# luo-ziyuan/NeRF_Signature

Hardware: AMD Instinct MI355X
Metric: training rays/sec @4096 rays (hotdog, 32-bit msg) (higher is better)
Workload: dtype f32 (hash gather, compositing) + fp16 MFMA with f32 accumulate (MLPs); 1 GPU; BASELINE configs[1]: Blender/hotdog-like S0, --wtmk_tcnn, 4096 content + 32x12x12 block rays, 32-bit msg; content_rays=4096, block_rays_total=4608, block_rays_this_rank=4608, message_dim=32, parallelism=dp1, capacity_overflow=False, recaptured_with_more_headroom_after_warmup=False, execution=hipgraph, graph_segments=1

## Files before the change

include/nerfsig.h:

```cpp
#ifndef NERFSIG_H_
#define NERFSIG_H_

#include <stddef.h>
#include <stdint.h>

#ifdef __cplusplus
extern "C" {
#endif

#define NSIG_OK 0
#define NSIG_ERR_ARG 1
#define NSIG_ERR_LAUNCH 2

#define NSIG_TABLE_ROWS (1u << 19)
#define NSIG_BASE_LEVELS 16
#define NSIG_MAX_MESSAGE_DIM 64

typedef void *nsig_stream_t;

int nsig_abi_version(void);
const char *nsig_last_error(void);


int rm_near_far_from_aabb(const float *rays_o, const float *rays_d, const float *aabb, uint32_t N, float min_near,
                          float *nears, float *fars, nsig_stream_t stream);
int rm_sph_from_ray(const float *rays_o, const float *rays_d, float radius, uint32_t N, float *coords,
                    nsig_stream_t stream);
int rm_morton3D(const int32_t *coords, uint32_t N, int32_t *indices, nsig_stream_t stream);
int rm_morton3D_invert(const int32_t *indices, uint32_t N, int32_t *coords, nsig_stream_t stream);
int rm_packbits(const float *grid, uint32_t n_bytes, float density_thresh, uint8_t *bitfield, nsig_stream_t stream);

size_t rg_refresh_draw_scratch_bytes(uint32_t N, uint32_t H);
int rg_refresh_begin(float *fresh, uint32_t n_cells, nsig_stream_t stream);
int rg_refresh_draw(int32_t *keys, int32_t *ids, uint32_t N, uint32_t H, const float *grid_cas, void *scratch, uint64_t seed, const int32_t *iter_dev,
                    uint32_t cas, nsig_stream_t stream);
int rg_refresh_points(const int32_t *keys, const int32_t *ids, uint32_t n, uint32_t H, float extent, float half_cell, uint64_t seed, const int32_t *iter_dev,
                      uint32_t cas, float *xyz, int32_t *cells, nsig_stream_t stream);
int rg_refresh_scatter(const float *sigmas, const int32_t *cells, uint32_t n, float density_scale, float *fresh, nsig_stream_t stream);
size_t rg_refresh_partials_bytes(uint32_t n_cells);
int rg_refresh_finish(float *grid, const float *fresh, uint32_t n_cells, float decay, void *partials, float density_thresh, uint8_t *bitfield,
                      float *mean_density, int32_t *iter_dev, const int32_t *count_ring, uint32_t window, const uint32_t *step_dev, int32_t *mean_count,
                      nsig_stream_t stream);


size_t rm_march_train_scratch_bytes(uint32_t N, uint32_t max_steps);
int rm_march_train_count(const float *rays_o, const float *rays_d, const uint8_t *grid, float bound, float dt_gamma,
                         uint32_t max_steps, uint32_t N, uint32_t C, uint32_t H, const float *nears,
                         const float *fars, const float *noises, int32_t *counts, float *t_rec,
                         nsig_stream_t stream);
int rm_march_train_scan(const int32_t *counts, uint32_t N, int32_t *rays, int32_t *counter, nsig_stream_t stream);
int rm_march_train_scan_blocks(uint32_t N);
int rm_march_train_scan_wide(const int32_t *counts, uint32_t N, int32_t *rays, int32_t *counter, int32_t *block_sums,
                             nsig_stream_t stream);
int rm_march_train_write(const float *rays_o, const float *rays_d, float bound, float dt_gamma, uint32_t max_steps,
                         uint32_t N, uint32_t C, uint32_t H, uint32_t M, const float *nears, const float *noises,
                         const float *t_rec, const int32_t *rays, const int32_t *counter, float *xyzs, float *dirs,
                         float *deltas, nsig_stream_t stream);

int rm_march_train_count_nf(const float *rays_o, const float *rays_d, const float *aabb, float min_near, const uint8_t *grid,
                            float bound, float dt_gamma, uint32_t max_steps, uint32_t N, uint32_t C, uint32_t H,
                            const float *noises, float *nears, float *fars, int32_t *counts, float *t_rec, nsig_stream_t stream);
int rm_march_train_scan_write_max_rays(void);
int rm_march_train_scan_write(const float *rays_o, const float *rays_d, float bound, float dt_gamma, uint32_t max_steps, uint32_t N,
                              uint32_t C, uint32_t H, uint32_t M, const float *nears, const float *noises, const float *t_rec,
                              const int32_t *counts, int32_t *rays, int32_t *counter, float *xyzs, float *dirs, float *deltas,
                              nsig_stream_t stream);

int rm_composite_train_fwd(const float *sigmas, const float *rgbs, const float *deltas, const int32_t *rays,
                           uint32_t M, uint32_t N, float T_thresh, float *weights_sum, float *depth, float *image,
                           nsig_stream_t stream);
int rm_composite_train_bwd(const float *grad_weights_sum, const float *grad_image, const float *sigmas,
                           const float *rgbs, const float *deltas, const int32_t *rays, const float *weights_sum,
                           const float *image, uint32_t M, uint32_t N, float T_thresh, float *grad_sigmas,
                           float *grad_rgbs, nsig_stream_t stream);


int rm_march(uint32_t n_alive, uint32_t n_step, const int32_t *rays_alive, const float *rays_t, const float *rays_o,
             const float *rays_d, float bound, float dt_gamma, uint32_t max_steps, uint32_t C, uint32_t H,
             const uint8_t *grid, const float *nears, const float *fars, float *xyzs, float *dirs, float *deltas,
             const float *noises, uint32_t M_rows, nsig_stream_t stream);
int rm_composite(uint32_t n_alive, uint32_t n_step, float T_thresh, int32_t *rays_alive, float *rays_t,
                 const float *sigmas, const float *rgbs, const float *deltas, float *weights_sum, float *depth,
                 float *image, nsig_stream_t stream);
int rm_compact_alive(const int32_t *rays_alive, uint32_t n_alive, int32_t *rays_alive_out, int32_t *n_out,
                     nsig_stream_t stream);

int rm_eval_begin(uint32_t N, uint32_t *ctl, int32_t *rays_alive, nsig_stream_t stream);
int rm_eval_march(const uint32_t *ctl, uint32_t N, const int32_t *rays_alive, const float *rays_t, const float *rays_o, const float *rays_d,
                  float bound, float dt_gamma, uint32_t max_steps, uint32_t C, uint32_t H, const uint8_t *density_bitfield, const float *fars,
                  float *xyzs, float *dirs, float *deltas, const float *noises, nsig_stream_t stream);
int rm_eval_composite(const uint32_t *ctl, uint32_t N, float T_thresh, float density_scale, int32_t *rays_alive, float *rays_t,
                      const float *sigmas, const float *rgbs, const float *deltas, float *weights_sum, float *depth, float *image,
                      nsig_stream_t stream);
int rm_eval_compact(uint32_t *ctl, uint32_t N, uint32_t max_steps, const int32_t *rays_alive, int32_t *rays_alive_out, nsig_stream_t stream);


int rg_get_rays(const float *poses, float fx, float fy, float cx, float cy, uint32_t H, uint32_t W, const int64_t *inds,
                uint32_t B, uint32_t N, float *rays_o, float *rays_d, nsig_stream_t stream);

int rg_sample_rays(const float *poses, uint32_t P, const float *images, float fx, float fy, float cx, float cy, uint32_t H, uint32_t W,
                   uint32_t N, const int32_t *step_counter, uint32_t stride, uint32_t offset, uint64_t seed, float *rays_o, float *rays_d,
                   float *gt, int64_t *inds_out, int32_t *pose_out, nsig_stream_t stream);


int hg_codebook_presum(const float *const *tables_host, uint32_t D, float *S, nsig_stream_t stream);

int hg_codebook_presum_sel(const float *const *all_tables_host, const float *message, uint32_t D, float *S,
                           nsig_stream_t stream);

int hg_encode_fwd(const float *x01, uint32_t M, const float *const *base_tables_host, const float *S, float *feat,
                  nsig_stream_t stream);

int hg_codebook_encode_fwd(const float *x01, uint32_t M, const float *const *tables_host, uint32_t D, float *out,
                           nsig_stream_t stream);

int hg_codebook_bwd(const float *x01, uint32_t M, const float *dfeat, float *G, nsig_stream_t stream);

int hg_scatter_sliced(const float *rec, uint32_t M, float *G, nsig_stream_t stream);

size_t hg_scatter_binned_scratch_bytes(uint32_t M);
int hg_scatter_binned(const float *rec, uint32_t M, float *G, void *scratch, nsig_stream_t stream);

size_t hg_scatter_plan_bytes(uint32_t M);
int hg_scatter_plan(const float *xyzs, uint32_t M, float bound, void *plan, nsig_stream_t stream);
int hg_scatter_planned(const void *plan, uint32_t M, float *G, nsig_stream_t stream);

int hg_fanout_grad(const float *G, float *const *grads_host, uint32_t D, int accumulate, nsig_stream_t stream);

int hg_level_lookup(const float *x01, uint32_t M, float resolution, int32_t *rows, float *weights,
                    nsig_stream_t stream);


int opt_codebook_adam(const float *G, float *const *params_host, float *const *exp_avg_host, float *const *exp_avg_sq_host,
                      uint32_t D, float beta1, float beta2, float eps, const float *step_size_host,
                      const float *inv_bc2_sqrt_host, float grad_scale, nsig_stream_t stream);

int opt_codebook_adam_sel(const float *G, float *const *params_host, float *const *exp_avg_host, float *const *exp_avg_sq_host,
                          float *const *steps_host, const float *message, uint32_t D, const float *lr, float beta1,
                          float beta2, float eps, float grad_scale, float *scratch, nsig_stream_t stream);

int opt_codebook_adam_sel_next(const float *G, float *const *params_host, float *const *exp_avg_host, float *const *exp_avg_sq_host,
                               float *const *steps_host, const float *message, uint32_t D, const float *lr, float beta1,
                               float beta2, float eps, float grad_scale, float *scratch, const float *next_message,
                               float *S_next, nsig_stream_t stream);


size_t mlp_packed_bytes(void);
int mlp_pack_weights(const float *sigma_params, const float *color_params, void *packed, nsig_stream_t stream);

int mlp_get_precision(void);
int mlp_set_precision(int mode);
int mlp_get_pipelined(void);
int mlp_set_pipelined(int mask);

#define FIELD_MASK_WORDS 6

#define NSIG_PLANES_F32 0
#define NSIG_PLANES_MIXED 1
int field_fwd(const float *xyzs, const float *dirs, uint32_t M, float bound, const float *const *base_tables_host,
              const float *S, const void *packed, float *sigmas, float *rgbs, float *geo_feat, uint32_t *masks,
              const void *planes, int planes_layout, nsig_stream_t stream);

size_t hg_planes_bytes(uint32_t M);
int hg_encode_planes(const float *xyzs, uint32_t M, float bound, const float *const *base_tables_host, const float *S,
                     void *planes, nsig_stream_t stream);
int hg_encode_planes_rows(const float *xyzs, uint32_t M_capacity, const uint32_t *rows_dev, float bound,
                          const float *const *base_tables_host, const float *S, void *planes, nsig_stream_t stream);
int hg_encode_planes_mixed(const float *xyzs, uint32_t M_capacity, const uint32_t *rows_dev, float bound, const float *const *base_tables_host,
                           const float *S, void *planes, nsig_stream_t stream);
int field_fwd_rows(const float *xyzs, const float *dirs, uint32_t M_capacity, const uint32_t *rows_dev, float bound,
                   const float *const *base_tables_host, const float *S, const void *packed, float *sigmas, float *rgbs, const void *planes,
                   int planes_layout, nsig_stream_t stream);

int hg_warm_tables(const float *const *base_tables_host, const float *S, float *sink, nsig_stream_t stream);

int hg_encode_codebook_plane(const float *xyzs, uint32_t M, float bound, const float *S, void *planes, int planes_layout, void *plan_to_reset,
                             nsig_stream_t stream);

int field_color_fwd(const float *dirs, const float *geo_feat, uint32_t M, const void *packed, float *rgbs,
                    nsig_stream_t stream);

int field_bwd(const float *xyzs, uint32_t M, float bound, const float *grad_sigmas, const float *grad_rgbs,
              const float *sigmas, const float *rgbs, const uint32_t *masks, const void *packed, float *G,
              float *dfeat_out, float *rec_out, nsig_stream_t stream);
int field_bwd_planned(const float *xyzs, uint32_t M, float bound, const float *grad_sigmas, const float *grad_rgbs,
                      const float *sigmas, const float *rgbs, const uint32_t *masks, const void *packed, void *plan,
                      nsig_stream_t stream);

int opt_adam_dense(uint32_t n, float *const *params_host, const float *const *grads_host, float *const *exp_avg_host,
                   float *const *exp_avg_sq_host, float *const *steps_host, const uint32_t *numel_host, const float *lr, float beta1,
                   float beta2, float eps, float grad_scale, float *scratch, nsig_stream_t stream);
int opt_adam_dense_host(uint32_t n, float *const *params_host, const float *const *grads_host, float *const *exp_avg_host,
                        float *const *exp_avg_sq_host, const uint32_t *numel_host, const float *step_sizes_host, const float *inv_bc2_host,
                        float beta1, float beta2, float eps, float grad_scale, nsig_stream_t stream);

int rm_composite_train_finish_fwd(const float *sigmas, const float *rgbs, const float *deltas, const int32_t *rays, uint32_t M, uint32_t N,
                                  float T_thresh, const float *nears, const float *fars, const float *bg, uint32_t bg_stride,
                                  float *weights_sum, float *depth, float *image, float *image_out, float *depth_out, nsig_stream_t stream);
int rm_composite_train_finish_bwd(const float *grad_weights_sum, const float *grad_image_out, const float *sigmas, const float *rgbs,
                                  const float *deltas, const int32_t *rays, const float *weights_sum, const float *image, const float *bg,
                                  uint32_t bg_stride, uint32_t M, uint32_t N, float T_thresh, uint32_t rays_in_order, float *grad_sigmas,
                                  float *grad_rgbs, nsig_stream_t stream);


int rm_finish_fwd(const float *image, const float *depth, const float *weights_sum, const float *nears, const float *fars, const float *bg,
                  uint32_t bg_stride, uint32_t N, float *image_out, float *depth_out, nsig_stream_t stream);
int rm_finish_bwd(const float *grad_image, const float *grad_depth, const float *depth, const float *nears, const float *fars, const float *bg,
                  uint32_t bg_stride, uint32_t N, float *grad_weights_sum, float *grad_depth_in, nsig_stream_t stream);

int loop_step_begin(float *G, uint32_t n_floats, const float *ring_dev, uint32_t slots, uint32_t width, uint32_t *counter, float *msg,
                    nsig_stream_t stream);
void *nsig_host_device_pointer(const void *pinned_host);

int wm_loss_fwd(const float *content, const float *gt, uint32_t n_content, const float *decoded, const float *message, uint32_t D, float temp,
                float lambda_w, float lambda_i, float *losses3, float *d_content, float *d_decoded, nsig_stream_t stream);
int wm_loss_bwd(const float *g_lossi, const float *g_lossw, const float *g_loss, float lambda_w, float lambda_i, const float *d_content,
                uint32_t n_content, const float *d_decoded, uint32_t D, float *grad_content, float *grad_decoded, nsig_stream_t stream);


int dec_bn_gelu_fwd(const float *x, const float *gamma, const float *beta, uint32_t N, uint32_t C, uint32_t P, float eps, float *y,
                    float *save, nsig_stream_t stream);
int dec_bn_gelu_bwd(const float *dy, const float *x, const float *gamma, const float *beta, const float *save, uint32_t N, uint32_t C,
                    uint32_t P, float *dx, float *dgamma, float *dbeta, nsig_stream_t stream);

size_t dec_workspace_bytes(uint32_t B, uint32_t Cin, uint32_t H, uint32_t W);
int dec_forward(const float *img, uint32_t input_mode, const float *mean_host, const float *std_host, const float *const *params_host,
                uint32_t B, uint32_t Cin, uint32_t H, uint32_t W, float eps, void *workspace, float *decoded, float *clamped_out,
                nsig_stream_t stream);
int dec_backward(const float *grad_decoded, const float *img, uint32_t input_mode, const float *mean_host, const float *std_host,
                 const float *const *params_host, uint32_t B, uint32_t Cin, uint32_t H, uint32_t W, void *workspace,
                 float *const *grads_host, float *grad_img, nsig_stream_t stream, nsig_stream_t weights_stream);

int dec_forward_train(const float *img, const float *mean_host, const float *std_host, const float *const *params_host, uint32_t B,
                      uint32_t Cin, uint32_t H, uint32_t W, float eps, void *workspace, float *decoded, float *clamped_out,
                      uint32_t distortion, const float *dist_param, const float *dist_noise, const float *bce_message, float bce_temp,
                      float bce_scale, float *bce_seed, nsig_stream_t stream);
int dec_backward_train(const float *grad_decoded, const float *img, const float *mean_host, const float *std_host,
                       const float *const *params_host, uint32_t B, uint32_t Cin, uint32_t H, uint32_t W, void *workspace,
                       float *const *grads_host, float *grad_img, uint32_t distortion, const float *dist_param,
                       const float *dist_noise, float *grad_scratch, nsig_stream_t stream, nsig_stream_t weights_stream);
int wm_distort_draw(uint32_t distortion, uint64_t seed, const uint32_t *step_counter, uint32_t n_noise, float *param_out,
                    float *noise_out, nsig_stream_t stream);
int wm_distort_fwd(const float *img, uint32_t B, uint32_t H, uint32_t W, uint32_t C, uint32_t distortion, const float *dist_param,
                   const float *dist_noise, float *out, nsig_stream_t stream);
int wm_distort_bwd(const float *grad_out, const float *img, uint32_t B, uint32_t H, uint32_t W, uint32_t C, uint32_t distortion,
                   const float *dist_param, const float *dist_noise, float *grad_img, nsig_stream_t stream);
int wm_distort_geom_fwd(const float *img, uint32_t B, uint32_t H, uint32_t W, uint32_t C, uint32_t distortion, const float *dist_param,
                        uint32_t W_out, float *out, float *clamped_out, nsig_stream_t stream);
int wm_distort_geom_bwd(const float *grad_out, const float *img, uint32_t B, uint32_t H, uint32_t W, uint32_t C, uint32_t distortion,
                        const float *dist_param, uint32_t W_out, float *grad_img, nsig_stream_t stream);


int field_fwd_trace(const float *xyzs, const float *dirs, uint32_t M, float bound, const float *const *base_tables_host,
                    const void *packed, const void *planes, float *sigmas, float *rgbs, uint32_t *masks, float *act_hs,
                    float *act_cin, float *act_h1, float *act_h2, nsig_stream_t stream);
int field_bwd_trace(uint32_t M, const float *grad_sigmas, const float *grad_rgbs, const float *sigmas, const float *rgbs,
                    const uint32_t *masks, const void *packed, float *d_hs, float *d_so, float *d_h1, float *d_h2, float *d_out,
                    void *d_planes, nsig_stream_t stream);
int hg_scatter_level(const float *xyzs, float bound, const void *d_plane, uint32_t M, uint32_t level, float *G,
                     nsig_stream_t stream);
size_t hg_scatter_levels_scratch_bytes(uint32_t M);
int hg_scatter_levels(const float *xyzs, float bound, const void *d_planes, uint32_t M, uint32_t stride, float *const *G_host,
                      void *scratch, nsig_stream_t stream);


int field_fwd_trace_rows(const float *xyzs, const float *dirs, uint32_t M_capacity, const uint32_t *rows_dev, float bound,
                         const float *const *base_tables_host, const void *packed, const void *planes, float *sigmas, float *rgbs,
                         uint32_t *masks, float *act_hs, float *act_cin, float *act_h1, float *act_h2, nsig_stream_t stream);
int field_bwd_trace_rows(uint32_t M_capacity, const uint32_t *rows_dev, const float *grad_sigmas, const float *grad_rgbs, const float *sigmas,
                         const float *rgbs, const uint32_t *masks, const void *packed, float *d_hs, float *d_so, float *d_h1, float *d_h2,
                         float *d_out, void *d_planes, nsig_stream_t stream);
size_t field_wgrad_scratch_bytes(uint32_t M);
int field_wgrad(uint32_t M, const uint32_t *rows_dev, const void *planes, const float *act_hs, const float *act_cin, const float *act_h1,
                const float *act_h2, const float *d_hs, const float *d_so, const float *d_h1, const float *d_h2, const float *d_out,
                void *scratch, float *grad_sigma_params, float *grad_color_params, nsig_stream_t stream);
size_t field_bwd_wgrad_scratch_bytes(uint32_t M);
int field_bwd_wgrad(uint32_t M, const uint32_t *rows_dev, const float *grad_sigmas, const float *grad_rgbs, const float *sigmas, const float *rgbs,
                    const uint32_t *masks, const void *packed, const void *planes, const float *act_hs, const float *act_cin, const float *act_h1,
                    const float *act_h2, void *d_planes, void *scratch, float *grad_sigma_params, float *grad_color_params, nsig_stream_t stream);
int field_fwd_trace_f16(const float *xyzs, const float *dirs, uint32_t M_capacity, const uint32_t *rows_dev, float bound,
                        const float *const *base_tables_host, const void *packed, const void *planes, float *sigmas, float *rgbs,
                        uint32_t *masks, void *act_hs, void *act_cin, void *act_h1, void *act_h2, nsig_stream_t stream);
int field_bwd_wgrad_f16(uint32_t M, const uint32_t *rows_dev, const float *grad_sigmas, const float *grad_rgbs, const float *sigmas, const float *rgbs,
                        const uint32_t *masks, const void *packed, const void *planes, const void *act_hs, const void *act_cin, const void *act_h1,
                        const void *act_h2, void *d_planes, void *scratch, float *grad_sigma_params, float *grad_color_params, nsig_stream_t stream);
int rm_composite_train_mse(const float *sigmas, const float *rgbs, const float *deltas, const int32_t *rays, uint32_t M, uint32_t N, float T_thresh,
                           const float *nears, const float *fars, const float *bg, uint32_t bg_stride, const float *gt, uint32_t n_values,
                           float grad_scale, float *weights_sum, float *depth, float *image, float *image_out, float *depth_out, float *grad_image,
                           float *grad_sigmas, float *grad_rgbs, nsig_stream_t stream);
int opt_ema_update(uint32_t n, const float *const *params_host, float *const *shadow_host, const uint32_t *numel_host, const uint32_t *num_updates,
                   double decay, nsig_stream_t stream);
int clean_loss(const float *image, const float *gt, uint32_t n_values, float grad_scale, float *loss, float *grad_image,
               uint32_t *step_dev, const int32_t *march_counter, int32_t *count_ring, float *loss_ring, uint32_t loss_ring_len,
               float *noise_next, uint32_t n_noise, uint64_t seed, nsig_stream_t stream);
size_t hg_levels_plan_bytes(uint32_t M);
int hg_levels_plan(const float *xyzs, uint32_t M, const uint32_t *rows_dev, float bound, void *plan, nsig_stream_t stream);
int hg_levels_scatter(const float *xyzs, uint32_t M, const uint32_t *rows_dev, float bound, const void *d_planes, uint32_t stride,
                      void *plan, float *const *G_host, nsig_stream_t stream);
int hg_levels_scatter_adam(const float *xyzs, uint32_t M, const uint32_t *rows_dev, float bound, const void *d_planes, uint32_t stride,
                           void *plan, float *const *params_host, float *const *exp_avg_host, float *const *exp_avg_sq_host,
                           float *const *steps_host, const float *lr, float beta1, float beta2, float eps, float grad_scale, float *scratch,
                           nsig_stream_t stream);


size_t mc_scratch_bytes(uint32_t nx, uint32_t ny, uint32_t nz);
int mc_count(const float *u, uint32_t nx, uint32_t ny, uint32_t nz, float threshold, void *scratch, uint32_t *totals, nsig_stream_t stream);
int mc_emit(const float *u, uint32_t nx, uint32_t ny, uint32_t nz, float threshold, void *scratch, uint32_t n_vertices, uint32_t n_triangles,
            float *vertices, int32_t *triangles, nsig_stream_t stream);

#ifdef __cplusplus
}
#endif
#endif
```

nerf_signature_amd/_native.py:

```python
import ctypes
import os

import torch

_PKG = os.path.dirname(os.path.abspath(__file__))
LIB_PATH = os.path.join(_PKG, "lib", "libnerfsig.so")

_c = ctypes
_vp, _u32, _fl, _int, _sz = _c.c_void_p, _c.c_uint32, _c.c_float, _c.c_int, _c.c_size_t

SIGNATURES = {
    "nsig_abi_version": [],
    "nsig_last_error": [],
    "nsig_host_device_pointer": [_vp],
    "rg_sample_rays": [_vp, _u32, _vp, _fl, _fl, _fl, _fl, _u32, _u32, _u32, _vp, _u32, _u32, _c.c_uint64, _vp, _vp, _vp, _vp, _vp, _vp],
    "rg_get_rays": [_vp, _fl, _fl, _fl, _fl, _u32, _u32, _vp, _u32, _u32, _vp, _vp, _vp],
    "rm_near_far_from_aabb": [_vp, _vp, _vp, _u32, _fl, _vp, _vp, _vp],
    "rm_sph_from_ray": [_vp, _vp, _fl, _u32, _vp, _vp],
    "rm_morton3D": [_vp, _u32, _vp, _vp],
    "rm_morton3D_invert": [_vp, _u32, _vp, _vp],
    "rm_packbits": [_vp, _u32, _fl, _vp, _vp],
    "rg_refresh_draw_scratch_bytes": [_u32, _u32],
    "rg_refresh_begin": [_vp, _u32, _vp],
    "rg_refresh_draw": [_vp, _vp, _u32, _u32, _vp, _vp, _c.c_uint64, _vp, _u32, _vp],
    "rg_refresh_points": [_vp, _vp, _u32, _u32, _fl, _fl, _c.c_uint64, _vp, _u32, _vp, _vp, _vp],
    "rg_refresh_scatter": [_vp, _vp, _u32, _fl, _vp, _vp],
    "rg_refresh_partials_bytes": [_u32],
    "rg_refresh_finish": [_vp, _vp, _u32, _fl, _vp, _fl, _vp, _vp, _vp, _vp, _u32, _vp, _vp, _vp],
    "rm_march_train_scratch_bytes": [_u32, _u32],
    "rm_march_train_count": [_vp, _vp, _vp, _fl, _fl, _u32, _u32, _u32, _u32, _vp, _vp, _vp, _vp, _vp, _vp],
    "rm_march_train_scan": [_vp, _u32, _vp, _vp, _vp],
    "rm_march_train_scan_blocks": [_u32],
    "rm_march_train_scan_wide": [_vp, _u32, _vp, _vp, _vp, _vp],
    "rm_march_train_write": [_vp, _vp, _fl, _fl, _u32, _u32, _u32, _u32, _u32, _vp, _vp, _vp, _vp, _vp, _vp, _vp, _vp, _vp],
    "rm_march_train_count_nf": [_vp, _vp, _vp, _fl, _vp, _fl, _fl, _u32, _u32, _u32, _u32, _vp, _vp, _vp, _vp, _vp, _vp],
    "rm_march_train_scan_write_max_rays": [],
    "rm_march_train_scan_write": [_vp, _vp, _fl, _fl, _u32, _u32, _u32, _u32, _u32, _vp, _vp, _vp, _vp, _vp, _vp, _vp, _vp, _vp, _vp],
    "rm_composite_train_fwd": [_vp, _vp, _vp, _vp, _u32, _u32, _fl, _vp, _vp, _vp, _vp],
    "rm_composite_train_bwd": [_vp, _vp, _vp, _vp, _vp, _vp, _vp, _vp, _u32, _u32, _fl, _vp, _vp, _vp],
    "rm_march": [_u32, _u32, _vp, _vp, _vp, _vp, _fl, _fl, _u32, _u32, _u32, _vp, _vp, _vp, _vp, _vp, _vp, _vp, _u32, _vp],
    "rm_composite": [_u32, _u32, _fl, _vp, _vp, _vp, _vp, _vp, _vp, _vp, _vp, _vp],
    "rm_compact_alive": [_vp, _u32, _vp, _vp, _vp],
    "rm_eval_begin": [_u32, _vp, _vp, _vp],
    "rm_eval_march": [_vp, _u32, _vp, _vp, _vp, _vp, _fl, _fl, _u32, _u32, _u32, _vp, _vp, _vp, _vp, _vp, _vp, _vp],
    "rm_eval_composite": [_vp, _u32, _fl, _fl, _vp, _vp, _vp, _vp, _vp, _vp, _vp, _vp, _vp],
    "rm_eval_compact": [_vp, _u32, _u32, _vp, _vp, _vp],
    "hg_encode_planes_rows": [_vp, _u32, _vp, _fl, _vp, _vp, _vp, _vp],
    "hg_encode_planes_mixed": [_vp, _u32, _vp, _fl, _vp, _vp, _vp, _vp],
    "field_fwd_rows": [_vp, _vp, _u32, _vp, _fl, _vp, _vp, _vp, _vp, _vp, _vp, _int, _vp],
    "hg_codebook_presum": [_vp, _u32, _vp, _vp],
    "hg_codebook_presum_sel": [_vp, _vp, _u32, _vp, _vp],
    "hg_encode_fwd": [_vp, _u32, _vp, _vp, _vp, _vp],
    "hg_codebook_encode_fwd": [_vp, _u32, _vp, _u32, _vp, _vp],
    "hg_codebook_bwd": [_vp, _u32, _vp, _vp, _vp],
    "hg_scatter_sliced": [_vp, _u32, _vp, _vp],
    "hg_fanout_grad": [_vp, _vp, _u32, _int, _vp],
    "hg_level_lookup": [_vp, _u32, _fl, _vp, _vp, _vp],
    "opt_codebook_adam": [_vp, _vp, _vp, _vp, _u32, _fl, _fl, _fl, _vp, _vp, _fl, _vp],
    "opt_codebook_adam_sel": [_vp, _vp, _vp, _vp, _vp, _vp, _u32, _vp, _fl, _fl, _fl, _fl, _vp, _vp],
    "opt_codebook_adam_sel_next": [_vp, _vp, _vp, _vp, _vp, _vp, _u32, _vp, _fl, _fl, _fl, _fl, _vp, _vp, _vp, _vp],
    "mlp_packed_bytes": [],
    "mlp_get_precision": [],
    "mlp_set_precision": [_int],
    "mlp_get_pipelined": [],
    "mlp_set_pipelined": [_int],
    "mlp_pack_weights": [_vp, _vp, _vp, _vp],
    "hg_planes_bytes": [_u32],
    "hg_encode_planes": [_vp, _u32, _fl, _vp, _vp, _vp, _vp],
    "hg_warm_tables": [_vp, _vp, _vp, _vp],
    "hg_encode_codebook_plane": [_vp, _u32, _fl, _vp, _vp, _int, _vp, _vp],
    "field_fwd": [_vp, _vp, _u32, _fl, _vp, _vp, _vp, _vp, _vp, _vp, _vp, _vp, _int, _vp],
    "field_color_fwd": [_vp, _vp, _u32, _vp, _vp, _vp],
    "opt_adam_dense_host": [_u32, _vp, _vp, _vp, _vp, _vp, _vp, _vp, _fl, _fl, _fl, _fl, _vp],
    "opt_adam_dense": [_u32, _vp, _vp, _vp, _vp, _vp, _vp, _vp, _fl, _fl, _fl, _fl, _vp, _vp],
    "rm_composite_train_finish_fwd": [_vp, _vp, _vp, _vp, _u32, _u32, _fl, _vp, _vp, _vp, _u32, _vp, _vp, _vp, _vp, _vp, _vp],
    "rm_composite_train_finish_bwd": [_vp, _vp, _vp, _vp, _vp, _vp, _vp, _vp, _vp, _u32, _u32, _u32, _fl, _u32, _vp, _vp, _vp],
    "rm_finish_fwd": [_vp, _vp, _vp, _vp, _vp, _vp, _u32, _u32, _vp, _vp, _vp],
    "rm_finish_bwd": [_vp, _vp, _vp, _vp, _vp, _vp, _u32, _u32, _vp, _vp, _vp],
    "loop_step_begin": [_vp, _u32, _vp, _u32, _u32, _vp, _vp, _vp],
    "wm_loss_fwd": [_vp, _vp, _u32, _vp, _vp, _u32, _fl, _fl, _fl, _vp, _vp, _vp, _vp],
    "wm_loss_bwd": [_vp, _vp, _vp, _fl, _fl, _vp, _u32, _vp, _u32, _vp, _vp, _vp],
    "dec_bn_gelu_fwd": [_vp, _vp, _vp, _u32, _u32, _u32, _fl, _vp, _vp, _vp],
    "dec_bn_gelu_bwd": [_vp, _vp, _vp, _vp, _vp, _u32, _u32, _u32, _vp, _vp, _vp, _vp],
    "dec_workspace_bytes": [_u32, _u32, _u32, _u32],
    "dec_forward": [_vp, _u32, _vp, _vp, _vp, _u32, _u32, _u32, _u32, _fl, _vp, _vp, _vp, _vp],
    "dec_backward": [_vp, _vp, _u32, _vp, _vp, _vp, _u32, _u32, _u32, _u32, _vp, _vp, _vp, _vp, _vp],
    "dec_forward_train": [_vp, _vp, _vp, _vp, _u32, _u32, _u32, _u32, _fl, _vp, _vp, _vp, _u32, _vp, _vp, _vp, _fl, _fl, _vp, _vp],
    "dec_backward_train": [_vp, _vp, _vp, _vp, _vp, _u32, _u32, _u32, _u32, _vp, _vp, _vp, _u32, _vp, _vp, _vp, _vp, _vp],
    "wm_distort_draw": [_u32, _c.c_uint64, _vp, _u32, _vp, _vp, _vp],
    "wm_distort_fwd": [_vp, _u32, _u32, _u32, _u32, _u32, _vp, _vp, _vp, _vp],
    "wm_distort_bwd": [_vp, _vp, _u32, _u32, _u32, _u32, _u32, _vp, _vp, _vp, _vp],
    "wm_distort_geom_fwd": [_vp, _u32, _u32, _u32, _u32, _u32, _vp, _u32, _vp, _vp, _vp],
    "wm_distort_geom_bwd": [_vp, _vp, _u32, _u32, _u32, _u32, _u32, _vp, _u32, _vp, _vp],
    "field_fwd_trace": [_vp, _vp, _u32, _fl, _vp, _vp, _vp, _vp, _vp, _vp, _vp, _vp, _vp, _vp, _vp],
    "field_bwd_trace": [_u32, _vp, _vp, _vp, _vp, _vp, _vp, _vp, _vp, _vp, _vp, _vp, _vp, _vp],
    "hg_scatter_level": [_vp, _fl, _vp, _u32, _u32, _vp, _vp],
    "hg_scatter_binned_scratch_bytes": [_u32],
    "hg_scatter_binned": [_vp, _u32, _vp, _vp, _vp],
    "hg_scatter_levels_scratch_bytes": [_u32],
    "hg_scatter_levels": [_vp, _fl, _vp, _u32, _u32, _vp, _vp, _vp],
    "field_bwd": [_vp, _u32, _fl, _vp, _vp, _vp, _vp, _vp, _vp, _vp, _vp, _vp, _vp],
    "field_bwd_planned": [_vp, _u32, _fl, _vp, _vp, _vp, _vp, _vp, _vp, _vp, _vp],
    "hg_scatter_plan_bytes": [_u32],
    "hg_scatter_plan": [_vp, _u32, _fl, _vp, _vp],
    "hg_scatter_planned": [_vp, _u32, _vp, _vp],
    "field_fwd_trace_rows": [_vp, _vp, _u32, _vp, _fl, _vp, _vp, _vp, _vp, _vp, _vp, _vp, _vp, _vp, _vp, _vp],
    "field_fwd_trace_f16": [_vp, _vp, _u32, _vp, _fl, _vp, _vp, _vp, _vp, _vp, _vp, _vp, _vp, _vp, _vp, _vp],
    "field_bwd_trace_rows": [_u32, _vp, _vp, _vp, _vp, _vp, _vp, _vp, _vp, _vp, _vp, _vp, _vp, _vp, _vp],
    "field_wgrad_scratch_bytes": [_u32],
    "field_wgrad": [_u32, _vp, _vp, _vp, _vp, _vp, _vp, _vp, _vp, _vp, _vp, _vp, _vp, _vp, _vp, _vp],
    "field_bwd_wgrad_scratch_bytes": [_u32],
    "field_bwd_wgrad": [_u32, _vp, _vp, _vp, _vp, _vp, _vp, _vp, _vp, _vp, _vp, _vp, _vp, _vp, _vp, _vp, _vp, _vp],
    "field_bwd_wgrad_f16": [_u32, _vp, _vp, _vp, _vp, _vp, _vp, _vp, _vp, _vp, _vp, _vp, _vp, _vp, _vp, _vp, _vp, _vp],
    "rm_composite_train_mse": [_vp, _vp, _vp, _vp, _u32, _u32, _fl, _vp, _vp, _vp, _u32, _vp, _u32, _fl, _vp, _vp, _vp, _vp, _vp, _vp, _vp, _vp, _vp],
    "opt_ema_update": [_u32, _vp, _vp, _vp, _vp, _c.c_double, _vp],
    "clean_loss": [_vp, _vp, _u32, _fl, _vp, _vp, _vp, _vp, _vp, _vp, _u32, _vp, _u32, _c.c_uint64, _vp],
    "hg_levels_plan_bytes": [_u32],
    "hg_levels_plan": [_vp, _u32, _vp, _fl, _vp, _vp],
    "hg_levels_scatter": [_vp, _u32, _vp, _fl, _vp, _u32, _vp, _vp, _vp],
    "hg_levels_scatter_adam": [_vp, _u32, _vp, _fl, _vp, _u32, _vp, _vp, _vp, _vp, _vp, _vp, _fl, _fl, _fl, _fl, _vp, _vp],
    "mc_scratch_bytes": [_u32, _u32, _u32],
    "mc_count": [_vp, _u32, _u32, _u32, _fl, _vp, _vp, _vp],
    "mc_emit": [_vp, _u32, _u32, _u32, _fl, _vp, _u32, _u32, _vp, _vp, _vp],
}
_RESTYPES = {"nsig_last_error": _c.c_char_p, "nsig_host_device_pointer": _c.c_void_p, "rm_march_train_scratch_bytes": _sz, "mlp_packed_bytes": _sz, "hg_planes_bytes": _sz, "dec_workspace_bytes": _sz, "hg_scatter_levels_scratch_bytes": _sz, "hg_scatter_binned_scratch_bytes": _sz, "hg_scatter_plan_bytes": _sz, "field_wgrad_scratch_bytes": _sz, "field_bwd_wgrad_scratch_bytes": _sz, "hg_levels_plan_bytes": _sz, "rg_refresh_partials_bytes": _sz, "rg_refresh_draw_scratch_bytes": _sz, "mc_scratch_bytes": _sz}

_lib = None


class NativeError(RuntimeError):
    pass


def load():
    global _lib
    if _lib is not None:
        return _lib
    path = os.environ.get("NERFSIG_LIB", LIB_PATH)
    if not os.path.exists(path):
        raise NativeError(f"{path} not found: the HIP extension is required (no fallback). "
                          f"Build it with `python -m nerf_signature_amd.build`.")
    _lib = ctypes.CDLL(path)
    _lib.nsig_last_error.restype = _c.c_char_p
    return _lib


_bound = {}


def fn(name):
    f = _bound.get(name)
    if f is None:
        lib = load()
        try:
            f = getattr(lib, name)
        except AttributeError as e:
            raise NativeError(f"libnerfsig.so does not export {name}; rebuild with `python -m nerf_signature_amd.build --force`") from e
        f.argtypes = SIGNATURES[name]
        f.restype = _RESTYPES.get(name, _int)
        _bound[name] = f
    return f


def verify_exports():
    for name in SIGNATURES:
        fn(name)
    return sorted(SIGNATURES)


def call(name, *args):
    rc = fn(name)(*args)
    if rc != 0:
        msg = load().nsig_last_error().decode("utf-8", "replace")
        raise (ValueError if rc == 1 else NativeError)(f"{name} failed (code {rc}): {msg}")


def mlp_precision_name():
    return ("fp16 MFMA with f32 accumulate (MLPs)" if fn("mlp_get_precision")() == 1 else "split-bf16 MFMA (3 per product) with f32 accumulate (MLPs)")


def mlp_mfma_per_wave():
    return (24, "f16") if fn("mlp_get_precision")() == 1 else (72, "bf16")


def set_mlp_precision(name):
    call("mlp_set_precision", {"bf16x3": 0, "f16": 1}[name])


def ptr(t):
    if t is None:
        return None
    if not t.is_cuda:
        raise ValueError("libnerfsig entry points take device tensors; got a CPU tensor")
    if not t.is_contiguous():
        raise ValueError("libnerfsig entry points take contiguous tensors")
    return t.data_ptr()


_raw_stream = getattr(torch._C, "_cuda_getCurrentRawStream", None)


def stream():
    if _raw_stream is not None:
        return _raw_stream(torch.cuda.current_device())
    return torch.cuda.current_stream().cuda_stream


def ptr_array(tensors):
    arr = (ctypes.c_void_p * len(tensors))(*[ptr(t) for t in tensors])
    return arr


def check(t, dtype, name, shape_last=None):
    if t.dtype != dtype:
        raise ValueError(f"{name}: expected dtype {dtype}, got {t.dtype}")
    if shape_last is not None and t.shape[-1] != shape_last:
        raise ValueError(f"{name}: expected last dimension {shape_last}, got {tuple(t.shape)}")
    return t
```

nerf_signature_amd/csrc/field.hip:

```cpp
#include <cstdlib>
#include <cstring>
#include <mutex>
#include <unordered_set>
#include "fieldmlp.h"

#include <stdlib.h>

namespace nsig {


__device__ inline float fwd_weight(int frag, int lane, int j, const float *__restrict__ sp, const float *__restrict__ cp) {
    const int r = lane & 31, h = lane >> 5;
    if (frag < F1) {
        const int rb = (frag - F0) >> 1, ks = (frag - F0) & 1;
        return sp[kSigmaW1 + (32 * rb + r) * 32 + 16 * ks + 8 * h + j];
    }
    if (frag < F2) return r < 16 ? sp[kSigmaW2 + r * 64 + k_from_acc(frag - F1, h, j)] : 0.0f;
    if (frag < F3) {
        const int rb = (frag - F2) >> 1, ks = (frag - F2) & 1;
        int cin;
        if (ks == 0) cin = 8 * h + j;
        else { const int rho = row_of_reg(h, j); cin = rho == 0 ? 31 : 15 + rho; }
        return cp[kColorW1 + (32 * rb + r) * 32 + cin];
    }
// ... 477 lines not shown
        color_branch<P>(lds, lane, h, dirs[3 * (size_t)sl], dirs[3 * (size_t)sl + 1], dirs[3 * (size_t)sl + 2], geo8, mask_c, rgb);
        if (s < M && h == 0) { rgbs[3 * (size_t)s] = rgb[0]; rgbs[3 * (size_t)s + 1] = rgb[1]; rgbs[3 * (size_t)s + 2] = rgb[2]; }
    }
}


template <typename P, bool kFull = false>
__global__ void __launch_bounds__(256) k_field_bwd(const float *__restrict__ xyzs, uint32_t M, float bound, float cb_cell,
                                                   const float *__restrict__ g_sigma, const float *__restrict__ g_rgb,
                                                   const float *__restrict__ sigmas, const float *__restrict__ rgbs,
                                                   const uint32_t *__restrict__ masks, const char *__restrict__ packed,
                                                   float *__restrict__ G, float *__restrict__ dfeat_out, float *__restrict__ rec_out,
                                                   GradTrace gt = GradTrace{}, uint32_t stride = 0, ScatterPlan plan = ScatterPlan{},
                                                   const uint32_t *__restrict__ rows_dev = nullptr) {
    extern __shared__ __attribute__((aligned(16))) char lds[];
    if (rows_dev != nullptr) {
        const uint32_t r = *rows_dev;
        if (r == 0) return;
        M = min(M, r);
    }
    stage_weights(lds, packed + P::kBwdOffset, (int)P::kBwdLds);
    constexpr size_t kHalf = kBwdBytes;
    constexpr bool kNormalise = P::kMfmaPerProduct == 1 && !kFull;
    const int lane = threadIdx.x & 63, wid = threadIdx.x >> 6;
    const int p = lane & 31, h = lane >> 5;
    const uint32_t n_tiles = ceil_div(M, 32u);
    const float e_lo = expf(-15.0f), e_hi = expf(15.0f);
    const bool planned = !kFull && plan.hd != nullptr;
    uint32_t gbits = 0;
    const uint32_t xcd = blockIdx.x & 7u, per_xcd = gridDim.x >> 3, n_chunks = ceil_div(n_tiles, 32u);
    for (uint32_t lq = blockIdx.x >> 3;; lq += per_xcd) {
        const uint32_t chunk = (lq >> 3) * 8u + xcd;
        if (chunk >= n_chunks) break;
        const uint32_t tile = (chunk * 8u + (lq & 7u)) * 4u + wid;
        if (tile >= n_tiles) continue;
        const uint32_t s = tile * 32 + p;
        const bool live = s < M;
        const uint32_t sl = min(s, M - 1);
        const uint32_t *mrow = masks + (size_t)tile * 192 + lane;
        const uint32_t mask_s = mrow[0], mask_c0 = mrow[64], mask_c1 = mrow[128];
        uint4 dst = make_uint4(0u, 0u, 0u, 0u);
        if (planned) dst = plan.dest[sl];

        typename P::Op dout[1];
        float dv[8];
#pragma unroll
        for (int j = 0; j < 8; ++j) {
            float v = 0.0f;
            if (j < 3 && h == 0 && live) {
                const float c = rgbs[3 * (size_t)sl + j];
                v = g_rgb[3 * (size_t)sl + j] * (c * (1.0f - c));
            }
            dv[j] = v;
            if (kFull) gt.d_out[(size_t)(8 * h + j) * stride + s] = v;
        }
        float head0 = 0.0f;
        if (h == 0 && live) head0 = g_sigma[sl] * fminf(fmaxf(sigmas[sl], e_lo), e_hi);
        float unscale = 1.0f;
        if (kNormalise) {
            float amp = fmaxf(fmaxf(fabsf(dv[0]), fabsf(dv[1])), fmaxf(fabsf(dv[2]), fabsf(head0)));
            amp = fmaxf(amp, __shfl_xor(amp, 32, 64));
            const uint32_t e = (__float_as_uint(amp) >> 23) & 0xffu;
            if (e >= 1u && e <= 253u) {
                const float sc = __uint_as_float((254u - e) << 23);
                unscale = __uint_as_float(e << 23);
                dv[0] *= sc; dv[1] *= sc; dv[2] *= sc; head0 *= sc;
            }
        }
#pragma unroll
        for (int j = 0; j < 8; j += 2) P::put2(dout[0], j >> 1, dv[j], dv[j + 1]);
        f32x16 hid[2];
        typename P::Op b4[4];
        mfma_layer<P, 2, 1>(lds, kHalf, B0, lane, dout, hid);
        mask_to_operand<P>(hid, mask_c1, b4);
        if (kFull) store_rows64(gt.d_h2, stride, s, h, hid, [=](float v, int i) { return ((mask_c1 >> mask_bit<P>(i)) & 1u) ? v : 0.0f; });
        mfma_layer<P, 2, 4>(lds, kHalf, B1, lane, b4, hid);
        mask_to_operand<P>(hid, mask_c0, b4);
        if (kFull) store_rows64(gt.d_h1, stride, s, h, hid, [=](float v, int i) { return ((mask_c0 >> mask_bit<P>(i)) & 1u) ? v : 0.0f; });
        f32x16 dso[1];
        mfma_layer<P, 1, 4>(lds, kHalf, B2, lane, b4, dso);

        typename P::Op dhead[1];
        float head8[8];
#pragma unroll
        for (int r = 0; r < 8; ++r) head8[r] = dso[0][r];
        if (h == 0) head8[0] = head0;
#pragma unroll
        for (int r = 0; r < 8; ++r)
            if (kFull) gt.d_so[(size_t)row_of_reg(h, r) * stride + s] = head8[r];
#pragma unroll
        for (int r = 0; r < 8; r += 2) P::put2(dhead[0], r >> 1, head8[r], head8[r + 1]);
        mfma_layer<P, 2, 1>(lds, kHalf, B3, lane, dhead, hid);
        mask_to_operand<P>(hid, mask_s, b4);
        if (kFull) {
            store_rows64(gt.d_hs, stride, s, h, hid, [=](float v, int i) { return ((mask_s >> mask_bit<P>(i)) & 1u) ? v : 0.0f; });
            f32x16 dall[1];
            mfma_layer<P, 1, 4>(lds, kHalf, B4F, lane, b4, dall);
#pragma unroll
            for (int r = 0; r < 16; r += 2) {
                float2 v;
                v.x = dall[0][r]; v.y = dall[0][r + 1];
                gt.d_planes[(size_t)(row_of_reg16(h, r) >> 1) * stride + s] = v;
            }
            continue;
        }
        f32x16 dfe[1];
        mfma_layer<P, 1, 4>(lds, kHalf, B4, lane, b4, dfe);

        const float g0 = __shfl(dfe[0][0], p, 64) * unscale, g1 = __shfl(dfe[0][1], p, 64) * unscale;
        if (!live) continue;
        if (dfeat_out != nullptr && h == 0) { dfeat_out[2 * (size_t)s] = g0; dfeat_out[2 * (size_t)s + 1] = g1; }
        const float two_b = 2.0f * bound;
        const float x01 = (xyzs[3 * (size_t)s] + bound) / two_b, y01 = (xyzs[3 * (size_t)s + 1] + bound) / two_b, z01 = (xyzs[3 * (size_t)s + 2] + bound) / two_b;
        if (planned) {
            uint32_t ix, iy, iz;
            float wx, wy, wz;
            codebook_axis(x01, ix, wx);
            codebook_axis(y01, iy, wy);
            codebook_axis(z01, iz, wz);
            const uint32_t q0 = 2u * (uint32_t)h;
            plan.queue[h ? dst.z : dst.x] = pair_entry(ix, pair_hash(iy, iz, q0), wx, wy, wz, g0, g1, q0);
            plan.queue[h ? dst.w : dst.y] = pair_entry(ix, pair_hash(iy, iz, q0 + 1u), wx, wy, wz, g0, g1, q0 + 1u);
            gbits = max(gbits, max(__float_as_uint(g0) & 0x7fffffffu, __float_as_uint(g1) & 0x7fffffffu));
            continue;
        }
        if (rec_out != nullptr && h == 0) {
            uint32_t ix, iy, iz;
            float wx, wy, wz;
            codebook_axis(x01, ix, wx);
            codebook_axis(y01, iy, wy);
            codebook_axis(z01, iz, wz);
            uint4 *r4 = reinterpret_cast<uint4 *>(rec_out) + 2 * (size_t)s;
            r4[0] = make_uint4(ix | (iy << 16), iz, __float_as_uint(wx), __float_as_uint(wy));
            r4[1] = make_uint4(__float_as_uint(wz), __float_as_uint(g0), __float_as_uint(g1), 0u);
        }
        if (G == nullptr || (g0 == 0.0f && g1 == 0.0f)) continue;
        Corner8 c;
        corner_rows(x01, y01, z01, cb_cell, c);
#pragma unroll
        for (int k = 0; k < 8; ++k) {
            if ((k >> 2) != h) continue;
            float *row = G + 2 * (size_t)c.row[k];
            atomicAdd(row, corner_weight(c, k, g0));
            atomicAdd(row + 1, corner_weight(c, k, g1));
        }
    }
    if (planned) {
#pragma unroll
        for (int d = 32; d >= 1; d >>= 1) gbits = max(gbits, (uint32_t)__shfl_xor((int)gbits, d, 64));
        if (lane == 0 && gbits > __hip_atomic_load(&plan.hd->gmax_bits, __ATOMIC_RELAXED, __HIP_MEMORY_SCOPE_AGENT)) atomicMax(&plan.hd->gmax_bits, gbits);
    }
}

template <typename P>
__device__ inline void field_bwd_pipelined(const char *lds, int lane, const float *__restrict__ xyzs, uint32_t M, float bound,
                                           const float *__restrict__ g_sigma, const float *__restrict__ g_rgb, const float *__restrict__ sigmas,
                                           const float *__restrict__ rgbs, const uint32_t *__restrict__ masks, ScatterPlan plan) {
    constexpr size_t kHalf = kBwdBytes;
    constexpr bool kNormalise = P::kMfmaPerProduct == 1;
    const int p = lane & 31, h = lane >> 5;
    const uint32_t wid = (uint32_t)__builtin_amdgcn_readfirstlane((int)(threadIdx.x >> 6));
    const uint32_t n_tiles = ceil_div(M, 32u);
    const float e_lo = expf(-15.0f), e_hi = expf(15.0f), two_b = 2.0f * bound;
    uint32_t gbits = 0;
    const uint32_t xcd = blockIdx.x & 7u, per_xcd = gridDim.x >> 3, n_chunks = ceil_div(n_tiles, 32u);
    uint32_t lq = blockIdx.x >> 3;
    auto next_tile = [&]() -> uint32_t {
        for (;; lq += per_xcd) {
            const uint32_t chunk = (lq >> 3) * 8u + xcd;
            if (chunk >= n_chunks) return ~0u;
            const uint32_t tile = (chunk * 8u + (lq & 7u)) * 4u + wid;
            if (tile < n_tiles) {
                lq += per_xcd;
                return tile;
            }
        }
    };
    typedef float f32x3u __attribute__((ext_vector_type(3), aligned(4)));
    uint32_t n_mask[3] = {0u, 0u, 0u};
    typedef uint32_t u32x4 __attribute__((ext_vector_type(4)));
    u32x4 n_dst = {0u, 0u, 0u, 0u};
    f32x3u n_rgb = {0.0f, 0.0f, 0.0f}, n_grgb = {0.0f, 0.0f, 0.0f}, n_xyz = {0.0f, 0.0f, 0.0f};
    float n_gs = 0.0f, n_sig = 0.0f;
    auto request = [&](uint32_t tile) {
        const uint32_t s = tile * 32 + p, sl = min(s, M - 1);
        const uint32_t *mrow = masks + (size_t)tile * 192 + lane;
        n_mask[0] = mrow[0]; n_mask[1] = mrow[64]; n_mask[2] = mrow[128];
        n_dst = *reinterpret_cast<const u32x4 *>(plan.dest + sl);
        n_rgb = *reinterpret_cast<const f32x3u *>(rgbs + 3 * (size_t)sl);
        n_grgb = *reinterpret_cast<const f32x3u *>(g_rgb + 3 * (size_t)sl);
        n_xyz = *reinterpret_cast<const f32x3u *>(xyzs + 3 * (size_t)sl);
        n_gs = g_sigma[sl];
        n_sig = sigmas[sl];
    };
    bool have = false;
    float p_x = 0.0f, p_y = 0.0f, p_z = 0.0f, p_g0 = 0.0f, p_g1 = 0.0f;
    uint32_t p_d0 = 0u, p_d1 = 0u;
    bool p_live = false;
    auto store_prev = [&]() {
        if (!p_live) return;
        uint32_t ix, iy, iz;
        float wx, wy, wz;
        codebook_axis((p_x + bound) / two_b, ix, wx);
        codebook_axis((p_y + bound) / two_b, iy, wy);
        codebook_axis((p_z + bound) / two_b, iz, wz);
        const uint32_t q0 = 2u * (uint32_t)h;
        plan.queue[p_d0] = pair_entry(ix, pair_hash(iy, iz, q0), wx, wy, wz, p_g0, p_g1, q0);
        plan.queue[p_d1] = pair_entry(ix, pair_hash(iy, iz, q0 + 1u), wx, wy, wz, p_g0, p_g1, q0 + 1u);
        gbits = max(gbits, max(__float_as_uint(p_g0) & 0x7fffffffu, __float_as_uint(p_g1) & 0x7fffffffu));
    };
    uint32_t tile = next_tile();
    if (tile != ~0u) request(tile);
    while (tile != ~0u) {
        const uint32_t s = tile * 32 + p;
        const bool live = s < M;
        float dv[3] = {0.0f, 0.0f, 0.0f}, head0 = 0.0f;
        if (h == 0 && live) {
            dv[0] = n_grgb.x * (n_rgb.x * (1.0f - n_rgb.x));
            dv[1] = n_grgb.y * (n_rgb.y * (1.0f - n_rgb.y));
            dv[2] = n_grgb.z * (n_rgb.z * (1.0f - n_rgb.z));
            head0 = n_gs * fminf(fmaxf(n_sig, e_lo), e_hi);
        }
        uint32_t mask_s = n_mask[0], mask_c0 = n_mask[1], mask_c1 = n_mask[2];
        uint32_t d0 = h ? n_dst.z : n_dst.x, d1 = h ? n_dst.w : n_dst.y;
        float cx = n_xyz.x, cy = n_xyz.y, cz = n_xyz.z;
        asm volatile("" : "+v"(dv[0]), "+v"(dv[1]), "+v"(dv[2]), "+v"(head0), "+v"(mask_s), "+v"(mask_c0), "+v"(mask_c1), "+v"(d0), "+v"(d1),
                     "+v"(cx), "+v"(cy), "+v"(cz) :: "memory");
        if (have) store_prev();
        const uint32_t upcoming = next_tile();
        if (upcoming != ~0u) request(upcoming);
        asm volatile("" ::: "memory");

        float unscale = 1.0f;
        if (kNormalise) {
            float amp = fmaxf(fmaxf(fabsf(dv[0]), fabsf(dv[1])), fmaxf(fabsf(dv[2]), fabsf(head0)));
            amp = fmaxf(amp, __shfl_xor(amp, 32, 64));
            const uint32_t e = (__float_as_uint(amp) >> 23) & 0xffu;
            if (e >= 1u && e <= 253u) {
                const float sc = __uint_as_float((254u - e) << 23);
                unscale = __uint_as_float(e << 23);
                dv[0] *= sc; dv[1] *= sc; dv[2] *= sc; head0 *= sc;
            }
        }
        typename P::Op dout[1];
        P::put2(dout[0], 0, dv[0], dv[1]);
        P::put2(dout[0], 1, dv[2], 0.0f);
        P::put2(dout[0], 2, 0.0f, 0.0f);
        P::put2(dout[0], 3, 0.0f, 0.0f);
        f32x16 hid[2];
        typename P::Op b4[4];
        mfma_layer<P, 2, 1>(lds, kHalf, B0, lane, dout, hid);
        mask_to_operand<P>(hid, mask_c1, b4);
        mfma_layer<P, 2, 4>(lds, kHalf, B1, lane, b4, hid);
        mask_to_operand<P>(hid, mask_c0, b4);
        f32x16 dso[1];
        mfma_layer<P, 1, 4>(lds, kHalf, B2, lane, b4, dso);
        typename P::Op dhead[1];
        float head8[8];
#pragma unroll
        for (int r = 0; r < 8; ++r) head8[r] = dso[0][r];
        if (h == 0) head8[0] = head0;
#pragma unroll
        for (int r = 0; r < 8; r += 2) P::put2(dhead[0], r >> 1, head8[r], head8[r + 1]);
        mfma_layer<P, 2, 1>(lds, kHalf, B3, lane, dhead, hid);
        mask_to_operand<P>(hid, mask_s, b4);
        f32x16 dfe[1];
        mfma_layer<P, 1, 4>(lds, kHalf, B4, lane, b4, dfe);
        p_g0 = __shfl(dfe[0][0], p, 64) * unscale;
        p_g1 = __shfl(dfe[0][1], p, 64) * unscale;
        p_x = cx; p_y = cy; p_z = cz; p_d0 = d0; p_d1 = d1; p_live = live;
        have = true;
        tile = upcoming;
    }
    if (have) store_prev();
#pragma unroll
    for (int d = 32; d >= 1; d >>= 1) gbits = max(gbits, (uint32_t)__shfl_xor((int)gbits, d, 64));
    if (lane == 0 && gbits > __hip_atomic_load(&plan.hd->gmax_bits, __ATOMIC_RELAXED, __HIP_MEMORY_SCOPE_AGENT)) atomicMax(&plan.hd->gmax_bits, gbits);
}

template <typename P>
__global__ void __launch_bounds__(256) k_field_bwd_train(const float *__restrict__ xyzs, uint32_t M, float bound, const float *__restrict__ g_sigma,
                                                         const float *__restrict__ g_rgb, const float *__restrict__ sigmas, const float *__restrict__ rgbs,
                                                         const uint32_t *__restrict__ masks, const char *__restrict__ packed, ScatterPlan plan) {
    extern __shared__ __attribute__((aligned(16))) char lds[];
    stage_weights(lds, packed + P::kBwdOffset, (int)P::kBwdLds);
    field_bwd_pipelined<P>(lds, threadIdx.x & 63, xyzs, M, bound, g_sigma, g_rgb, sigmas, rgbs, masks, plan);
}

}

using namespace nsig;

NSIG_EXPORT size_t mlp_packed_bytes(void) { return kPackedBytes; }

static int g_mlp_precision = -1;
static int mlp_precision() {
    if (g_mlp_precision < 0) {
        const char *e = getenv("NERFSIG_MLP");
        g_mlp_precision = (e != nullptr && (e[0] == 'b' || e[0] == 'B')) ? 0 : 1;
    }
    return g_mlp_precision;
}
NSIG_EXPORT int mlp_get_precision(void) { return mlp_precision(); }
NSIG_EXPORT int mlp_set_precision(int mode) {
    NSIG_REQUIRE(mode == 0 || mode == 1, "mlp_set_precision: 0 (bf16x3) or 1 (f16)");
    g_mlp_precision = mode;
    return NSIG_OK;
}

NSIG_EXPORT int mlp_pack_weights(const float *sigma_params, const float *color_params, void *packed, nsig_stream_t stream) {
    NSIG_REQUIRE(sigma_params && color_params && packed, "mlp_pack_weights: null pointer");
    NSIG_REQUIRE((reinterpret_cast<uintptr_t>(packed) & 15) == 0, "mlp_pack_weights: packed must be 16-byte aligned");
    const int total = (kFwdFrags + kBwdFrags) * 512;
    k_pack_weights<<<ceil_div(total, 256), 256, 0, as_stream(stream)>>>(sigma_params, color_params, reinterpret_cast<__bf16 *>(packed));
    return check_launch("mlp_pack_weights");
}

static int g_mlp_pipelined = 3;
static int mlp_pipelined() {
    return g_mlp_pipelined;
}
static bool fwd_pipelined() { return (mlp_pipelined() & 1) != 0; }
static bool bwd_pipelined() { return (mlp_pipelined() & 2) != 0; }
NSIG_EXPORT int mlp_get_pipelined(void) { return mlp_pipelined(); }
NSIG_EXPORT int mlp_set_pipelined(int mask) {
    NSIG_REQUIRE(mask >= 0 && mask <= 3, "mlp_set_pipelined: bit 0 = forward, bit 1 = backward");
    g_mlp_pipelined = mask;
    return NSIG_OK;
}
static uint32_t field_grid(uint32_t M, bool forward = false, uint32_t per_cu = 0) {
    const uint32_t blocks = ceil_div(ceil_div(ceil_div(M, 32u), 4u), 8u) * 8u;
    const uint32_t cap = (uint32_t)kCUs * (per_cu ? per_cu : (forward ? 4u : 3u));
    return blocks < cap ? blocks : cap;
}

static int fill_base_tables(const float *const *host, TablePtrs &base, const char *who) {
    NSIG_REQUIRE(host, "%s: null base table list", who);
    for (int l = 0; l < NSIG_BASE_LEVELS; ++l) {
        NSIG_REQUIRE(host[l] != nullptr, "%s: base table %d is null", who, l);
        base.p[l] = host[l];
    }
    return NSIG_OK;
}

static SlotTable default_slots(bool with_codebook) {
    static const uint8_t kWith[8][4] = {{16, 255, 255, 255}, {15, 255, 255, 255}, {14, 0, 255, 255}, {13, 1, 255, 255}, {12, 2, 3, 255}, {11, 4, 5, 255}, {10, 9, 255, 255}, {8, 7, 6, 255}};
    static const uint8_t kWithout[8][4] = {{15, 255, 255, 255}, {14, 255, 255, 255}, {13, 255, 255, 255}, {12, 255, 255, 255}, {11, 0, 1, 255}, {10, 2, 3, 255}, {9, 8, 4, 255}, {7, 6, 5, 255}};
    SlotTable t{};
    for (int slot = 0; slot < 8; ++slot)
        for (int k = 0; k < 4; ++k) {
            const uint8_t l = (with_codebook ? kWith : kWithout)[slot][k];
            if (l != 255) t.level[slot][t.n[slot]++] = l;
        }
    return t;
}

NSIG_EXPORT int hg_warm_tables(const float *const *base_tables_host, const float *S, float *sink, nsig_stream_t stream) {
    NSIG_REQUIRE(sink != nullptr, "hg_warm_tables: sink is one writable float (never written)");
    TablePtrs base{};
    if (int e = fill_base_tables(base_tables_host, base, "hg_warm_tables")) return e;
    k_warm_tables<<<8 * 128, 256, 0, as_stream(stream)>>>(base, S, default_slots(S != nullptr), sink);
    return check_launch("hg_warm_tables");
}

NSIG_EXPORT size_t hg_planes_bytes(uint32_t M) { return (size_t)(NSIG_BASE_LEVELS + 1) * ceil_div(M, 32u) * 32u * sizeof(float2); }

static int check_layout(int layout, const char *who) {
    NSIG_REQUIRE(layout == NSIG_PLANES_F32 || layout == NSIG_PLANES_MIXED, "%s: planes_layout must be NSIG_PLANES_F32 (0) or NSIG_PLANES_MIXED (1)", who);
    return NSIG_OK;
}

static int encode_planes_impl(const float *xyzs, uint32_t M, float bound, const float *const *base_tables_host, const float *S, void *planes,
                              const uint32_t *rows_dev, nsig_stream_t stream, bool mixed = false) {
    if (M == 0) return NSIG_OK;
    NSIG_REQUIRE(xyzs && planes, "hg_encode_planes: null pointer");
    NSIG_REQUIRE(bound > 0.0f, "hg_encode_planes: bound must be positive");
    NSIG_REQUIRE((reinterpret_cast<uintptr_t>(planes) & 7) == 0, "hg_encode_planes: planes must be 8-byte aligned");
    TablePtrs base{};
    if (int e = fill_base_tables(base_tables_host, base, "hg_encode_planes")) return e;
    const uint32_t stride = ceil_div(M, 32u) * 32u;
    const SlotTable tab = default_slots(S != nullptr);
    int covered[NSIG_BASE_LEVELS + 1] = {};
    for (int s = 0; s < 8; ++s)
        for (int i = 0; i < tab.n[s]; ++i) covered[tab.level[s][i]] += 1;
    for (int l = 0; l < NSIG_BASE_LEVELS + (S != nullptr ? 1 : 0); ++l)
        NSIG_REQUIRE(covered[l] == 1, "hg_encode_planes: level %d is assigned to %d slots", l, covered[l]);
    NSIG_REQUIRE(S != nullptr || covered[NSIG_BASE_LEVELS] == 0, "hg_encode_planes: slot table names the codebook level but S is NULL");
    const uint32_t tiles = ceil_div(stride, 256u);
    const uint32_t per_slot = tiles < 8192u ? tiles : 8192u;
    if (mixed) k_encode_planes<true><<<per_slot * 8, 256, 0, as_stream(stream)>>>(xyzs, M, bound, base, make_level_geom(), S, reinterpret_cast<float2 *>(planes), stride, tab, rows_dev);
    else k_encode_planes<false><<<per_slot * 8, 256, 0, as_stream(stream)>>>(xyzs, M, bound, base, make_level_geom(), S, reinterpret_cast<float2 *>(planes), stride, tab, rows_dev);
    return check_launch("hg_encode_planes");
}

NSIG_EXPORT int hg_encode_planes_mixed(const float *xyzs, uint32_t M_capacity, const uint32_t *rows_dev, float bound, const float *const *base_tables_host,
                                       const float *S, void *planes, nsig_stream_t stream) {
    NSIG_REQUIRE(mlp_precision() == 1, "hg_encode_planes_mixed: the mixed layout carries the fp16 MLP's operands (mlp_set_precision(1))");
    return encode_planes_impl(xyzs, M_capacity, bound, base_tables_host, S, planes, rows_dev, stream, true);
}

NSIG_EXPORT int hg_encode_planes(const float *xyzs, uint32_t M, float bound, const float *const *base_tables_host, const float *S, void *planes,
                                 nsig_stream_t stream) {
    return encode_planes_impl(xyzs, M, bound, base_tables_host, S, planes, nullptr, stream);
}

NSIG_EXPORT int hg_encode_planes_rows(const float *xyzs, uint32_t M_capacity, const uint32_t *rows_dev, float bound, const float *const *base_tables_host,
                                      const float *S, void *planes, nsig_stream_t stream) {
    NSIG_REQUIRE(rows_dev != nullptr, "hg_encode_planes_rows: null row count");
    return encode_planes_impl(xyzs, M_capacity, bound, base_tables_host, S, planes, rows_dev, stream);
}

NSIG_EXPORT int hg_encode_codebook_plane(const float *xyzs, uint32_t M, float bound, const float *S, void *planes, int planes_layout, void *plan_to_reset,
                                         nsig_stream_t stream) {
    if (M == 0) return NSIG_OK;
    if (int e = check_layout(planes_layout, "hg_encode_codebook_plane")) return e;
    NSIG_REQUIRE(xyzs && S && planes, "hg_encode_codebook_plane: null pointer");
    NSIG_REQUIRE(bound > 0.0f, "hg_encode_codebook_plane: bound must be positive");
    NSIG_REQUIRE((reinterpret_cast<uintptr_t>(planes) & 7) == 0, "hg_encode_codebook_plane: planes must be 8-byte aligned");
    NSIG_REQUIRE(plan_to_reset == nullptr || (reinterpret_cast<uintptr_t>(plan_to_reset) & 15) == 0, "hg_encode_codebook_plane: plan must be 16-byte aligned");
    const uint32_t stride = ceil_div(M, 32u) * 32u;
    float2 *plane = planes_layout == NSIG_PLANES_MIXED ? mixed_f32_plane(planes, stride, NSIG_BASE_LEVELS) : reinterpret_cast<float2 *>(planes) + (size_t)NSIG_BASE_LEVELS * stride;
    k_encode_codebook_plane<<<ceil_div(stride, 256u), 256, 0, as_stream(stream)>>>(xyzs, M, bound, make_level_geom().cell[NSIG_BASE_LEVELS], S, plane, stride,
                                                                                  reinterpret_cast<BinHeader *>(plan_to_reset));
    return check_launch("hg_encode_codebook_plane");
}

static int field_fwd_impl(const float *xyzs, const float *dirs, uint32_t M, float bound, const float *const *base_tables_host,
                          const float *S, const void *packed, float *sigmas, float *rgbs, float *geo_feat, uint32_t *masks,
                          const void *planes, int planes_layout, const uint32_t *rows_dev, nsig_stream_t stream) {
    if (M == 0) return NSIG_OK;
    NSIG_REQUIRE(xyzs && packed && sigmas, "field_fwd: null pointer");
    NSIG_REQUIRE(rgbs == nullptr || dirs != nullptr, "field_fwd: dirs is required when rgbs is requested");
    NSIG_REQUIRE(bound > 0.0f, "field_fwd: bound must be positive");
    NSIG_REQUIRE((reinterpret_cast<uintptr_t>(packed) & 15) == 0, "field_fwd: packed must be 16-byte aligned");
    TablePtrs base{};
    if (int e = fill_base_tables(base_tables_host, base, "field_fwd")) return e;
    const char *pk = reinterpret_cast<const char *>(packed);
    hipStream_t st = as_stream(stream);
    const bool f16 = mlp_precision() == 1;
    if (planes == nullptr) {
        if (f16) k_field_fwd<F16, 0><<<field_grid(M, true), 256, F16::kFwdLds, st>>>(xyzs, dirs, M, bound, base, make_level_geom(), S, nullptr, 0, pk, sigmas, rgbs, geo_feat, masks, ActTrace{}, rows_dev);
        else k_field_fwd<Bf16x3, 0><<<field_grid(M, true), 256, Bf16x3::kFwdLds, st>>>(xyzs, dirs, M, bound, base, make_level_geom(), S, nullptr, 0, pk, sigmas, rgbs, geo_feat, masks, ActTrace{}, rows_dev);
        return check_launch("field_fwd");
    }
    NSIG_REQUIRE((reinterpret_cast<uintptr_t>(planes) & 7) == 0, "field_fwd: planes must be 8-byte aligned");
    const uint32_t stride = ceil_div(M, 32u) * 32u;
    const float2 *pl = reinterpret_cast<const float2 *>(planes);
    if (int e = check_layout(planes_layout, "field_fwd")) return e;
    const bool mixed = planes_layout == NSIG_PLANES_MIXED;
    NSIG_REQUIRE(!mixed || f16, "field_fwd: this plane set was written in the mixed (fp16) layout; the split-bf16 MLP needs hg_encode_planes");
    if (f16 && fwd_pipelined() && dirs != nullptr && rgbs != nullptr && geo_feat == nullptr) {
        if (mixed) k_field_fwd_train<F16, true><<<field_grid(M, true, 2), 256, F16::kFwdLds, st>>>(dirs, M, S != nullptr, pl, stride, pk, sigmas, rgbs, masks, rows_dev);
        else k_field_fwd_train<F16, false><<<field_grid(M, true, 2), 256, F16::kFwdLds, st>>>(dirs, M, S != nullptr, pl, stride, pk, sigmas, rgbs, masks, rows_dev);
        return check_launch("field_fwd");
    }
    if (f16) k_field_fwd<F16, 1><<<field_grid(M, true), 256, F16::kFwdLds, st>>>(xyzs, dirs, M, bound, base, make_level_geom(), S, pl, stride, pk, sigmas, rgbs, geo_feat, masks, ActTrace{}, rows_dev, mixed);
    else k_field_fwd<Bf16x3, 1><<<field_grid(M, true), 256, Bf16x3::kFwdLds, st>>>(xyzs, dirs, M, bound, base, make_level_geom(), S, pl, stride, pk, sigmas, rgbs, geo_feat, masks, ActTrace{}, rows_dev);
    return check_launch("field_fwd");
}

NSIG_EXPORT int field_fwd(const float *xyzs, const float *dirs, uint32_t M, float bound, const float *const *base_tables_host,
                          const float *S, const void *packed, float *sigmas, float *rgbs, float *geo_feat, uint32_t *masks,
                          const void *planes, int planes_layout, nsig_stream_t stream) {
    return field_fwd_impl(xyzs, dirs, M, bound, base_tables_host, S, packed, sigmas, rgbs, geo_feat, masks, planes, planes_layout, nullptr, stream);
}

NSIG_EXPORT int field_fwd_rows(const float *xyzs, const float *dirs, uint32_t M_capacity, const uint32_t *rows_dev, float bound,
                               const float *const *base_tables_host, const float *S, const void *packed, float *sigmas, float *rgbs, const void *planes,
                               int planes_layout, nsig_stream_t stream) {
    NSIG_REQUIRE(rows_dev != nullptr, "field_fwd_rows: null row count");
    return field_fwd_impl(xyzs, dirs, M_capacity, bound, base_tables_host, S, packed, sigmas, rgbs, nullptr, nullptr, planes, planes_layout, rows_dev, stream);
}

NSIG_EXPORT int field_color_fwd(const float *dirs, const float *geo_feat, uint32_t M, const void *packed, float *rgbs, nsig_stream_t stream) {
    if (M == 0) return NSIG_OK;
    NSIG_REQUIRE(dirs && geo_feat && packed && rgbs, "field_color_fwd: null pointer");
    if (mlp_precision() == 1) k_field_color<F16><<<field_grid(M), 256, F16::kFwdLds, as_stream(stream)>>>(dirs, geo_feat, M, reinterpret_cast<const char *>(packed), rgbs);
    else k_field_color<Bf16x3><<<field_grid(M), 256, Bf16x3::kFwdLds, as_stream(stream)>>>(dirs, geo_feat, M, reinterpret_cast<const char *>(packed), rgbs);
    return check_launch("field_color_fwd");
}

NSIG_EXPORT int field_bwd(const float *xyzs, uint32_t M, float bound, const float *grad_sigmas, const float *grad_rgbs, const float *sigmas,
                          const float *rgbs, const uint32_t *masks, const void *packed, float *G, float *dfeat_out, float *rec_out,
                          nsig_stream_t stream) {
    if (M == 0) return NSIG_OK;
    NSIG_REQUIRE(xyzs && grad_sigmas && grad_rgbs && sigmas && rgbs && masks && packed, "field_bwd: null pointer");
    NSIG_REQUIRE(G || dfeat_out || rec_out, "field_bwd: at least one of G / dfeat_out / rec_out must be given");
    NSIG_REQUIRE(bound > 0.0f, "field_bwd: bound must be positive");
    if (mlp_precision() == 1)
        k_field_bwd<F16, false><<<field_grid(M), 256, F16::kBwdLds, as_stream(stream)>>>(xyzs, M, bound, 1.0f / kCodebookResolution, grad_sigmas, grad_rgbs, sigmas, rgbs, masks,
                                                                                 reinterpret_cast<const char *>(packed), G, dfeat_out, rec_out);
    else
        k_field_bwd<Bf16x3, false><<<field_grid(M), 256, Bf16x3::kBwdLds, as_stream(stream)>>>(xyzs, M, bound, 1.0f / kCodebookResolution, grad_sigmas, grad_rgbs, sigmas, rgbs,
                                                                                       masks, reinterpret_cast<const char *>(packed), G, dfeat_out, rec_out);
    return check_launch("field_bwd");
}

NSIG_EXPORT int field_bwd_planned(const float *xyzs, uint32_t M, float bound, const float *grad_sigmas, const float *grad_rgbs, const float *sigmas,
                                  const float *rgbs, const uint32_t *masks, const void *packed, void *plan, nsig_stream_t stream) {
    if (M == 0) return NSIG_OK;
    NSIG_REQUIRE(xyzs && grad_sigmas && grad_rgbs && sigmas && rgbs && masks && packed && plan, "field_bwd_planned: null pointer");
    NSIG_REQUIRE(bound > 0.0f && (reinterpret_cast<uintptr_t>(plan) & 15) == 0 && M < (1u << 28), "field_bwd_planned: bound must be positive, plan 16-byte aligned, M < 2^28");
    if (mlp_precision() == 1 && bwd_pipelined())
        k_field_bwd_train<F16><<<field_grid(M), 256, F16::kBwdLds, as_stream(stream)>>>(xyzs, M, bound, grad_sigmas, grad_rgbs, sigmas, rgbs, masks,
                                                                                reinterpret_cast<const char *>(packed), scatter_plan_view(plan, M));
    else if (mlp_precision() == 1)
        k_field_bwd<F16, false><<<field_grid(M), 256, F16::kBwdLds, as_stream(stream)>>>(xyzs, M, bound, 1.0f / kCodebookResolution, grad_sigmas, grad_rgbs, sigmas, rgbs, masks,
                                                                                 reinterpret_cast<const char *>(packed), nullptr, nullptr, nullptr, GradTrace{}, 0,
                                                                                 scatter_plan_view(plan, M));
    else
        k_field_bwd<Bf16x3, false><<<field_grid(M), 256, Bf16x3::kBwdLds, as_stream(stream)>>>(xyzs, M, bound, 1.0f / kCodebookResolution, grad_sigmas, grad_rgbs, sigmas, rgbs,
                                                                                       masks, reinterpret_cast<const char *>(packed), nullptr, nullptr, nullptr, GradTrace{}, 0,
                                                                                       scatter_plan_view(plan, M));
    return check_launch("field_bwd_planned");
}


static int fwd_trace_impl(const float *xyzs, const float *dirs, uint32_t M, const uint32_t *rows_dev, float bound, const float *const *base_tables_host,
                          const void *packed, const void *planes, float *sigmas, float *rgbs, uint32_t *masks, float *act_hs,
                          float *act_cin, float *act_h1, float *act_h2, nsig_stream_t stream, bool trace_f16 = false) {
    if (M == 0) return NSIG_OK;
    NSIG_REQUIRE(xyzs && dirs && packed && planes && sigmas && rgbs && masks && act_hs && act_cin && act_h1 && act_h2, "field_fwd_trace: null pointer");
    NSIG_REQUIRE(bound > 0.0f, "field_fwd_trace: bound must be positive");
    NSIG_REQUIRE(M <= (1u << 26), "field_fwd_trace: M=%u out of range (<= 2^26: the lane part of a trace address is a 32-bit byte offset of up to 32 x stride)", M);
    TablePtrs base{};
    if (int e = fill_base_tables(base_tables_host, base, "field_fwd_trace")) return e;
    const uint32_t stride = ceil_div(M, 32u) * 32u;
    ActTrace tr{act_hs, act_cin, act_h1, act_h2};
    if (trace_f16)
        k_field_fwd_trace<_Float16><<<field_grid(M), 256, Bf16x3::kFwdLds, as_stream(stream)>>>(dirs, M, reinterpret_cast<const float2 *>(planes), stride,
                                                                                        reinterpret_cast<const char *>(packed), sigmas, rgbs, masks, tr, rows_dev);
    else if (!fwd_pipelined())
        k_field_fwd<Bf16x3, 1, true><<<field_grid(M), 256, Bf16x3::kFwdLds, as_stream(stream)>>>(xyzs, dirs, M, bound, base, make_level_geom(), nullptr,
                                                                                         reinterpret_cast<const float2 *>(planes), stride,
                                                                                         reinterpret_cast<const char *>(packed), sigmas, rgbs, nullptr, masks, tr,
                                                                                         rows_dev);
    else
        k_field_fwd_trace<float><<<field_grid(M), 256, Bf16x3::kFwdLds, as_stream(stream)>>>(dirs, M, reinterpret_cast<const float2 *>(planes), stride,
                                                                                     reinterpret_cast<const char *>(packed), sigmas, rgbs, masks, tr, rows_dev);
    return check_launch("field_fwd_trace");
}

NSIG_EXPORT int field_fwd_trace(const float *xyzs, const float *dirs, uint32_t M, float bound, const float *const *base_tables_host,
                                const void *packed, const void *planes, float *sigmas, float *rgbs, uint32_t *masks, float *act_hs,
                                float *act_cin, float *act_h1, float *act_h2, nsig_stream_t stream) {
    return fwd_trace_impl(xyzs, dirs, M, nullptr, bound, base_tables_host, packed, planes, sigmas, rgbs, masks, act_hs, act_cin, act_h1, act_h2, stream);
}

NSIG_EXPORT int field_fwd_trace_f16(const float *xyzs, const float *dirs, uint32_t M_capacity, const uint32_t *rows_dev, float bound,
                                    const float *const *base_tables_host, const void *packed, const void *planes, float *sigmas, float *rgbs, uint32_t *masks,
                                    void *act_hs, void *act_cin, void *act_h1, void *act_h2, nsig_stream_t stream) {
    return fwd_trace_impl(xyzs, dirs, M_capacity, rows_dev, bound, base_tables_host, packed, planes, sigmas, rgbs, masks, reinterpret_cast<float *>(act_hs),
                          reinterpret_cast<float *>(act_cin), reinterpret_cast<float *>(act_h1), reinterpret_cast<float *>(act_h2), stream, true);
}

NSIG_EXPORT int field_fwd_trace_rows(const float *xyzs, const float *dirs, uint32_t M_capacity, const uint32_t *rows_dev, float bound,
                                     const float *const *base_tables_host, const void *packed, const void *planes, float *sigmas, float *rgbs,
                                     uint32_t *masks, float *act_hs, float *act_cin, float *act_h1, float *act_h2, nsig_stream_t stream) {
    NSIG_REQUIRE(rows_dev != nullptr, "field_fwd_trace_rows: null row count");
    return fwd_trace_impl(xyzs, dirs, M_capacity, rows_dev, bound, base_tables_host, packed, planes, sigmas, rgbs, masks, act_hs, act_cin, act_h1, act_h2, stream);
}

static int bwd_trace_impl(uint32_t M, const uint32_t *rows_dev, const float *grad_sigmas, const float *grad_rgbs, const float *sigmas, const float *rgbs,
                          const uint32_t *masks, const void *packed, float *d_hs, float *d_so, float *d_h1, float *d_h2, float *d_out,
                          void *d_planes, nsig_stream_t stream) {
    if (M == 0) return NSIG_OK;
    NSIG_REQUIRE(grad_sigmas && grad_rgbs && sigmas && rgbs && masks && packed && d_hs && d_so && d_h1 && d_h2 && d_out && d_planes,
                 "field_bwd_trace: null pointer");
    NSIG_REQUIRE(M <= (1u << 26), "field_bwd_trace: M=%u out of range (<= 2^26: the lane part of a trace address is a 32-bit byte offset of up to 32 x stride)", M);
    const uint32_t stride = ceil_div(M, 32u) * 32u;
    GradTrace gt{d_hs, d_h1, d_h2, d_so, d_out, reinterpret_cast<float2 *>(d_planes)};
    k_field_bwd<Bf16x3, true><<<field_grid(M), 256, Bf16x3::kBwdLds, as_stream(stream)>>>(nullptr, M, 1.0f, 1.0f / kCodebookResolution, grad_sigmas, grad_rgbs, sigmas,
                                                                               rgbs, masks, reinterpret_cast<const char *>(packed), nullptr, nullptr,
                                                                               nullptr, gt, stride, ScatterPlan{}, rows_dev);
    return check_launch("field_bwd_trace");
}

NSIG_EXPORT int field_bwd_trace(uint32_t M, const float *grad_sigmas, const float *grad_rgbs, const float *sigmas, const float *rgbs,
                                const uint32_t *masks, const void *packed, float *d_hs, float *d_so, float *d_h1, float *d_h2, float *d_out,
                                void *d_planes, nsig_stream_t stream) {
    return bwd_trace_impl(M, nullptr, grad_sigmas, grad_rgbs, sigmas, rgbs, masks, packed, d_hs, d_so, d_h1, d_h2, d_out, d_planes, stream);
}

NSIG_EXPORT int field_bwd_trace_rows(uint32_t M_capacity, const uint32_t *rows_dev, const float *grad_sigmas, const float *grad_rgbs, const float *sigmas,
                                     const float *rgbs, const uint32_t *masks, const void *packed, float *d_hs, float *d_so, float *d_h1, float *d_h2,
                                     float *d_out, void *d_planes, nsig_stream_t stream) {
    NSIG_REQUIRE(rows_dev != nullptr, "field_bwd_trace_rows: null row count");
    return bwd_trace_impl(M_capacity, rows_dev, grad_sigmas, grad_rgbs, sigmas, rgbs, masks, packed, d_hs, d_so, d_h1, d_h2, d_out, d_planes, stream);
}
```

nerf_signature_amd/csrc/hashgrid.hip:

```cpp
#include <cstdlib>
#include "hashgrid.h"

namespace nsig {

__global__ void __launch_bounds__(256) k_codebook_presum(CodebookPtrs tabs, uint32_t D, float4 *__restrict__ S) {
    const uint32_t e = blockIdx.x * blockDim.x + threadIdx.x;
    if (e >= NSIG_TABLE_ROWS / 2) return;
    float4 acc = {0.f, 0.f, 0.f, 0.f};
    uint32_t i = 0;
    for (; i + 4 <= D; i += 4) {
        const float4 a = reinterpret_cast<const float4 *>(tabs.p[i])[e];
        const float4 b = reinterpret_cast<const float4 *>(tabs.p[i + 1])[e];
        const float4 c = reinterpret_cast<const float4 *>(tabs.p[i + 2])[e];
        const float4 d = reinterpret_cast<const float4 *>(tabs.p[i + 3])[e];
        acc.x = (((acc.x + a.x) + b.x) + c.x) + d.x;
        acc.y = (((acc.y + a.y) + b.y) + c.y) + d.y;
        acc.z = (((acc.z + a.z) + b.z) + c.z) + d.z;
        acc.w = (((acc.w + a.w) + b.w) + c.w) + d.w;
    }
    for (; i < D; ++i) {
        const float4 a = reinterpret_cast<const float4 *>(tabs.p[i])[e];
        acc.x += a.x; acc.y += a.y; acc.z += a.z; acc.w += a.w;
    }
    S[e] = acc;
// ... 500 lines not shown
        if (threadIdx.x == 0) pl.chunk_max[(size_t)level * pl.n_chunks + chunk] = 0u;
        return;
    }
    if (threadIdx.x < kBinSlices) {
        h[threadIdx.x] = 0;
        roff[threadIdx.x] = my_roff;
    }
    if (threadIdx.x == 0) wg_max = 0;
    __syncthreads();
    ENT_STAMP(0);
    const bool live = m < n, merged = level < kMergeLevels;
    LevelPoint p{};
    if (live) {
        const float two_b = 2.0f * bound, cell = geom.cell[level];
        axis_cell((px + bound) / two_b, cell, p.ix, p.wx);
        axis_cell((py + bound) / two_b, cell, p.iy, p.wy);
        axis_cell((pz + bound) / two_b, cell, p.iz, p.wz);
    } else {
        g = make_float2(0.0f, 0.0f);
    }
    const bool leader = run_leader(merged, live, p);
    uint32_t sl[4], hyz[4], rank[4];
    if (leader) {
#pragma unroll
        for (uint32_t q = 0; q < 4; ++q) {
            hyz[q] = pair_hash(p.iy, p.iz, q);
            sl[q] = pair_slice(hyz[q]);
            rank[q] = atomicAdd(&h[sl[q]], merged ? 2u : 1u);
        }
    }
    ENT_STAMP(1);
    float c[4][2][2];
    uint32_t gb = max(__float_as_uint(g.x) & 0x7fffffffu, __float_as_uint(g.y) & 0x7fffffffu);
    if (merged) {
        const uint32_t l16 = lane & 15u;
        const uint32_t row_leaders = (uint32_t)(__ballot(leader || !live) >> (lane & 48u)) & 0xffffu;
        const uint32_t higher = row_leaders & ~((2u << l16) - 1u);
        const uint32_t run_end = higher ? (uint32_t)__ffs((int)higher) - 2u : 15u;
        gb = 0;
#pragma unroll
        for (uint32_t q = 0; q < 4; ++q) {
            const float fz = (q & 1u) ? p.wz : 1.0f - p.wz, fy = (q >> 1) ? p.wy : 1.0f - p.wy;
            const float a0 = (g.x * fz) * fy, a1 = (g.y * fz) * fy;
            c[q][0][0] = run_sum(a0 * (1.0f - p.wx), l16, run_end);
            c[q][0][1] = run_sum(a1 * (1.0f - p.wx), l16, run_end);
            c[q][1][0] = run_sum(a0 * p.wx, l16, run_end);
            c[q][1][1] = run_sum(a1 * p.wx, l16, run_end);
            if (leader)
#pragma unroll
                for (int t = 0; t < 4; ++t) gb = max(gb, __float_as_uint(c[q][t >> 1][t & 1]) & 0x7fffffffu);
        }
    }
    ENT_STAMP(2);
    __syncthreads();
    ENT_STAMP(3);
    if (threadIdx.x < kBinSlices) {
        const uint32_t t = h[threadIdx.x];
        uint32_t incl = t;
#pragma unroll
        for (int d = 1; d < 64; d <<= 1) {
            const uint32_t v = (uint32_t)__shfl_up((int)incl, d, 64);
            if ((int)threadIdx.x >= d) incl += v;
        }
        base[threadIdx.x] = incl - t;
        if (threadIdx.x == kBinSlices - 1) base[kBinSlices] = incl;
    }
    __syncthreads();
    ENT_STAMP(4);
    const uint32_t total = base[kBinSlices];
    const bool direct = total > kLevelStage;
    uint4 *__restrict__ queue = pl.queue + (size_t)level * kLevelQueueStride * M;
    if (leader) {
#pragma unroll
        for (uint32_t q = 0; q < 4; ++q) {
            uint4 e0, e1 = make_uint4(0u, 0u, 0u, 0u);
            if (merged) {
                const uint32_t key = p.ix | ((hyz[q] & (kBinRows - 1)) << 16);
                e0 = make_uint4(key, __float_as_uint(0.0f), __float_as_uint(c[q][0][0]), __float_as_uint(c[q][0][1]));
                e1 = make_uint4(key, __float_as_uint(1.0f), __float_as_uint(c[q][1][0]), __float_as_uint(c[q][1][1]));
            } else {
                e0 = pair_entry(p.ix, hyz[q], p.wx, p.wy, p.wz, g.x, g.y, q);
            }
            if (direct) {
                uint4 *__restrict__ dst = queue + roff[sl[q]] + rank[q];
                dst[0] = e0;
                if (merged) dst[1] = e1;
            } else {
                const uint32_t at = base[sl[q]] + rank[q];
                staged[at] = e0;
                slice_of[at] = (uint8_t)sl[q];
                if (merged) {
                    staged[at + 1] = e1;
                    slice_of[at + 1] = (uint8_t)sl[q];
                }
            }
        }
    }
    ENT_STAMP(5);
    __syncthreads();
    ENT_STAMP(6);
    if (!direct && total != 0u) {
        typedef uint32_t u32x4_t __attribute__((ext_vector_type(4)));
        constexpr uint32_t kPer = kLevelStage / kBinThreads;
        uint32_t sj[kPer], ro[kPer], ba[kPer];
        u32x4_t e[kPer];
#pragma unroll
        for (uint32_t u = 0; u < kPer; ++u) {
            const uint32_t j = min(threadIdx.x + u * kBinThreads, total - 1u);
            sj[u] = slice_of[j];
            const uint4 t = staged[j];
            e[u] = u32x4_t{t.x, t.y, t.z, t.w};
        }
#pragma unroll
        for (uint32_t u = 0; u < kPer; ++u) asm volatile("" : "+v"(sj[u]));
#pragma unroll
        for (uint32_t u = 0; u < kPer; ++u) {
            ro[u] = roff[sj[u]];
            ba[u] = base[sj[u]];
        }
#pragma unroll
        for (uint32_t u = 0; u < kPer; ++u) asm volatile("" : "+v"(ro[u]), "+v"(ba[u]), "+v"(e[u]));
#pragma unroll
        for (uint32_t u = 0; u < kPer; ++u) {
            const uint32_t j = threadIdx.x + u * kBinThreads;
            if (j < total) __builtin_nontemporal_store(e[u], reinterpret_cast<u32x4_t *>(queue + ro[u] + (j - ba[u])));
        }
    }
    gb = wave_max_u32(gb);
    if (lane == 0 && gb) atomicMax(&wg_max, gb);
    __syncthreads();
    if (threadIdx.x == 0) pl.chunk_max[(size_t)level * pl.n_chunks + chunk] = wg_max;
    ENT_STAMP(7);
}

#ifdef NSIG_ENT_TIMING
NSIG_EXPORT int level_entries_phase_ticks(unsigned long long *out144, int reset) {
    if (hipMemcpyFromSymbol(out144, HIP_SYMBOL(g_ent_phase), sizeof(unsigned long long) * 144) != hipSuccess) return 1;
    if (reset) {
        unsigned long long zero[144] = {};
        if (hipMemcpyToSymbol(HIP_SYMBOL(g_ent_phase), zero, sizeof(zero)) != hipSuccess) return 1;
    }
    return 0;
}
#endif

__device__ inline long long to_fixed(float c, int k) { return __double2ll_rn(ldexp((double)c, k)); }

__device__ inline int fixed_scale(uint32_t gmax_bits, uint32_t n) {
    int E;
    frexpf(__uint_as_float(gmax_bits), &E);
    return n > 2048u ? 62 - E - (32 - __builtin_clz(n)) : 51 - E;
}

__device__ inline void adam_update(float g, float &p, float &m, float &v, float beta1, float beta2, float eps, float step_size, float inv_bc2_sqrt) {
    m = m + (1.0f - beta1) * (g - m);
    v = v * beta2 + ((1.0f - beta2) * g) * g;
    const float denom = sqrtf(v) * inv_bc2_sqrt + eps;
    p = p - step_size * (m / denom);
}

constexpr int kOwnerAdamMax = 32;
struct OwnerAdam {
    float *p[NSIG_BASE_LEVELS], *m[NSIG_BASE_LEVELS], *v[NSIG_BASE_LEVELS];
    const float *scratch;
    float beta1, beta2, eps, grad_scale;
    uint32_t on;
};

__global__ void __launch_bounds__(1024) k_scatter_binned(const BinHeader *__restrict__ hd_all, const uint4 *__restrict__ queue_all, uint32_t M,
                                                         ScatterTargets tg, uint32_t replicas,
                                                         const uint32_t *__restrict__ set_max = nullptr, uint32_t n_set_max = 0, OwnerAdam adam = OwnerAdam{},
                                                         unsigned long long *__restrict__ slabs = nullptr) {
    extern __shared__ unsigned long long acc64[];
    const BinHeader *__restrict__ hd = hd_all + blockIdx.y;
    const uint4 *__restrict__ queue = queue_all + (size_t)blockIdx.y * 4 * M;
    float *__restrict__ G = tg.g[blockIdx.y];
    const uint32_t slice = blockIdx.x / replicas, replica = blockIdx.x - slice * replicas;
    static_assert(kBinSlices == 64, "one slice count per lane");
    const uint32_t lane = threadIdx.x & 63u, cnt = hd->counts[lane];
    uint32_t before = lane < slice ? cnt : 0u;
#pragma unroll
    for (int d = 32; d >= 1; d >>= 1) before += (uint32_t)__shfl_xor((int)before, d, 64);
    const uint32_t start = (uint32_t)__builtin_amdgcn_readfirstlane((int)before);
    const uint32_t n = (uint32_t)__builtin_amdgcn_readfirstlane(__shfl((int)cnt, (int)slice, 64)), chunk = ceil_div(n, replicas);
    const uint32_t beg = min(n, replica * chunk), end = min(n, beg + chunk);
    constexpr int kAhead = 4;
    typedef uint32_t u32x4_t __attribute__((ext_vector_type(4)));
    const u32x4_t *__restrict__ q = reinterpret_cast<const u32x4_t *>(queue + start);
    const uint32_t round = blockDim.x * kAhead;
    u32x4_t cur[kAhead] = {}, nxt[kAhead];
    if (beg < end) {
#pragma unroll
        for (int u = 0; u < kAhead; ++u) cur[u] = __builtin_nontemporal_load(q + min(beg + u * blockDim.x + threadIdx.x, end - 1));
    }
    uint32_t gb = hd->gmax_bits, mx = 0;
    __shared__ uint32_t smax;
    if (set_max != nullptr) {
        for (uint32_t i = threadIdx.x; i < n_set_max; i += blockDim.x) mx = max(mx, set_max[(size_t)blockIdx.y * n_set_max + i]);
        if (threadIdx.x == 0) smax = 0;
    }
    if (beg < end || adam.on)
        for (uint32_t i = threadIdx.x; i < 2u * kBinRows; i += blockDim.x) acc64[i] = 0ull;
    __syncthreads();
    if (set_max != nullptr) {
#pragma unroll
        for (int d = 32; d >= 1; d >>= 1) mx = max(mx, (uint32_t)__shfl_xor((int)mx, d, 64));
        if (lane == 0 && mx) atomicMax(&smax, mx);
        __syncthreads();
        gb = smax;
    }
    const bool poisoned = gb >= 0x7f800000u;
    const int k = poisoned ? 0 : fixed_scale(gb, n);
    float *out = G + 2 * (size_t)slice * kBinRows;
    if (beg >= end && !adam.on) {
        if (poisoned || replicas == 1) {
            const float f = poisoned ? __uint_as_float(0x7fc00000u) : 0.0f;
            for (uint32_t i4 = threadIdx.x; i4 < kBinRows / 2u; i4 += blockDim.x) *reinterpret_cast<float4 *>(out + 4u * i4) = make_float4(f, f, f, f);
        }
        return;
    }
    if (beg < end) {
        for (uint32_t base = beg; base < end; base += round) {
#pragma unroll
            for (int u = 0; u < kAhead; ++u) nxt[u] = __builtin_nontemporal_load(q + min(base + round + u * blockDim.x + threadIdx.x, end - 1));
            __builtin_amdgcn_sched_barrier(0);
#pragma unroll
            for (int u = 0; u < kAhead; ++u) {
                if (base + u * blockDim.x + threadIdx.x < end) {
                    const uint32_t ix = cur[u][0] & 0xffffu, hyz = cur[u][0] >> 16;
                    const float wx = __uint_as_float(cur[u][1]), a0 = __uint_as_float(cur[u][2]), a1 = __uint_as_float(cur[u][3]);
                    unsigned long long *d0 = acc64 + 2u * ((ix ^ hyz) & (kBinRows - 1)), *d1 = acc64 + 2u * (((ix + 1u) ^ hyz) & (kBinRows - 1));
                    if (wx != 1.0f) {
                        atomicAdd(d0, (unsigned long long)to_fixed(a0 * (1.0f - wx), k));
                        atomicAdd(d0 + 1, (unsigned long long)to_fixed(a1 * (1.0f - wx), k));
                    }
                    if (wx != 0.0f) {
                        atomicAdd(d1, (unsigned long long)to_fixed(a0 * wx, k));
                        atomicAdd(d1 + 1, (unsigned long long)to_fixed(a1 * wx, k));
                    }
                }
            }
#pragma unroll
            for (int u = 0; u < kAhead; ++u) cur[u] = nxt[u];
        }
    }
    __syncthreads();
    if (adam.on) {
        constexpr uint32_t kTrips = kBinRows / 2u / 1024u;
        typedef float f32x4_t __attribute__((ext_vector_type(4)));
        const size_t first = (size_t)slice * (kBinRows / 2u);
        f32x4_t *pp = reinterpret_cast<f32x4_t *>(adam.p[blockIdx.y]) + first, *pm = reinterpret_cast<f32x4_t *>(adam.m[blockIdx.y]) + first,
                *pv = reinterpret_cast<f32x4_t *>(adam.v[blockIdx.y]) + first;
        const float ss = adam.scratch[blockIdx.y], ib = adam.scratch[kOwnerAdamMax + blockIdx.y];
        f32x4_t p[kTrips], m[kTrips], v[kTrips];
#pragma unroll
        for (uint32_t u = 0; u < kTrips; ++u) {
            const uint32_t i4 = threadIdx.x + u * 1024u;
            p[u] = pp[i4];
            m[u] = __builtin_nontemporal_load(pm + i4);
            v[u] = __builtin_nontemporal_load(pv + i4);
        }
#pragma unroll
        for (uint32_t u = 0; u < kTrips; ++u) {
            const uint32_t i4 = threadIdx.x + u * 1024u;
#pragma unroll
            for (int c = 0; c < 4; ++c) {
                const long long a = (long long)acc64[4u * i4 + c];
                const float g = (poisoned ? __uint_as_float(0x7fc00000u) : (a != 0 ? (float)ldexp((double)a, -k) : 0.0f)) * adam.grad_scale;
                float pe = p[u][c], me = m[u][c], ve = v[u][c];
                adam_update(g, pe, me, ve, adam.beta1, adam.beta2, adam.eps, ss, ib);
                p[u][c] = pe; m[u][c] = me; v[u][c] = ve;
            }
            pp[i4] = p[u];
            __builtin_nontemporal_store(m[u], pm + i4);
            __builtin_nontemporal_store(v[u], pv + i4);
        }
        return;
    }
    if (poisoned || replicas == 1) {
        for (uint32_t i4 = threadIdx.x; i4 < kBinRows / 2u; i4 += blockDim.x) {
            float r[4];
#pragma unroll
            for (int c = 0; c < 4; ++c) {
                const long long v = (long long)acc64[4u * i4 + c];
                r[c] = poisoned ? __uint_as_float(0x7fc00000u) : (v != 0 ? (float)ldexp((double)v, -k) : 0.0f);
            }
            *reinterpret_cast<float4 *>(out + 4u * i4) = make_float4(r[0], r[1], r[2], r[3]);
        }
    } else {
        typedef unsigned long long u64x2_t __attribute__((ext_vector_type(2)));
        constexpr uint32_t kSlab = 2u * kBinRows;
        u64x2_t *mine = reinterpret_cast<u64x2_t *>(slabs + ((size_t)blockIdx.y * kBinSlices * replicas + (size_t)slice * replicas + replica) * kSlab);
        for (uint32_t i2 = threadIdx.x; i2 < kBinRows; i2 += blockDim.x) mine[i2] = *reinterpret_cast<const u64x2_t *>(acc64 + 2u * i2);
    }
}

constexpr uint32_t kMergeParts = 4, kMergeThreads = 1024;
__global__ void __launch_bounds__(kMergeThreads) k_scatter_merge(const BinHeader *__restrict__ hd_all, ScatterTargets tg, uint32_t replicas,
                                                                 const unsigned long long *__restrict__ slabs) {
    constexpr uint32_t kSlab = 2u * kBinRows, kPartWords = kSlab / kMergeParts, kTrips = kPartWords / kMergeThreads;
    static_assert(kPartWords % kMergeThreads == 0, "whole trips");
    const BinHeader *__restrict__ hd = hd_all + blockIdx.y;
    const uint32_t slice = blockIdx.x / kMergeParts, part = blockIdx.x - slice * kMergeParts;
    const uint32_t n = hd->counts[slice], gb = hd->gmax_bits;
    if (n == 0 || gb >= 0x7f800000u) return;
    const int k = fixed_scale(gb, n);
    const uint32_t chunk = ceil_div(n, replicas);
    const unsigned long long *slice_slabs = slabs + ((size_t)blockIdx.y * kBinSlices + slice) * replicas * kSlab + (size_t)part * kPartWords;
    unsigned long long sum[kTrips];
#pragma unroll
    for (uint32_t u = 0; u < kTrips; ++u) sum[u] = 0ull;
    for (uint32_t r = 0; r < replicas; ++r) {
        if (min(n, r * chunk) >= n) break;
        unsigned long long got[kTrips];
#pragma unroll
        for (uint32_t u = 0; u < kTrips; ++u) got[u] = __builtin_nontemporal_load(slice_slabs + (size_t)r * kSlab + threadIdx.x + u * kMergeThreads);
#pragma unroll
        for (uint32_t u = 0; u < kTrips; ++u) sum[u] += got[u];
    }
    float *out = tg.g[blockIdx.y] + 2 * (size_t)slice * kBinRows + (size_t)part * kPartWords;
#pragma unroll
    for (uint32_t u = 0; u < kTrips; ++u) {
        const long long v = (long long)sum[u];
        if (v != 0) atomicAdd(out + threadIdx.x + u * kMergeThreads, (float)ldexp((double)v, -k));
    }
}

__global__ void __launch_bounds__(256) k_level_records(const float *__restrict__ xyzs, float bound, const float2 *__restrict__ dplanes, uint32_t M,
                                                       uint32_t stride, LevelGeom geom, uint4 *__restrict__ rec) {
    const uint32_t m = blockIdx.x * 256 + threadIdx.x, level = blockIdx.y;
    if (m >= M) return;
    const float2 g = dplanes[(size_t)level * stride + m];
    const float two_b = 2.0f * bound, cell = geom.cell[level];
    uint32_t idx[3];
    float w[3];
#pragma unroll
    for (int a = 0; a < 3; ++a) axis_cell((xyzs[3 * (size_t)m + a] + bound) / two_b, cell, idx[a], w[a]);
    uint4 *r4 = rec + 2 * ((size_t)level * M + m);
    r4[0] = make_uint4(idx[0] | (idx[1] << 16), idx[2], __float_as_uint(w[0]), __float_as_uint(w[1]));
    r4[1] = make_uint4(__float_as_uint(w[2]), __float_as_uint(g.x), __float_as_uint(g.y), 0u);
}

__global__ void __launch_bounds__(256) k_fanout(const float4 *__restrict__ G, GradPtrs grads, uint32_t D, int accumulate) {
    const uint32_t e = blockIdx.x * blockDim.x + threadIdx.x;
    if (e >= NSIG_TABLE_ROWS / 2) return;
    const float4 g = G[e];
    for (uint32_t i = 0; i < D; ++i) {
        float4 *dst = reinterpret_cast<float4 *>(grads.p[i]) + e;
        if (accumulate) {
            float4 v = *dst;
            v.x += g.x; v.y += g.y; v.z += g.z; v.w += g.w;
            *dst = v;
        } else *dst = g;
    }
}

__global__ void __launch_bounds__(256) k_level_lookup(const float *__restrict__ x01, uint32_t M, float cell, int32_t *__restrict__ rows,
                                                      float *__restrict__ weights) {
    const uint32_t m = blockIdx.x * blockDim.x + threadIdx.x;
    if (m >= M) return;
    Corner8 c;
    corner_rows(x01[3 * (size_t)m], x01[3 * (size_t)m + 1], x01[3 * (size_t)m + 2], cell, c);
#pragma unroll
    for (int k = 0; k < 8; ++k) rows[8 * (size_t)m + k] = (int32_t)c.row[k];
    weights[3 * (size_t)m] = c.wx; weights[3 * (size_t)m + 1] = c.wy; weights[3 * (size_t)m + 2] = c.wz;
}

struct AdamPtrs {
    float *p[NSIG_MAX_MESSAGE_DIM];
    float *m[NSIG_MAX_MESSAGE_DIM];
    float *v[NSIG_MAX_MESSAGE_DIM];
    float step_size[NSIG_MAX_MESSAGE_DIM];
    float inv_bc2_sqrt[NSIG_MAX_MESSAGE_DIM];
};

__global__ void __launch_bounds__(256) k_codebook_adam(const float4 *__restrict__ G, AdamPtrs a, uint32_t D, float beta1, float beta2, float eps,
                                                       float grad_scale) {
    const uint32_t e = blockIdx.x * blockDim.x + threadIdx.x;
    if (e >= NSIG_TABLE_ROWS / 2) return;
    float4 g = G[e];
    g.x *= grad_scale; g.y *= grad_scale; g.z *= grad_scale; g.w *= grad_scale;
    for (uint32_t i = 0; i < D; ++i) {
        float4 *pp = reinterpret_cast<float4 *>(a.p[i]) + e, *pm = reinterpret_cast<float4 *>(a.m[i]) + e, *pv = reinterpret_cast<float4 *>(a.v[i]) + e;
        float4 p = *pp, m = *pm, v = *pv;
        const float ss = a.step_size[i], ib = a.inv_bc2_sqrt[i];
        adam_update(g.x, p.x, m.x, v.x, beta1, beta2, eps, ss, ib);
        adam_update(g.y, p.y, m.y, v.y, beta1, beta2, eps, ss, ib);
        adam_update(g.z, p.z, m.z, v.z, beta1, beta2, eps, ss, ib);
        adam_update(g.w, p.w, m.w, v.w, beta1, beta2, eps, ss, ib);
        *pp = p; *pm = m; *pv = v;
    }
}


struct PairPtrs {
    const float *p[2 * NSIG_MAX_MESSAGE_DIM];
};

__global__ void __launch_bounds__(256) k_codebook_presum_sel(PairPtrs tabs, const float *__restrict__ message, uint32_t D, float4 *__restrict__ S) {
    __shared__ const float4 *sel[NSIG_MAX_MESSAGE_DIM];
    if (threadIdx.x < D) sel[threadIdx.x] = reinterpret_cast<const float4 *>(tabs.p[2 * threadIdx.x + (message[threadIdx.x] != 0.0f)]);
    __syncthreads();
    const uint32_t e = blockIdx.x * blockDim.x + threadIdx.x;
    if (e >= NSIG_TABLE_ROWS / 2) return;
    float4 acc = {0.f, 0.f, 0.f, 0.f};
    uint32_t i = 0;
    for (; i + 8 <= D; i += 8) {
        float4 t[8];
#pragma unroll
        for (int u = 0; u < 8; ++u) t[u] = sel[i + u][e];
#pragma unroll
        for (int u = 0; u < 8; ++u) {
            acc.x += t[u].x; acc.y += t[u].y; acc.z += t[u].z; acc.w += t[u].w;
        }
    }
    for (; i < D; ++i) {
        const float4 a = sel[i][e];
        acc.x += a.x; acc.y += a.y; acc.z += a.z; acc.w += a.w;
    }
    S[e] = acc;
}

struct AdamPairPtrs {
    float *p[2 * NSIG_MAX_MESSAGE_DIM];
    float *m[2 * NSIG_MAX_MESSAGE_DIM];
    float *v[2 * NSIG_MAX_MESSAGE_DIM];
};
struct StepPtrs {
    float *s[2 * NSIG_MAX_MESSAGE_DIM];
};

__global__ void k_adam_prepare(StepPtrs steps, const float *__restrict__ message, uint32_t D, const float *__restrict__ lr, float beta1, float beta2,
                               float *__restrict__ scratch) {
    const uint32_t i = threadIdx.x;
    if (i >= D) return;
    float *sp = steps.s[2 * i + (message[i] != 0.0f)];
    const float step = *sp + 1.0f;
    *sp = step;
    scratch[i] = (float)((double)*lr / (1.0 - exp((double)step * log((double)beta1))));
    scratch[D + i] = (float)(1.0 / sqrt(1.0 - exp((double)step * log((double)beta2))));
}

typedef float nsig_f32x4 __attribute__((ext_vector_type(4)));
template <bool NT>
__device__ __forceinline__ float4 ld4(const float4 *p) {
    if (!NT) return *p;
    const nsig_f32x4 v = __builtin_nontemporal_load(reinterpret_cast<const nsig_f32x4 *>(p));
    return make_float4(v.x, v.y, v.z, v.w);
}
template <bool NT>
__device__ __forceinline__ void st4(float4 *p, const float4 &a) {
    if (!NT) {
        *p = a;
        return;
    }
    const nsig_f32x4 v = {a.x, a.y, a.z, a.w};
    __builtin_nontemporal_store(v, reinterpret_cast<nsig_f32x4 *>(p));
// ... 250 lines not shown
    const float step = *a.step[i] + 1.0f;
    *a.step[i] = step;
    scratch[i] = (float)((double)*lr / (1.0 - exp((double)step * log((double)beta1))));
    scratch[kDenseMax + i] = (float)(1.0 / sqrt(1.0 - exp((double)step * log((double)beta2))));
}

__global__ void __launch_bounds__(256) k_adam_dense(DenseAdam a, uint32_t n, const float *__restrict__ scratch, float beta1, float beta2, float eps,
                                                    float grad_scale) {
    uint32_t i = 0;
    while (i + 1 < n && blockIdx.x >= a.chunk0[i + 1]) ++i;
    const uint32_t base = (blockIdx.x - a.chunk0[i]) * kDenseChunk;
    const float ss = scratch[a.slot[i]], ib = scratch[kDenseMax + a.slot[i]];
    float *__restrict__ pp = a.p[i], *__restrict__ pm = a.m[i], *__restrict__ pv = a.v[i];
    const float *__restrict__ pg = a.g[i];
#pragma unroll
    for (int u = 0; u < 4; ++u) {
        const uint32_t e = base + u * 256 + threadIdx.x;
        if (e < a.numel[i]) {
            float p = pp[e], m = pm[e], v = pv[e];
            adam_update(pg[e] * grad_scale, p, m, v, beta1, beta2, eps, ss, ib);
            pp[e] = p; pm[e] = m; pv[e] = v;
        }
    }
}

struct DenseScalars {
    float ss[kDenseMax], ib[kDenseMax];
};
__global__ void __launch_bounds__(256) k_adam_dense_host(DenseAdam a, uint32_t n, DenseScalars sc, float beta1, float beta2, float eps, float grad_scale) {
    uint32_t i = 0;
    while (i + 1 < n && blockIdx.x >= a.chunk0[i + 1]) ++i;
    const uint32_t base = (blockIdx.x - a.chunk0[i]) * kDenseChunk;
    const float ss = sc.ss[i], ib = sc.ib[i];
    float *__restrict__ pp = a.p[i], *__restrict__ pm = a.m[i], *__restrict__ pv = a.v[i];
    const float *__restrict__ pg = a.g[i];
#pragma unroll
    for (int u = 0; u < 4; ++u) {
        const uint32_t e = base + u * 256 + threadIdx.x;
        if (e < a.numel[i]) {
            float p = pp[e], m = pm[e], v = pv[e];
            adam_update(pg[e] * grad_scale, p, m, v, beta1, beta2, eps, ss, ib);
            pp[e] = p; pm[e] = m; pv[e] = v;
        }
    }
}

NSIG_EXPORT int opt_adam_dense_host(uint32_t n, float *const *params_host, const float *const *grads_host, float *const *exp_avg_host,
                                    float *const *exp_avg_sq_host, const uint32_t *numel_host, const float *step_sizes_host, const float *inv_bc2_host,
                                    float beta1, float beta2, float eps, float grad_scale, nsig_stream_t stream) {
    NSIG_REQUIRE(params_host && grads_host && exp_avg_host && exp_avg_sq_host && numel_host && step_sizes_host && inv_bc2_host, "opt_adam_dense_host: null pointer");
    hipStream_t st = as_stream(stream);
    for (uint32_t first = 0; first < n; first += kDenseMax) {
        const uint32_t cnt = n - first < (uint32_t)kDenseMax ? n - first : (uint32_t)kDenseMax;
        DenseAdam a{};
        DenseScalars sc{};
        uint32_t chunks = 0;
        for (uint32_t i = 0; i < cnt; ++i) {
            const uint32_t j = first + i;
            NSIG_REQUIRE(params_host[j] && grads_host[j] && exp_avg_host[j] && exp_avg_sq_host[j] && numel_host[j] > 0,
                         "opt_adam_dense_host: tensor %u has a null pointer or no elements", j);
            a.p[i] = params_host[j]; a.g[i] = grads_host[j]; a.m[i] = exp_avg_host[j]; a.v[i] = exp_avg_sq_host[j];
            a.numel[i] = numel_host[j];
            a.chunk0[i] = chunks;
            chunks += ceil_div(numel_host[j], kDenseChunk);
            sc.ss[i] = step_sizes_host[j];
            sc.ib[i] = inv_bc2_host[j];
        }
        a.chunk0[cnt] = chunks;
        k_adam_dense_host<<<chunks, 256, 0, st>>>(a, cnt, sc, beta1, beta2, eps, grad_scale);
        if (int e = check_launch("opt_adam_dense_host")) return e;
    }
    return NSIG_OK;
}

constexpr uint32_t kDenseChunk4 = 4096, kDenseBigNumel = 1u << 16, kDenseRideAlong = 1024;
__global__ void __launch_bounds__(256) k_adam_dense_v4(DenseAdam a, uint32_t n, const float *__restrict__ scratch, float beta1, float beta2, float eps,
                                                       float grad_scale) {
    uint32_t i = 0;
    while (i + 1 < n && blockIdx.x >= a.chunk0[i + 1]) ++i;
    const uint32_t base = (blockIdx.x - a.chunk0[i]) * (kDenseChunk4 / 4), n4 = a.numel[i] / 4;
    const float ss = scratch[a.slot[i]], ib = scratch[kDenseMax + a.slot[i]];
    float4 *__restrict__ pp = reinterpret_cast<float4 *>(a.p[i]), *__restrict__ pm = reinterpret_cast<float4 *>(a.m[i]), *__restrict__ pv = reinterpret_cast<float4 *>(a.v[i]);
    const float4 *__restrict__ pg = reinterpret_cast<const float4 *>(a.g[i]);
    float4 p[4], m[4], v[4], g[4];
#pragma unroll
    for (int u = 0; u < 4; ++u) {
        const uint32_t e = min(base + u * 256u + threadIdx.x, n4 - 1u);
        p[u] = ld4<true>(pp + e); m[u] = ld4<true>(pm + e); v[u] = ld4<true>(pv + e); g[u] = ld4<true>(pg + e);
    }
#pragma unroll
    for (int u = 0; u < 4; ++u) {
        const uint32_t e = base + u * 256u + threadIdx.x;
        if (e >= n4) break;
        adam_update(g[u].x * grad_scale, p[u].x, m[u].x, v[u].x, beta1, beta2, eps, ss, ib);
        adam_update(g[u].y * grad_scale, p[u].y, m[u].y, v[u].y, beta1, beta2, eps, ss, ib);
        adam_update(g[u].z * grad_scale, p[u].z, m[u].z, v[u].z, beta1, beta2, eps, ss, ib);
        adam_update(g[u].w * grad_scale, p[u].w, m[u].w, v[u].w, beta1, beta2, eps, ss, ib);
        st4<false>(pp + e, p[u]); st4<true>(pm + e, m[u]); st4<true>(pv + e, v[u]);
    }
}

NSIG_EXPORT int opt_adam_dense(uint32_t n, float *const *params_host, const float *const *grads_host, float *const *exp_avg_host,
                               float *const *exp_avg_sq_host, float *const *steps_host, const uint32_t *numel_host, const float *lr, float beta1,
                               float beta2, float eps, float grad_scale, float *scratch, nsig_stream_t stream) {
    NSIG_REQUIRE(params_host && grads_host && exp_avg_host && exp_avg_sq_host && steps_host && numel_host && lr && scratch, "opt_adam_dense: null pointer");
    hipStream_t st = as_stream(stream);
    for (uint32_t first = 0; first < n; first += kDenseMax) {
        const uint32_t cnt = n - first < (uint32_t)kDenseMax ? n - first : (uint32_t)kDenseMax;
        DenseAdam all{}, small{}, big{};
        uint32_t n_small = 0, n_big = 0, chunks_small = 0, chunks_big = 0;
        auto vectorisable = [&](uint32_t j) {
            return numel_host[j] % 4 == 0 && aligned16(params_host[j]) && aligned16(grads_host[j]) && aligned16(exp_avg_host[j]) && aligned16(exp_avg_sq_host[j]);
        };
        bool any_big = false;
        for (uint32_t i = 0; i < cnt; ++i) any_big = any_big || (numel_host[first + i] >= kDenseBigNumel && vectorisable(first + i));
        for (uint32_t i = 0; i < cnt; ++i) {
            const uint32_t j = first + i;
            NSIG_REQUIRE(params_host[j] && grads_host[j] && exp_avg_host[j] && exp_avg_sq_host[j] && steps_host[j] && numel_host[j] > 0,
                         "opt_adam_dense: tensor %u has a null pointer or no elements", j);
            all.step[i] = steps_host[j];
            const bool wide = numel_host[j] >= (any_big ? kDenseRideAlong : kDenseBigNumel) && vectorisable(j);
            DenseAdam &d = wide ? big : small;
            uint32_t &k = wide ? n_big : n_small, &chunks = wide ? chunks_big : chunks_small;
            d.p[k] = params_host[j]; d.g[k] = grads_host[j]; d.m[k] = exp_avg_host[j]; d.v[k] = exp_avg_sq_host[j];
            d.numel[k] = numel_host[j];
            d.slot[k] = (uint8_t)i;
            d.chunk0[k] = chunks;
            chunks += ceil_div(numel_host[j], wide ? kDenseChunk4 : kDenseChunk);
            ++k;
        }
        small.chunk0[n_small] = chunks_small;
        big.chunk0[n_big] = chunks_big;
        float *sc = scratch + (size_t)first * 2;
        k_adam_dense_prepare<<<1, kDenseMax, 0, st>>>(all, cnt, lr, beta1, beta2, sc);
        if (int e = check_launch("opt_adam_dense (prepare)")) return e;
        if (n_big) {
            k_adam_dense_v4<<<chunks_big, 256, 0, st>>>(big, n_big, sc, beta1, beta2, eps, grad_scale);
            if (int e = check_launch("opt_adam_dense (wide)")) return e;
        }
        if (n_small) {
            k_adam_dense<<<chunks_small, 256, 0, st>>>(small, n_small, sc, beta1, beta2, eps, grad_scale);
            if (int e = check_launch("opt_adam_dense")) return e;
        }
    }
    return NSIG_OK;
}

static size_t binned_scratch_bytes(uint32_t M, uint32_t sets) { return (size_t)sets * (sizeof(BinHeader) + (size_t)4 * M * sizeof(uint4)); }

static int reserve_owner_lds(const char *who) {
    static bool attr_set = false;
    const size_t lds = (size_t)kBinRows * 2 * sizeof(unsigned long long);
    if (!attr_set) {
        if (hipFuncSetAttribute(reinterpret_cast<const void *>(k_scatter_binned), hipFuncAttributeMaxDynamicSharedMemorySize, (int)lds) != hipSuccess) {
            set_error("%s: cannot reserve %zu bytes of LDS", who, lds);
            return NSIG_ERR_LAUNCH;
        }
        attr_set = true;
    }
    return NSIG_OK;
}

static int owner_targets_aligned(const ScatterTargets &tg, uint32_t sets, const char *who) {
    for (uint32_t i = 0; i < sets; ++i) NSIG_REQUIRE(aligned16(tg.g[i]), "%s: gradient table %u must be 16-byte aligned", who, i);
    return NSIG_OK;
}

static int launch_binned(const float *rec, uint32_t M, uint32_t sets, const ScatterTargets &tg, uint32_t replicas, void *scratch, hipStream_t st,
                         const char *who) {
    static_assert(sizeof(BinHeader) % 16 == 0 && kBinGrid == 16 * 16, "the queues follow the headers 16-byte aligned; k_bin_scan walks 16 x 16 workgroups");
    BinHeader *hd = reinterpret_cast<BinHeader *>(scratch);
    uint4 *queue = reinterpret_cast<uint4 *>(hd + sets);
    for (uint32_t i = 0; i < sets; ++i)
        if (hipMemsetAsync(&hd[i].gmax_bits, 0, sizeof(uint32_t), st) != hipSuccess) {
            set_error("%s: hipMemsetAsync failed", who);
            return NSIG_ERR_LAUNCH;
        }
    const size_t lds = (size_t)kBinRows * 2 * sizeof(unsigned long long);
    if (int e = reserve_owner_lds(who)) return e;
    if (int e = owner_targets_aligned(tg, sets, who)) return e;
    const uint32_t blocks = ceil_div(M, kBinThreads) < kBinGrid ? ceil_div(M, kBinThreads) : kBinGrid;
    k_bin_count<<<dim3(blocks, sets), kBinThreads, 0, st>>>(rec, M, hd);
    k_bin_scan<<<sets, 1024, 0, st>>>(hd, blocks);
    k_bin_write<<<dim3(blocks, sets), kBinThreads, 0, st>>>(rec, M, hd, queue);
    unsigned long long *slabs = replicas > 1 ? reinterpret_cast<unsigned long long *>(queue + (size_t)sets * 4 * M) : nullptr;
    k_scatter_binned<<<dim3(kBinSlices * replicas, sets), 1024, lds, st>>>(hd, queue, M, tg, replicas, nullptr, 0u, OwnerAdam{}, slabs);
    if (replicas > 1) k_scatter_merge<<<dim3(kBinSlices * kMergeParts, sets), kMergeThreads, 0, st>>>(hd, tg, replicas, slabs);
    return check_launch(who);
}

NSIG_EXPORT size_t hg_scatter_binned_scratch_bytes(uint32_t M) { return binned_scratch_bytes(M, 1) + scatter_merge_bytes(kBinReplicas); }

NSIG_EXPORT int hg_scatter_binned(const float *rec, uint32_t M, float *G, void *scratch, nsig_stream_t stream) {
    if (M == 0) return NSIG_OK;
    NSIG_REQUIRE(rec && G && scratch, "hg_scatter_binned: null pointer");
    NSIG_REQUIRE((reinterpret_cast<uintptr_t>(rec) & 15) == 0 && (reinterpret_cast<uintptr_t>(scratch) & 15) == 0 && M < (1u << 28),
                 "hg_scatter_binned: rec and scratch must be 16-byte aligned and M < 2^28");
    ScatterTargets tg{};
    tg.g[0] = G;
    return launch_binned(rec, M, 1, tg, kBinReplicas, scratch, as_stream(stream), "hg_scatter_binned");
}

NSIG_EXPORT size_t hg_scatter_plan_bytes(uint32_t M) { return scatter_plan_bytes(M); }

NSIG_EXPORT int hg_scatter_plan(const float *xyzs, uint32_t M, float bound, void *plan, nsig_stream_t stream) {
    if (M == 0) return NSIG_OK;
    NSIG_REQUIRE(xyzs && plan, "hg_scatter_plan: null pointer");
    NSIG_REQUIRE((reinterpret_cast<uintptr_t>(plan) & 15) == 0 && M < (1u << 28) && bound > 0.0f, "hg_scatter_plan: plan must be 16-byte aligned, M < 2^28, bound > 0");
    const ScatterPlan pl = scatter_plan_view(plan, M);
    hipStream_t st = as_stream(stream);
    const uint32_t blocks = ceil_div(M, kBinThreads) < kBinGrid ? ceil_div(M, kBinThreads) : kBinGrid;
    k_plan_count<<<blocks, kBinThreads, 0, st>>>(xyzs, M, bound, pl.hd);
    k_plan_dest<<<blocks, kBinThreads, 0, st>>>(xyzs, M, bound, pl.hd, pl.dest);
    return check_launch("hg_scatter_plan");
}

NSIG_EXPORT int hg_scatter_planned(const void *plan, uint32_t M, float *G, nsig_stream_t stream) {
    if (M == 0) return NSIG_OK;
    NSIG_REQUIRE(plan && G, "hg_scatter_planned: null pointer");
    NSIG_REQUIRE((reinterpret_cast<uintptr_t>(plan) & 15) == 0 && M < (1u << 28), "hg_scatter_planned: plan must be 16-byte aligned and M < 2^28");
    if (int e = reserve_owner_lds("hg_scatter_planned")) return e;
    const ScatterPlan pl = scatter_plan_view(const_cast<void *>(plan), M);
    ScatterTargets tg{};
    tg.g[0] = G;
    if (int e = owner_targets_aligned(tg, 1, "hg_scatter_planned")) return e;
    k_scatter_binned<<<dim3(kBinSlices * kBinReplicas, 1), 1024, (size_t)kBinRows * 2 * sizeof(unsigned long long), as_stream(stream)>>>(pl.hd, pl.queue, M, tg,
                                                                                                                                           kBinReplicas, nullptr, 0u,
                                                                                                                                           OwnerAdam{}, pl.slabs);
    k_scatter_merge<<<dim3(kBinSlices * kMergeParts, 1), kMergeThreads, 0, as_stream(stream)>>>(pl.hd, tg, kBinReplicas, pl.slabs);
    return check_launch("hg_scatter_planned");
}

NSIG_EXPORT size_t hg_scatter_levels_scratch_bytes(uint32_t M) {
    return (size_t)NSIG_BASE_LEVELS * M * 32 + binned_scratch_bytes(M, NSIG_BASE_LEVELS);
}

NSIG_EXPORT int hg_scatter_levels(const float *xyzs, float bound, const void *d_planes, uint32_t M, uint32_t stride, float *const *G_host,
                                  void *scratch, nsig_stream_t stream) {
    NSIG_REQUIRE(xyzs && d_planes && G_host && scratch, "hg_scatter_levels: null pointer");
    NSIG_REQUIRE(bound > 0.0f && stride >= M && M < (1u << 28), "hg_scatter_levels: bad bound, stride < M or M >= 2^28");
    NSIG_REQUIRE((reinterpret_cast<uintptr_t>(scratch) & 15) == 0, "hg_scatter_levels: scratch must be 16-byte aligned");
    ScatterTargets tg{};
    for (int l = 0; l < NSIG_BASE_LEVELS; ++l) {
        NSIG_REQUIRE(G_host[l], "hg_scatter_levels: table %d has a null pointer", l);
        tg.g[l] = G_host[l];
    }
    hipStream_t st = as_stream(stream);
    if (M == 0) {
        for (int l = 0; l < NSIG_BASE_LEVELS; ++l)
            if (hipMemsetAsync(tg.g[l], 0, (size_t)NSIG_TABLE_ROWS * 2 * sizeof(float), st) != hipSuccess) {
                set_error("hg_scatter_levels: hipMemsetAsync failed");
                return NSIG_ERR_LAUNCH;
            }
        return NSIG_OK;
    }
    uint4 *rec = reinterpret_cast<uint4 *>(scratch);
    k_level_records<<<dim3(ceil_div(M, 256u), NSIG_BASE_LEVELS), 256, 0, st>>>(xyzs, bound, reinterpret_cast<const float2 *>(d_planes), M, stride,
                                                                              make_level_geom(), rec);
    if (int e = check_launch("hg_scatter_levels (records)")) return e;
    return launch_binned(reinterpret_cast<const float *>(rec), M, NSIG_BASE_LEVELS, tg, 1u,
                         reinterpret_cast<char *>(scratch) + (size_t)NSIG_BASE_LEVELS * M * 32, st, "hg_scatter_levels");
}

NSIG_EXPORT size_t hg_levels_plan_bytes(uint32_t M) { return levels_plan_bytes(M); }

NSIG_EXPORT int hg_levels_plan(const float *xyzs, uint32_t M, const uint32_t *rows_dev, float bound, void *plan, nsig_stream_t stream) {
    if (M == 0) return NSIG_OK;
    NSIG_REQUIRE(xyzs && plan, "hg_levels_plan: null pointer");
    NSIG_REQUIRE((reinterpret_cast<uintptr_t>(plan) & 15) == 0 && M < (1u << 27) && bound > 0.0f, "hg_levels_plan: plan must be 16-byte aligned, M < 2^27, bound > 0");
    const LevelsPlan pl = levels_plan_view(plan, M);
    hipStream_t st = as_stream(stream);
    k_levels_count<<<dim3(pl.n_chunks, NSIG_BASE_LEVELS), kBinThreads, 0, st>>>(xyzs, M, rows_dev, bound, make_level_geom(), pl);
    k_levels_scan<<<NSIG_BASE_LEVELS, kBinThreads, 0, st>>>(M, rows_dev, pl);
    return check_launch("hg_levels_plan");
}

template <typename Prepare>
static int levels_scatter_launch(const char *who, const float *xyzs, uint32_t M, const uint32_t *rows_dev, float bound, const void *d_planes, uint32_t stride, void *plan,
                                 const ScatterTargets &tg, const OwnerAdam &adam, hipStream_t st, Prepare prepare) {
    NSIG_REQUIRE(xyzs && d_planes && plan, "%s: null pointer", who);
    NSIG_REQUIRE((reinterpret_cast<uintptr_t>(plan) & 15) == 0 && (reinterpret_cast<uintptr_t>(d_planes) & 7) == 0 && M < (1u << 27) && bound > 0.0f && stride >= M,
                 "%s: plan must be 16-byte and d_planes 8-byte aligned, M < 2^27, bound > 0, stride >= M", who);
    if (!adam.on)
        if (int e = owner_targets_aligned(tg, NSIG_BASE_LEVELS, who)) return e;
    if (int e = reserve_owner_lds(who)) return e;
    const size_t staging = (size_t)kLevelStage * sizeof(uint4);
    static bool attr_set = false;
    if (!attr_set) {
        if (hipFuncSetAttribute(reinterpret_cast<const void *>(k_level_entries), hipFuncAttributeMaxDynamicSharedMemorySize, (int)staging) != hipSuccess) {
            set_error("%s: cannot reserve %zu bytes of LDS", who, staging);
            return NSIG_ERR_LAUNCH;
        }
        attr_set = true;
    }
    const LevelsPlan pl = levels_plan_view(plan, M);
    k_level_entries<<<dim3(pl.n_chunks, NSIG_BASE_LEVELS), kBinThreads, staging, st>>>(xyzs, M, rows_dev, bound, reinterpret_cast<const float2 *>(d_planes), stride,
                                                                                     make_level_geom(), pl);
    if (int e = check_launch(who)) return e;
    if (int e = prepare()) return e;
    const uint32_t M_stride = M * (kLevelQueueStride / 4);
#ifdef NSIG_LEVELS_SPLIT
    for (int l = 0; l < NSIG_BASE_LEVELS; ++l) {
        ScatterTargets one{};
        one.g[0] = tg.g[l];
        k_scatter_binned<<<dim3(kBinSlices, 1), 1024, (size_t)kBinRows * 2 * sizeof(unsigned long long), st>>>(pl.hd + l, pl.queue + (size_t)l * kLevelQueueStride * M,
                                                                                                               M_stride, one, 1u, pl.chunk_max + (size_t)l * pl.n_chunks, pl.n_chunks);
    }
#else
    k_scatter_binned<<<dim3(kBinSlices, NSIG_BASE_LEVELS), 1024, (size_t)kBinRows * 2 * sizeof(unsigned long long), st>>>(pl.hd, pl.queue, M_stride, tg, 1u,
                                                                                                                          pl.chunk_max, pl.n_chunks, adam);
#endif
    return check_launch(who);
}

NSIG_EXPORT int hg_levels_scatter(const float *xyzs, uint32_t M, const uint32_t *rows_dev, float bound, const void *d_planes, uint32_t stride, void *plan,
                                  float *const *G_host, nsig_stream_t stream) {
    NSIG_REQUIRE(G_host, "hg_levels_scatter: null pointer");
    ScatterTargets tg{};
    for (int l = 0; l < NSIG_BASE_LEVELS; ++l) {
        NSIG_REQUIRE(G_host[l], "hg_levels_scatter: table %d has a null pointer", l);
        tg.g[l] = G_host[l];
    }
    hipStream_t st = as_stream(stream);
    if (M == 0) {
        for (int l = 0; l < NSIG_BASE_LEVELS; ++l)
            if (hipMemsetAsync(tg.g[l], 0, (size_t)NSIG_TABLE_ROWS * 2 * sizeof(float), st) != hipSuccess) {
                set_error("hg_levels_scatter: hipMemsetAsync failed");
                return NSIG_ERR_LAUNCH;
            }
        return NSIG_OK;
    }
    return levels_scatter_launch("hg_levels_scatter", xyzs, M, rows_dev, bound, d_planes, stride, plan, tg, OwnerAdam{}, st, []() { return (int)NSIG_OK; });
}

NSIG_EXPORT int hg_levels_scatter_adam(const float *xyzs, uint32_t M, const uint32_t *rows_dev, float bound, const void *d_planes, uint32_t stride, void *plan,
                                       float *const *params_host, float *const *exp_avg_host, float *const *exp_avg_sq_host, float *const *steps_host, const float *lr,
                                       float beta1, float beta2, float eps, float grad_scale, float *scratch, nsig_stream_t stream) {
    NSIG_REQUIRE(params_host && exp_avg_host && exp_avg_sq_host && steps_host && lr && scratch, "hg_levels_scatter_adam: null pointer");
    NSIG_REQUIRE(M >= 1, "hg_levels_scatter_adam: M must be positive (a step without points still runs the owners: the device row count may be zero)");
    NSIG_REQUIRE(xyzs && d_planes && plan, "hg_levels_scatter_adam: null pointer");
    NSIG_REQUIRE((reinterpret_cast<uintptr_t>(plan) & 15) == 0 && (reinterpret_cast<uintptr_t>(d_planes) & 7) == 0 && M < (1u << 27) && bound > 0.0f && stride >= M,
                 "hg_levels_scatter_adam: plan must be 16-byte and d_planes 8-byte aligned, M < 2^27, bound > 0, stride >= M");
    static_assert(kOwnerAdamMax == kDenseMax, "k_adam_dense_prepare's scratch layout");
    OwnerAdam adam{};
    DenseAdam all{};
    for (int l = 0; l < NSIG_BASE_LEVELS; ++l) {
        NSIG_REQUIRE(params_host[l] && exp_avg_host[l] && exp_avg_sq_host[l] && steps_host[l], "hg_levels_scatter_adam: table %d has a null pointer", l);
        NSIG_REQUIRE(aligned16(params_host[l]) && aligned16(exp_avg_host[l]) && aligned16(exp_avg_sq_host[l]), "hg_levels_scatter_adam: table %d must be 16-byte aligned", l);
        adam.p[l] = params_host[l]; adam.m[l] = exp_avg_host[l]; adam.v[l] = exp_avg_sq_host[l];
        all.step[l] = steps_host[l];
    }
    adam.scratch = scratch;
    adam.beta1 = beta1; adam.beta2 = beta2; adam.eps = eps; adam.grad_scale = grad_scale;
    adam.on = 1u;
    hipStream_t st = as_stream(stream);
    return levels_scatter_launch("hg_levels_scatter_adam", xyzs, M, rows_dev, bound, d_planes, stride, plan, ScatterTargets{}, adam, st, [&]() {
        k_adam_dense_prepare<<<1, kDenseMax, 0, st>>>(all, NSIG_BASE_LEVELS, lr, beta1, beta2, scratch);
        return check_launch("hg_levels_scatter_adam (prepare)");
    });
}

NSIG_EXPORT int hg_scatter_level(const float *xyzs, float bound, const void *d_plane, uint32_t M, uint32_t level, float *G, nsig_stream_t stream) {
    if (M == 0) return NSIG_OK;
    NSIG_REQUIRE(xyzs && d_plane && G, "hg_scatter_level: null pointer");
    NSIG_REQUIRE(level < NSIG_BASE_LEVELS && bound > 0.0f, "hg_scatter_level: level %u out of range or bad bound", level);
    static bool attr_set = false;
    const size_t lds = (size_t)kSliceRows * 2 * sizeof(float);
    if (!attr_set) {
        if (hipFuncSetAttribute(reinterpret_cast<const void *>(k_scatter_level), hipFuncAttributeMaxDynamicSharedMemorySize, (int)lds) != hipSuccess) {
            set_error("hg_scatter_level: cannot reserve %zu bytes of LDS", lds);
            return NSIG_ERR_LAUNCH;
        }
        attr_set = true;
    }
    k_scatter_level<<<kSlices * kReplicas, 1024, lds, as_stream(stream)>>>(xyzs, bound, reinterpret_cast<const float2 *>(d_plane), M,
                                                                         1.0f / kBaseResolution[level], G);
    return check_launch("hg_scatter_level");
}
```

nerf_signature_amd/fieldops.py:

```python
import os

import torch
from torch.autograd import Function
from torch.amp import custom_bwd, custom_fwd

from . import _native as nv

T_ROWS = 1 << 19
MASK_WORDS = 6

_fwd32 = custom_fwd(device_type="cuda", cast_inputs=torch.float32)
_bwd = custom_bwd(device_type="cuda")


def message_bits(message):
    if message is None:
        return None
    if isinstance(message, torch.Tensor):
        return tuple(int(v) for v in message.detach().to("cpu", torch.float32).tolist())
    return tuple(int(v) for v in message)


def select_tables(tables, bits):
    if len(tables) != 2 * len(bits):
# ... 129 lines not shown


def field_backward(xyzs, bound, g_sigma, g_rgb, sigmas, rgbs, masks, packed, G=None, want_dfeat=False, want_rec=False):
    xyzs = xyzs.contiguous().float()
    M = xyzs.shape[0]
    dfeat = torch.empty(M, 2, dtype=torch.float32, device=xyzs.device) if want_dfeat else None
    rec = torch.empty(M, 8, dtype=torch.float32, device=xyzs.device) if want_rec else None
    nv.call("field_bwd", nv.ptr(xyzs), M, float(bound), nv.ptr(g_sigma.contiguous().float()), nv.ptr(g_rgb.contiguous().float()),
            nv.ptr(sigmas), nv.ptr(rgbs), nv.ptr(masks), nv.ptr(packed), nv.ptr(G), nv.ptr(dfeat), nv.ptr(rec), nv.stream())
    if want_dfeat and want_rec:
        return dfeat, rec
    return rec if want_rec else dfeat


BINNED_MIN_POINTS = 65536


def binned_min_points():
    from .switches import deterministic
    return 1 if deterministic() else BINNED_MIN_POINTS


def codebook_scatter_sliced(rec, G, binned=None):
    M = rec.shape[0]
    if (M >= binned_min_points()) if binned is None else binned:
        scratch = torch.empty(int(nv.fn("hg_scatter_binned_scratch_bytes")(M)), dtype=torch.uint8, device=rec.device)
        nv.call("hg_scatter_binned", nv.ptr(rec), M, nv.ptr(G), nv.ptr(scratch), nv.stream())
    else:
        nv.call("hg_scatter_sliced", nv.ptr(rec), M, nv.ptr(G), nv.stream())
    return G


_PLAN_STREAM = None
_PENDING_PLANS = []
_LIVE_PLANS = []


def set_plan_stream(stream):
    global _PLAN_STREAM
    prev, _PLAN_STREAM = _PLAN_STREAM, stream
    return prev


def flush_plans():
    while _PENDING_PLANS:
        _PENDING_PLANS.pop(0).launch()


def forget_plan_events():
    alive = []
    for ref in _LIVE_PLANS:
        plan = ref()
        if plan is not None:
            if plan.launched:
                plan.ready = None
            alive.append(ref)
    _LIVE_PLANS[:] = alive


class ScatterPlan:

    def __init__(self, xyzs, bound):
        self.M, self.xyzs, self.bound = xyzs.shape[0], xyzs, float(bound)
        self.buf = torch.empty(int(nv.fn("hg_scatter_plan_bytes")(self.M)), dtype=torch.uint8, device=xyzs.device)
        self.stream, self.ready, self.launched = _PLAN_STREAM, None, False
        self.src_ready = None
        if self.stream is not None and self.stream == torch.cuda.current_stream():
            self.stream = None
        if self.stream is None:
            self.launch()
        else:
            if self.stream != torch.cuda.current_stream():
                self.src_ready = torch.cuda.Event()
                self.src_ready.record()
            _PENDING_PLANS.append(self)

    def launch(self):
        if self.launched:
            return
        self.launched = True
        if self.stream is None:
            nv.call("hg_scatter_plan", nv.ptr(self.xyzs), self.M, self.bound, nv.ptr(self.buf), nv.stream())
        else:
            if self.src_ready is not None:
                self.stream.wait_event(self.src_ready)
            nv.call("hg_scatter_plan", nv.ptr(self.xyzs), self.M, self.bound, nv.ptr(self.buf), self.stream.cuda_stream)
            self.xyzs.record_stream(self.stream)
            self.buf.record_stream(self.stream)
            self.ready = torch.cuda.Event()
            self.ready.record(self.stream)
            import weakref
            _LIVE_PLANS.append(weakref.ref(self))
        self.xyzs = None

    def join(self):
        if not self.launched:
            if self in _PENDING_PLANS:
                _PENDING_PLANS.remove(self)
            self.stream = None
            self.launch()
        elif self.ready is not None:
            if self.stream is None or torch.cuda.current_stream() != self.stream:
                torch.cuda.current_stream().wait_event(self.ready)
            self.ready = None


class _KeptPlan:

    def __init__(self, M, buf):
        self.M, self.buf, self.launched, self.ready = M, buf, True, None

    def join(self):
        pass


class FixedPoints:

    def __init__(self, xyzs, bound, base_tables):
        self.M, self.bound = int(xyzs.shape[0]), float(bound)
        self.xyzs_ptr = xyzs.data_ptr()
        self.planes = torch.empty(int(nv.fn("hg_planes_bytes")(self.M)), dtype=torch.uint8, device=xyzs.device)
        self.plan = _KeptPlan(self.M, torch.empty(int(nv.fn("hg_scatter_plan_bytes")(self.M)), dtype=torch.uint8, device=xyzs.device))
        self.refreshes = 0
        self.refresh(xyzs, base_tables)

    @staticmethod
    def _tables_key(base_tables):
        return tuple((t.data_ptr(), t._version) for t in base_tables) + (mixed_planes(),)

    def refresh(self, xyzs, base_tables):
        if xyzs.data_ptr() != self.xyzs_ptr or xyzs.shape[0] != self.M:
            raise ValueError("FixedPoints.refresh: these are not the points the cache was built for")
        base_ptrs = nv.ptr_array([_check_table(t.detach(), "base table") for t in base_tables])
        self.layout = encode_planes(xyzs, self.M, self.bound, base_ptrs, None, self.planes)
        nv.call("hg_scatter_plan", nv.ptr(xyzs), self.M, self.bound, nv.ptr(self.plan.buf), nv.stream())
        self.key = self._tables_key(base_tables)
        self.refreshes += 1

    def check(self, xyzs, bound, base_tables):
        if xyzs.data_ptr() != self.xyzs_ptr or xyzs.shape[0] != self.M or float(bound) != self.bound:
            raise ValueError("FixedPoints: the field pass was handed other points than the cache was built for")
        if self._tables_key(base_tables) != self.key and not torch.cuda.is_current_stream_capturing():
            self.refresh(xyzs, base_tables)


def field_backward_planned(xyzs, bound, g_sigma, g_rgb, sigmas, rgbs, masks, packed, plan, G):
    plan.join()
    nv.call("field_bwd_planned", nv.ptr(xyzs), plan.M, float(bound), nv.ptr(g_sigma.contiguous().float()), nv.ptr(g_rgb.contiguous().float()),
            nv.ptr(sigmas), nv.ptr(rgbs), nv.ptr(masks), nv.ptr(packed), nv.ptr(plan.buf), nv.stream())
    nv.call("hg_scatter_planned", nv.ptr(plan.buf), plan.M, nv.ptr(G), nv.stream())
    return G


def field_backward_into(xyzs, bound, g_sigma, g_rgb, sigmas, rgbs, masks, packed, G, plan=None):
    if plan is not None:
        return field_backward_planned(xyzs, bound, g_sigma, g_rgb, sigmas, rgbs, masks, packed, plan, G)
    rec = field_backward(xyzs, bound, g_sigma, g_rgb, sigmas, rgbs, masks, packed, want_rec=True)
    return codebook_scatter_sliced(rec, G)


class GradSink:

    def __init__(self, device, tail=0):
        self.arena = torch.zeros(T_ROWS * 2 + tail, dtype=torch.float32, device=device)
        self.G = self.arena[:T_ROWS * 2].view(T_ROWS, 2)
        self.tail = self.arena[T_ROWS * 2:]
        self.selected = None

    def zero_(self):
        self.G.zero_()
        self.selected = None

    def fanout(self, accumulate=False):
        if self.selected is None:
            return
        slab = torch.empty(len(self.selected), T_ROWS, 2, dtype=torch.float32, device=self.G.device)
        grads = [slab[i] for i in range(len(self.selected))]
        fanout_grad(self.G, grads)
        for p, g in zip(self.selected, grads):
            p.grad = g if (p.grad is None or not accumulate) else p.grad + g


class SharedGradient(GradSink):

    def __init__(self, device):
        super().__init__(device)
        self.carrier = None
        self.live = None
        from .switches import dropin_off
        self.dense_takeover = not dropin_off("dense_adam")

    def pending(self):
        return self.carrier is not None and self.carrier.grad is self.G

    def begin_accumulation(self, selected):
        if self.pending():
            if len(selected) == len(self.live) and all(a is b for a, b in zip(selected, self.live)):
                return
            self.dissolve()
        self.G.zero_()
        self.live = list(selected)
        self.carrier = selected[0]
        if self.carrier.grad is not None:
            self.G.add_(self.carrier.grad)
        self.carrier.grad = self.G

    def dissolve(self):
        if not self.pending():
            self.carrier = self.live = None
            return
        slab = torch.empty(len(self.live), T_ROWS, 2, dtype=torch.float32, device=self.G.device)
        grads = [slab[i] for i in range(len(self.live))]
        fanout_grad(self.G, grads)
        for p, g in zip(self.live, grads):
            p.grad = g if (p.grad is None or p.grad is self.G) else p.grad + g
        self.carrier = self.live = None

    def consumed(self):
        if self.carrier is not None and self.carrier.grad is self.G:
            self.carrier.grad = None
        self.carrier = self.live = None


class _Tables:
    __slots__ = ("base", "sel")

    def __init__(self, base, sel):
        self.base, self.sel = list(base), list(sel)


class _FieldFunction(Function):

    @staticmethod
    @_fwd32
    def forward(ctx, xyzs, dirs, bound, packed, S, sink, tabs, fixed, *diff):
        base, sel = tabs.base, tabs.sel
        n_sel = len(sel)
        need_grad = n_sel > 0 and len(diff) > 0
        xyzs = xyzs.contiguous().float()
        if fixed is not None:
            ctx.plan = fixed.plan if need_grad else None
        else:
            ctx.plan = ScatterPlan(xyzs, bound) if need_grad and xyzs.shape[0] >= binned_min_points() else None
        sigmas, rgbs, _, masks = field_forward(xyzs, dirs, bound, base, S, packed, want_masks=need_grad, fixed=fixed)
        ctx.bound, ctx.n_diff, ctx.need_grad, ctx.sink = bound, len(diff), need_grad, sink
        if need_grad:
            ctx.mlp_precision = nv.fn("mlp_get_precision")()
            ctx.save_for_backward(xyzs, sigmas, rgbs, masks, packed)
            if sink is not None:
                sink.selected = list(sel)
                ctx.sink_selected = sink.selected
        return sigmas, rgbs

    @staticmethod
    @_bwd
    def backward(ctx, g_sigma, g_rgb):
        head = (None,) * 8
        if not ctx.need_grad:
            return head + (None,) * ctx.n_diff
        xyzs, sigmas, rgbs, masks, packed = ctx.saved_tensors
        plan, ctx.plan = ctx.plan, None
        if nv.fn("mlp_get_precision")() != ctx.mlp_precision:
            raise RuntimeError("mlp_set_precision was called between a field forward pass and its backward: the saved ReLU masks belong to the forward's "
                               "arithmetic (run the backward before switching, or switch before the forward)")
        if ctx.sink is not None:
            if isinstance(ctx.sink, SharedGradient):
                ctx.sink.begin_accumulation(ctx.sink_selected)
            field_backward_into(xyzs, ctx.bound, g_sigma, g_rgb, sigmas, rgbs, masks, packed, ctx.sink.G, plan)
            return head + (None,) * ctx.n_diff
        G = torch.zeros(T_ROWS, 2, dtype=torch.float32, device=xyzs.device)
        field_backward_into(xyzs, ctx.bound, g_sigma, g_rgb, sigmas, rgbs, masks, packed, G, plan)
        slab = torch.empty(ctx.n_diff, T_ROWS, 2, dtype=torch.float32, device=xyzs.device)
        grads = [slab[i] for i in range(ctx.n_diff)]
        fanout_grad(G, grads, accumulate=False)
        return head + tuple(grads)



_SH4 = None


def sh4_basis(d):
    global _SH4
    if _SH4 is None or _SH4.device != d.device:
        c1, c2a, c2b, c2c = 0.4886025119029199, 1.0925484305920792, 0.31539156525252005, 0.5462742152960396
        c3a, c3b, c3c, c3d, c3e = 0.5900435899266435, 2.890611442640554, 0.4570457994644658, 0.3731763325901154, 1.445305721320277
        names = ["1", "x", "y", "z", "xy", "yz", "xz", "xx", "yy", "zz", "xxx", "xyy", "xzz", "yxx", "yyy", "yzz", "zxx", "zyy", "zzz", "xyz"]
        rows = {n: i for i, n in enumerate(names)}
        terms = [{"1": 0.28209479177387814}, {"y": -c1}, {"z": c1}, {"x": -c1},
                 {"xy": c2a}, {"yz": -c2a}, {"zz": 2 * c2b, "xx": -c2b, "yy": -c2b}, {"xz": -c2a}, {"xx": c2c, "yy": -c2c},
                 {"yxx": -3 * c3a, "yyy": c3a}, {"xyz": c3b}, {"yzz": -4 * c3c, "yxx": c3c, "yyy": c3c}, {"zzz": 2 * c3d, "zxx": -3 * c3d, "zyy": -3 * c3d},
                 {"xzz": -4 * c3c, "xxx": c3c, "xyy": c3c}, {"zxx": c3e, "zyy": -c3e}, {"xxx": -c3a, "xyy": 3 * c3a}]
        C = torch.zeros(20, 16, dtype=torch.float64)
        for k, t in enumerate(terms):
            for n, v in t.items():
                C[rows[n], k] = v
        _SH4 = C.float().to(d.device)
    x, y, z = d.unbind(-1)
    xx, yy, zz = x * x, y * y, z * z
    mono = torch.stack([torch.ones_like(x), x, y, z, x * y, y * z, x * z, xx, yy, zz, x * xx, x * yy, x * zz, y * xx, y * yy, y * zz, z * xx, z * yy, z * zz, x * y * z], dim=-1)
    return mono @ _SH4


class _DensityFunction(Function):

    @staticmethod
    @_fwd32
    def forward(ctx, xyzs, bound, packed, S, sink, tabs, sigma_params, *diff):
        xyzs = xyzs.contiguous().float()
        sigmas, _, geo, _ = field_forward(xyzs, None, bound, tabs.base, S, packed, want_rgb=False, want_geo=True)
        ctx.bound, ctx.n_diff, ctx.sink, ctx.tabs, ctx.S = float(bound), len(diff), sink, tabs, S
        ctx.save_for_backward(xyzs, sigmas, sigma_params.detach())
        if sink is not None:
            sink.selected = list(tabs.sel)
            ctx.sink_selected = sink.selected
        return sigmas, geo

    @staticmethod
    @_bwd
    def backward(ctx, g_sigma, g_geo):
        head = (None,) * 7
        xyzs, sigmas, params = ctx.saved_tensors
        M, dev = xyzs.shape[0], xyzs.device
        W1, W2 = params[:2048].view(64, 32), params[2048:3072].view(16, 64)
        x01 = (xyzs + ctx.bound) / (2 * ctx.bound)
        feat = encode(x01, ctx.tabs.base, ctx.S)
        pre = feat @ W1.t()
        d_so = torch.zeros(M, 16, dtype=torch.float32, device=dev)
        if g_sigma is not None:
            d_so[:, 0] = g_sigma.float() * sigmas.clamp(min=3.059023205018258e-07, max=3269017.3724721107)
        if g_geo is not None:
            d_so[:, 1:] = g_geo.float()
        dfeat = (((d_so @ W2) * (pre > 0)) @ W1)[:, 30:32].contiguous()
        if ctx.sink is not None:
            if isinstance(ctx.sink, SharedGradient):
                ctx.sink.begin_accumulation(ctx.sink_selected)
            codebook_scatter(x01, dfeat, ctx.sink.G)
            return head + (None,) * ctx.n_diff
        G = torch.zeros(T_ROWS, 2, dtype=torch.float32, device=dev)
        codebook_scatter(x01, dfeat, G)
        slab = torch.empty(ctx.n_diff, T_ROWS, 2, dtype=torch.float32, device=dev)
        grads = [slab[i] for i in range(ctx.n_diff)]
        fanout_grad(G, grads, accumulate=False)
        return head + tuple(grads)


def density_apply(xyzs, bound, packed, base_tables, selected, S, sink, sigma_params):
    if sink is None:
        diff = tuple(selected) if any(t.requires_grad for t in selected) else ()
    else:
        diff = next(((t,) for t in selected if t.requires_grad), ())
    return _DensityFunction.apply(xyzs, bound, packed, S, sink, _Tables(base_tables, selected), sigma_params, *diff)


class _ColorFunction(Function):

    @staticmethod
    @_fwd32
    def forward(ctx, dirs, geo_feat, packed, color_params):
        rgbs = field_color(dirs, geo_feat, packed)
        ctx.save_for_backward(dirs.contiguous().float(), geo_feat.contiguous().float(), rgbs, color_params.detach())
        return rgbs

    @staticmethod
    @_bwd
    def backward(ctx, g_rgb):
        dirs, geo, rgbs, params = ctx.saved_tensors
        Wc1, Wc2, Wc3 = params[:2048].view(64, 32), params[2048:6144].view(64, 64), params[6144:7168].view(16, 64)
        cin = torch.cat([sh4_basis(((dirs + 1) / 2) * 2 - 1), geo, torch.ones_like(geo[:, :1])], dim=-1)
        p1 = cin @ Wc1.t()
        p2 = torch.relu(p1) @ Wc2.t()
        d_out = torch.zeros(dirs.shape[0], 16, dtype=torch.float32, device=dirs.device)
        d_out[:, :3] = g_rgb.float() * rgbs * (1 - rgbs)
        d_cin = (((d_out @ Wc3) * (p2 > 0)) @ Wc2 * (p1 > 0)) @ Wc1
        return None, d_cin[:, 16:31].contiguous(), None, None


def color_apply(dirs, geo_feat, packed, color_params):
    return _ColorFunction.apply(dirs, geo_feat, packed, color_params)


def field_apply(xyzs, dirs, bound, packed, base_tables, selected, S=None, sink=None, fixed=None):
    if len(selected) and S is None:
        S = codebook_presum(selected)
    if not torch.is_grad_enabled():
        diff = ()
    elif sink is None:
        diff = tuple(selected) if any(t.requires_grad for t in selected) else ()
    else:
        diff = next(((t,) for t in selected if t.requires_grad), ())
    return _FieldFunction.apply(xyzs, dirs, bound, packed, S, sink, _Tables(base_tables, selected), fixed, *diff)
```

nerf_signature_amd/trainer.py:

```python
import ctypes
import os

import numpy as np
import torch
import torch.nn.functional as F

from . import _native as nv
from . import fieldops as fo
from . import dp
from .capture import SegmentedCapture, warm_up
from .dp import GradExchange, exchange_active, world_size
from .distortion import DistortionLayer, host_uniform, scaled_width
from .hidden_models import normalize_img, set_grad_arena, set_weights_stream


def loss_w_bce(decoded, keys, temp=10.0):
    return F.binary_cross_entropy_with_logits(decoded * temp, keys, reduction="mean")


def loss_w_mse(decoded, keys, temp=10.0):
    return torch.mean((decoded * temp - (2 * keys - 1)) ** 2)


class _WatermarkLoss(torch.autograd.Function):
# ... 197 lines not shown
            layer = self.__dict__["_nsig_distortion_layer"] = DistortionLayer(kind)
        o = data["watermark"]["rays_o_block"]
        layer.draw(tuple(o.shape), o.device)
    name = getattr(self.opt, "loss_w", "bce")
    if name not in ("bce", "mse"):
        raise NotImplementedError
    graph = self.__dict__.get("_nsig_block_graph")
    if graph is None:
        from .blockgraph import StepGraph
        graph = self.__dict__["_nsig_block_graph"] = StepGraph()
    return train_step(self.model, data, message, vars(self.opt), lambda_w=self.lambda_w, lambda_i=self.lambda_i, loss_w=loss_w_bce if name == "bce" else loss_w_mse,
                      color_space=getattr(self.opt, "color_space", "srgb"), distortion=layer, block_graph=graph)


def eval_step(model, data, message, render_kwargs, render_whole=True, lambda_w=1.0, lambda_i=1.0, loss_w=loss_w_bce, color_space="srgb", distortion=None):
    dev = message.device
    decoded, gt_rgb = None, None
    lossi, lossw, loss = (torch.zeros(1, device=dev) for _ in range(3))
    kw = dict(render_kwargs)
    if not render_whole:
        out = model.render(data["rays_o_block"], data["rays_d_block"], message, staged=False, bg_color=1, perturb=False, force_all_rays=True, **kw)
        pred_rgb, pred_depth = torch.clamp(out["image"], min=0, max=1), out["depth"]
        if isinstance(distortion, str):
            distortion = DistortionLayer(distortion) if distortion != "none" else None
        pred_rgb_dist = pred_rgb
        if distortion is not None:
            distortion.draw(tuple(pred_rgb.shape), pred_rgb.device)
            pred_rgb_dist = distortion(pred_rgb)
        decoded = model.msg_decoder(model.normalization(pred_rgb_dist.permute(0, 3, 1, 2)))
        gt_rgb = data.get("images_block")
        if gt_rgb is not None:
            lossi = ((pred_rgb - gt_rgb) ** 2).mean()
        lossw = loss_w(decoded, message.to(decoded.device).unsqueeze(-1))
        loss = lambda_w * lossw + lambda_i * lossi
    else:
        B, H, W, C = data["images"].shape
        images = data["images"]
        if color_space == "linear":
            images[..., :3] = srgb_to_linear(images[..., :3])
        gt_rgb = images[..., :3] * images[..., 3:] + 1 * (1 - images[..., 3:]) if C == 4 else images
        out = model.render(data["rays_o"], data["rays_d"], message, staged=True, bg_color=1, perturb=False, force_all_rays=True, **kw)
        pred_rgb = torch.clamp(out["image"].reshape(-1, H, W, 3), min=0, max=1)
        pred_depth = out["depth"].reshape(-1, H, W)
    return pred_rgb, pred_depth, gt_rgb, decoded, lossi, lossw, loss


def test_step(model, data, message, render_kwargs, bg_color=None, perturb=False):
    H, W = data["H"], data["W"]
    out = model.render(data["rays_o"], data["rays_d"], message, staged=True, bg_color=bg_color, perturb=perturb, **dict(render_kwargs))
    return torch.clamp(out["image"].reshape(-1, H, W, 3), min=0, max=1), out["depth"].reshape(-1, H, W)


test_step.__test__ = False


class WatermarkLoop:

    def __init__(self, model, optimizer, render_kwargs, lambda_w=1.0, lambda_i=1.0, lr_scheduler=None, use_sink=True, side_stream=None, distortion="none",
                 distortion_seed=0):
        self.distortion = None if distortion in (None, "none") else (distortion if isinstance(distortion, DistortionLayer) else DistortionLayer(distortion, distortion_seed))
        self.side_stream = side_stream
        self.plan_stream = side_stream
        self.model, self.optimizer, self.lr_scheduler = model, optimizer, lr_scheduler
        self.render_kwargs = dict(render_kwargs)
        self.lambda_w, self.lambda_i = lambda_w, lambda_i
        dev = next(model.parameters()).device
        self.sink = fo.GradSink(dev) if use_sink else None
        model.grad_sink = self.sink
        self.exchange = GradExchange(list(model.msg_decoder.parameters()))
        self.last = None

    def _sharded(self, data):
        return local_blocks(data["watermark"])[2] is not None

    def step(self, data, message):
        if getattr(self.model, "device_select", False):
            raise RuntimeError("the model is in device-select mode (a GraphedWatermarkLoop prepared it): its sink records all 2D tables as "
                               "selected, which the eager optimiser step would update wrongly; call GraphedWatermarkLoop.close() first")
        self.optimizer.zero_grad(set_to_none=True)
        if self.sink is not None:
            self.sink.zero_()
        if self.distortion is not None:
            o = data["watermark"]["rays_o_block"]
            self.distortion.draw(tuple(o.shape), o.device)
        prev = fo.set_plan_stream(self.plan_stream)
        try:
            out = train_step(self.model, data, message, self.render_kwargs, self.lambda_w, self.lambda_i, side_stream=self.side_stream, distortion=self.distortion)
        finally:
            fo.set_plan_stream(prev)
        sharded = self._sharded(data)
        backward_from_loss_kernel(out, dp.content_grad_scale(sharded))
        if self.side_stream is not None:
            torch.cuda.current_stream().wait_stream(self.side_stream)
        if self.sink is None and exchange_active():
            raise RuntimeError("data-parallel steps need the GradSink route (use_sink=True): per-table gradients are not exchanged")
        self.exchange.shared_scale = 1.0 if sharded else None
        self.exchange(self.sink.G if self.sink is not None else None)
        if self.sink is not None and hasattr(self.optimizer, "step_shared"):
            self.optimizer.step_shared(self.sink.selected, self.sink.G)
        elif self.sink is not None:
            self.sink.fanout()
        self.optimizer.step()
        if self.lr_scheduler is not None:
            self.lr_scheduler.step()
        self.last = out
        return out


class BIT_ACC:

    def __init__(self, device=None):
        self.V, self.N, self.instant_V = 0, 0, 0

    def clear(self):
        self.V, self.N = 0, 0

    def update(self, preds, truths):
        diff = ~torch.logical_xor(preds > 0, truths > 0)
        acc = (torch.sum(diff, dim=-1) / diff.shape[-1]).item()
        self.instant_V = acc
        self.V += acc
        self.N += 1

    def measure(self):
        return self.V / self.N

    def report(self):
        return f"bit_acc = {self.measure():.6f}"


class PSNRMeter:

    def __init__(self):
        self.V, self.N = 0, 0

    def clear(self):
        self.V, self.N = 0, 0

    def update(self, preds, truths):
        p = preds.detach().cpu().numpy() if torch.is_tensor(preds) else preds
        t = truths.detach().cpu().numpy() if torch.is_tensor(truths) else truths
        self.V += -10 * np.log10(np.mean((p - t) ** 2))
        self.N += 1

    def measure(self):
        return self.V / self.N

    def report(self):
        return f"PSNR = {self.measure():.6f}"


class GraphedWatermarkLoop:

    def __init__(self, model, optimizer, render_kwargs, data, lambda_w=1.0, lambda_i=1.0, lr_lambda=None, headroom=0.0, overlap_content=True,
                 content_headroom=None, content_sampler=None, fixed_blocks=False, distortion="none", distortion_seed=0):
        self.distortion = None if distortion in (None, "none") else (distortion if isinstance(distortion, DistortionLayer) else DistortionLayer(distortion, distortion_seed))
        self.fixed_blocks = bool(fixed_blocks)
        self._refix_pending = False
        self._kept_key = None
        self.content_sampler = content_sampler
        self._s_for = None
        self.marched = None
        self._pending_content = None
        self.side_stream = torch.cuda.Stream() if overlap_content else None
        self.plan_stream = self.side_stream
        self.weights_stream = self.side_stream
        self.content_backward_first = False
        if not hasattr(optimizer, "step_shared_sel"):
            raise TypeError("GraphedWatermarkLoop needs nerf_signature_amd.optim.CodebookAdam(capturable=True)")
        if not any(t.requires_grad for t in model.msg_encoder.tables()):
            raise NotImplementedError("GraphedWatermarkLoop captures the step that trains the codebook; with a frozen codebook "
                                      "(finetune_decoder=True) drive the model with WatermarkLoop")
        self.model, self.optimizer = model, optimizer
        self.render_kwargs = dict(render_kwargs)
        self.lambda_w, self.lambda_i = lambda_w, lambda_i
        self.lr_lambda, self.headroom = lr_lambda, headroom
        self.content_headroom = headroom if content_headroom is None else content_headroom
        dev = next(model.parameters()).device
        self.device = dev
        self._warm_sink = torch.zeros(1, dtype=torch.float32, device=dev)
        D = model.message_dim
        self.sink = fo.GradSink(dev, tail=sum(p.numel() for p in model.msg_decoder.parameters()))
        model.grad_sink = self.sink
        self.exchange = GradExchange(list(model.msg_decoder.parameters()), average=False)
        self.data = {"watermark": {k: v.clone() for k, v in data["watermark"].items()},
                     "content": {k: v.clone() for k, v in data["content"].items()}}
        self.msg_all = torch.zeros(2 * D + 1, dtype=torch.float32, device=dev)
        self.msg_dev, self.msg_next_dev = self.msg_all[:D], self.msg_all[D:2 * D]
        self.stage_width = 2 * D + (1 if lr_lambda is not None else 0)
        self.msg_ring = torch.zeros(16, self.stage_width, dtype=torch.float32).pin_memory()
        self.msg_events = [None] * len(self.msg_ring)
        self.stage_counter = torch.zeros(1, dtype=torch.int32, device=dev)
        self.ring_dev = nv.fn("nsig_host_device_pointer")(ctypes.c_void_p(self.msg_ring.data_ptr()))
        self.stage_in_graph = bool(self.ring_dev)
        self.base_lr = float(optimizer.param_groups[0]["lr"])
        self.lr_dev = self.msg_all[2 * D]
        self.lr_dev.fill_(self.base_lr)
        for g in optimizer.param_groups:
            g["lr"] = self.lr_dev
        self.tables = model.msg_encoder.tables()
        self.selected = None
        self._capture_stream = None
        self.sharded = False
        self.opt_shard = None
        self.out = None
        self.steps_done = 0
        self._replays = 0
        self.capacity_rows = None
        if not hasattr(model, "_graphed_loops"):
            model._graphed_loops = []
        model._graphed_loops.append(self)

    def resume_at(self, step):
        if self.selected is not None and self._replays:
            raise RuntimeError("resume_at: the loop has already replayed steps")
        self.steps_done = int(step)
        self._replays = int(step)
        self.stage_counter.fill_(int(step))

    def invalidate(self):
        self._s_for = None
        self.model._packed()
        if self.fixed_blocks and self.selected is not None:
            self._fix_blocks()

    @torch.no_grad()
    def gather_codebook(self, optimizer_state=True):
        if self.opt_shard is None:
            return
        import torch.distributed as dist
        from .optim import _prepare_device_state
        b0, b1 = self.opt_shard
        world = dist.get_world_size()
        _prepare_device_state(self.optimizer, self.tables)
        kinds = [lambda t: t.data]
        if optimizer_state:
            dp_state = self.optimizer.state
            kinds += [lambda t, k=k: dp_state[t][k] for k in ("exp_avg", "exp_avg_sq", "step") if all(k in dp_state[t] for t in self.tables)]
        for get in kinds:
            own = torch.stack([get(t).reshape(-1) for t in self.tables[2 * b0:2 * b1]])
            every = torch.empty((world,) + tuple(own.shape), dtype=own.dtype, device=own.device)
            dp._all_gather_into(every.view(world * own.shape[0], -1), own)
            for i, t in enumerate(self.tables):
                get(t).reshape(-1).copy_(every.view(len(self.tables), -1)[i])
        from .optim import _bump_versions
        _bump_versions(self.tables)
        self.model._codebook_stale = False

    def close(self):
        self.gather_codebook()
        self.model.codebook_shard = None
        self.model.device_select = False
        self.model.point_capacity = None
        if self in getattr(self.model, "_graphed_loops", ()):
            self.model._graphed_loops.remove(self)

    def _forward_backward(self):
        if self.stage_in_graph and torch.cuda.is_current_stream_capturing():
            nv.call("loop_step_begin", nv.ptr(self.sink.G), self.sink.G.numel(), ctypes.c_void_p(self.ring_dev), len(self.msg_ring),
                    self.stage_width, nv.ptr(self.stage_counter), nv.ptr(self.msg_all), nv.stream())
        else:
            self.sink.zero_()
            if self.content_sampler is not None and torch.cuda.is_current_stream_capturing():
                self.stage_counter += 1
        if self.content_sampler is not None:
            ct = self.data["content"]
            self.content_sampler.sample_into(self.stage_counter, ct["rays_o"], ct["rays_d"], ct["images"])
        if self.distortion is not None and self.distortion.name != "scaling":
            o = self.data["watermark"]["rays_o_block"]
            self.distortion.draw_on_device(self.stage_counter, tuple(o.shape), o.device)
        prev = fo.set_plan_stream(self.plan_stream)
        try:
            out = train_step(self.model, self.data, self.msg_dev, self.render_kwargs, self.lambda_w, self.lambda_i, side_stream=self.side_stream,
                             presum_first=self.marched is not None, presum_adopt=torch.cuda.is_current_stream_capturing(),
                             blocks_first=self.side_stream is not None and self._blocks_issued_first(),
                             content_backward_now=(self.lambda_i * dp.content_grad_scale(self.sharded)) if (self.content_backward_first and self.side_stream is not None) else None,
                             distortion=self.distortion)
        finally:
            fo.set_plan_stream(prev)
        set_weights_stream(self.weights_stream)
        set_grad_arena(self.sink.tail)
        try:
            backward_from_loss_kernel(out, dp.content_grad_scale(self.sharded), self.side_stream, self.content_backward_first)
        finally:
            set_weights_stream(None)
            set_grad_arena(None)
        join_stream(torch.cuda.current_stream(), self.side_stream)
        if self.weights_stream is not self.side_stream:
            join_stream(torch.cuda.current_stream(), self.weights_stream)
        return out

    def _optimise(self, defer_collective=False):
        scale = 1.0 / world_size()
        scale_cb = 1.0 if self.sharded else scale
        tables, msg, msg_next = self.tables, self.msg_dev, self.msg_next_dev
        if self.opt_shard is not None:
            b0, b1 = self.opt_shard
            tables, msg, msg_next = self.tables[2 * b0:2 * b1], self.msg_dev[b0:b1], self.msg_next_dev[b0:b1]
        S = self.model._presum_cache[1]
        self.optimizer.step_shared_sel(tables, msg, self.sink.G, self.lr_dev, scale_cb, next_message_dev=msg_next, S_next=S)
        self.optimizer.step_dense(self.lr_dev, scale)
        if self.opt_shard is None:
            return None
        import torch.distributed as dist
        post = lambda: dp.collective(lambda: dist.all_reduce(S, op=dist.ReduceOp.SUM), last=True, name="all_reduce_presum")
        if defer_collective:
            return post
        post()
        return None

    def _march_ahead(self):
        kw, wm = self.render_kwargs, self.data["watermark"]
        args = (kw.get("dt_gamma", 0), kw.get("max_steps", 1024))
        block_o, block_d, _ = local_blocks(wm)
        if self.fixed_blocks:
            self.marched = self.marched[:1]
        else:
            self.marched = (self.model.march_ahead(block_o, block_d, *args),)

    @torch.no_grad()
    def _fix_blocks(self):
        kw = self.render_kwargs
        block_o, block_d, _ = local_blocks(self.data["watermark"])
        rec = self.model.fix_rays(block_o, block_d, kw.get("dt_gamma", 0), kw.get("max_steps", 1024))
        self.marched = (rec,) + tuple(self.marched[1:] if self.marched else ())
        self._refix_pending = False
        self._kept_key = self._kept_inputs_key()

    def _optimise_and_march(self):
        if not self.march_ahead or self.fixed_blocks:
            return self._optimise()
        main = torch.cuda.current_stream()
        self.side_stream.wait_stream(main)
        with torch.cuda.stream(self.side_stream):
            self._march_ahead()
            self._warm_tables()
        post = self._optimise(defer_collective=True)
        main.wait_stream(self.side_stream)
        if post is not None:
            post()

    def _warm_tables(self):
        if self.opt_shard is not None or self.fixed_blocks or getattr(self.model, "_presum_cache", None) is None:
            return
        tables = nv.ptr_array([t.detach() for t in self.model.encoder.tables()])
        nv.call("hg_warm_tables", tables, nv.ptr(self.model._presum_cache[1]), nv.ptr(self._warm_sink), nv.stream())

    def point_counts(self):
        if self.marched is not None:
            return int(self.marched[0]["counter"][0]), int(self.model.step_counter[self.capacity_rows[-1], 0])
        a, b = self.model.step_counter[self.capacity_rows, 0].tolist()
        return (a, b) if self._blocks_issued_first() else (b, a)

    def _blocks_issued_first(self):
        return self.side_stream is None or self.content_backward_first

    def _kept_inputs_key(self):
        m = self.model
        return m.grid_key() + tuple((t.data_ptr(), t._version) for t in m.encoder.tables())

    def _set_inputs(self, message, data, next_data=None, next_message=None, eager_copy=True):
        if self.fixed_blocks and self.selected is not None and not self._refix_pending and self._kept_key != self._kept_inputs_key():
            self._refix_pending = True
        if self._refix_pending:
            self._fix_blocks()
        slot = self._replays % len(self.msg_ring)
        if self.msg_events[slot] is not None:
            self.msg_events[slot].synchronize()
        D = self.msg_dev.numel()
        self.msg_ring[slot][:D].copy_(message.detach().to("cpu", torch.float32))
        self.msg_ring[slot][D:2 * D].copy_((message if next_message is None else next_message).detach().to("cpu", torch.float32))
        if self.lr_lambda is not None:
            self.msg_ring[slot][2 * D] = self.base_lr * self.lr_lambda(self.steps_done)
        if eager_copy:
            self.msg_all[:self.stage_width].copy_(self.msg_ring[slot][:self.stage_width], non_blocking=True)
            ev = torch.cuda.Event()
            ev.record()
            self.msg_events[slot] = ev
        if self._pending_content is not None:
            for k, v in self._pending_content.items():
                self.data["content"][k].copy_(v, non_blocking=True)
            self._pending_content = None
        if data is not None:
            for part in ("watermark", "content"):
                for k, v in data.get(part, {}).items():
                    self.data[part][k].copy_(v, non_blocking=True)
            if self.fixed_blocks and self.selected is not None and "watermark" in data:
                self._fix_blocks()
            if self.march_ahead and self.selected is not None and "watermark" in data and not self.fixed_blocks:
                self._march_ahead()
        if next_data is not None:
            if not self.march_ahead:
                raise ValueError("next_data needs overlap_content=True (the march-ahead)")
            for k, v in next_data.get("watermark", {}).items():
                self.data["watermark"][k].copy_(v, non_blocking=True)
                self._refix_pending = self.fixed_blocks
            content = next_data.get("content")
            if content is not None:
                self._pending_content = content

    def prepare(self, message):
        model = self.model
        model.device_select = False
        model.point_capacity = None
        self.optimizer.zero_grad(set_to_none=True)
        self.sink.zero_()
        block_o, block_d, shard = local_blocks(self.data["watermark"])
        self.sharded = shard is not None
        self.exchange.shared_scale = 1.0 if self.sharded else None
        self.opt_shard = dp.optimizer_shard(model.message_dim) if self.sharded else None
        model.codebook_shard = self.opt_shard
        if self.distortion is not None and self.distortion.name == "scaling":
            o = self.data["watermark"]["rays_o_block"]
            self.distortion._buffers(tuple(o.shape), o.device)
            self.distortion.set_scaling(host_uniform(self.distortion.seed, self._replays, 0.75, 1.25))
        beside = self.side_stream is not None
        self.content_backward_first = beside
        self.weights_stream = self.side_stream if not beside else (getattr(self, "_own_weights_stream", None) or torch.cuda.Stream())
        self._own_weights_stream = self.weights_stream if beside else None
        with torch.no_grad():
            model.render(block_o, block_d, message, staged=False, bg_color=1,
                         perturb=False, force_all_rays=True, **self.render_kwargs)
            n_block = int(model.step_counter[(model.local_step - 1) % 16, 0])
            model.render(self.data["content"]["rays_o"], self.data["content"]["rays_d"], message, staged=False, bg_color=1, perturb=False,
                         force_all_rays=True, **self.render_kwargs)
            n_content = int(model.step_counter[(model.local_step - 1) % 16, 0])
        from .raymarching import padded_point_count
        rays_block = block_o.numel() // 3
        rays_content = self.data["content"]["rays_o"].numel() // 3
        if rays_block == rays_content:
            raise ValueError("block and content renders must have different ray counts to carry separate capacities")
        cap_block = padded_point_count(int(n_block * (1.0 + self.headroom)))
        cap_content = padded_point_count(int(n_content * (1.0 + self.content_headroom)))
        model.point_capacity = {rays_block: cap_block, rays_content: cap_content}
        model.device_select = True
        self._set_inputs(message, None)

        if self.fixed_blocks:
            if not self.march_ahead:
                raise ValueError("fixed_blocks needs overlap_content=True (the kept samples live in the march-ahead record)")
            self._fix_blocks()
        warm_up(self._warm_up_step, 3, self.optimizer, [p for g in self.optimizer.param_groups for p in g["params"] if p.requires_grad])

        self.variants = {}
        if self.distortion is not None and self.distortion.name == "scaling":
            W = self.data["watermark"]["rays_o_block"].shape[2]
            a_factor_of = {scaled_width(W, f): f for f in (0.75 + 0.5 * i / 4096.0 for i in range(4096))}
            for w in sorted(a_factor_of):
                self.distortion.set_scaling(a_factor_of[w])
                self.variants[w] = self._capture(cap_block, cap_content)
        else:
            self.variants[None] = self._capture(cap_block, cap_content)
        self._select(next(iter(self.variants)))
        return self

    def _select(self, key):
        v = self.variants[key]
        self.selected, self.out = v["capture"], v["out"]
        self.capacity_rows, self.capacities = v["capacity_rows"], v["capacities"]

    @property
    def segments(self):
        return self.selected.segments if self.selected is not None else []

    @property
    def between(self):
        return self.selected.between if self.selected is not None else []

    @property
    def graphs(self):
        return tuple(self.selected.segments) if self.selected is not None else None

    @property
    def march_ahead(self):
        return self.side_stream is not None

    def _warm_up_step(self):
        self.optimizer.zero_grad(set_to_none=True)
        self._forward_backward()
        self.exchange(self.sink.G)
        self._optimise()

    def _captured_step(self):
        out = self._forward_backward()
        self.exchange(self.sink.G)
        self._optimise_and_march()
        return out

    def _segment_ended(self):
        fo.forget_plan_events()
        self.model._presum_event = None

    def _first_segment_replayed(self):
        slot = self._replays % len(self.msg_ring)
        self._replays += 1
        if self.stage_in_graph:
            ev = torch.cuda.Event()
            ev.record()
            self.msg_events[slot] = ev

    def _capture(self, cap_block, cap_content):
        model = self.model
        self.optimizer.zero_grad(set_to_none=True)
        if self.march_ahead and not self.fixed_blocks:
            self._march_ahead()
        if self._capture_stream is None:
            self._capture_stream = torch.cuda.Stream()
        capture = SegmentedCapture(self._capture_stream, on_boundary=self._segment_ended, after_first=self._first_segment_replayed)
        out = capture.capture(self._captured_step)
        capacity_rows = [(model.local_step - 2) % 16, (model.local_step - 1) % 16]
        self.content_capacity = cap_content
        if self.marched is not None:
            capacity_rows = [(model.local_step - 1) % 16]
        return {"capture": capture, "out": out, "capacity_rows": capacity_rows,
                "capacities": [cap_block, cap_content] if self._blocks_issued_first() else [cap_content, cap_block]}

    def step(self, message, data=None, next_data=None, next_message=None):
        if self.selected is None:
            if data is not None:
                self._set_inputs(message, data)
                data = None
            self.prepare(message)
        unannounced = self._s_for is None or not torch.equal(self._s_for, message.detach().to("cpu", torch.float32))
        self._set_inputs(message, data, next_data, next_message, eager_copy=unannounced or not self.stage_in_graph)
        if unannounced:
            self.model.prepare_message(self.msg_dev)
        self._s_for = None if next_message is None else next_message.detach().to("cpu", torch.float32).clone()
        if self.distortion is not None and self.distortion.name == "scaling":
            self.distortion.set_scaling(host_uniform(self.distortion.seed, self._replays, 0.75, 1.25))
            self._select(self.distortion.out_width(self.data["watermark"]["rays_o_block"].shape[2]))
        self.selected.replay()
        self.steps_done += 1
        if self.opt_shard is not None:
            self.model._codebook_stale = True
        return self.out

    def ensure_capacity(self, growth=1.25):
        if self.selected is None:
            return False
        over = bool(self.overflowed())
        if exchange_active():
            import torch.distributed as dist
            flag = torch.tensor([1.0 if over else 0.0], device=self.device if dist.get_backend() == "nccl" else "cpu")
            dist.all_reduce(flag, op=dist.ReduceOp.MAX)
            over = bool(flag.item() > 0)
        if not over:
            return False
        self.headroom = (1.0 + self.headroom) * growth - 1.0
        self.content_headroom = (1.0 + self.content_headroom) * growth - 1.0
        message = self.msg_dev.detach().to("cpu", torch.float32)
        torch.cuda.synchronize()
        self.selected, self.marched = None, None
        self.model.drop_marched()
        self._s_for = None
        self.prepare(message)
        return True

    def overflowed(self):
        if self.marched is not None and len(self.marched) > 1:
            return any(int(r["counter"][0]) > r["capacity"] for r in self.marched)
        if self.marched is not None:
            return int(self.marched[0]["counter"][0]) > self.marched[0]["capacity"] or \
                int(self.model.step_counter[self.capacity_rows[-1], 0]) > self.content_capacity
        totals = self.model.step_counter[self.capacity_rows, 0].tolist()
# ... 2 lines not shown
```

Baseline: 4.485 million rays/s.

## Merge block and content field backward and scatter into single launches

Instead of running the field backward and the binned hash-table scatter once for the block render and once for the content render, the sink holds the first backward segment and launches one two-segment kernel for both, followed by one two-plan scatter and merge. The goal is fewer launches, better occupancy for the smaller segment, and less scatter traffic over the shared gradient table. In exchange it adds per-tile segment selection, cross-stream event waits when the two backwards run on different streams, and a flush path to make sure the held segment is always emitted.

```diff
diff --git a/include/nerfsig.h b/include/nerfsig.h
--- a/include/nerfsig.h
+++ b/include/nerfsig.h
@@ -124,6 +124,7 @@
 size_t hg_scatter_plan_bytes(uint32_t M);
 int hg_scatter_plan(const float *xyzs, uint32_t M, float bound, void *plan, nsig_stream_t stream);
 int hg_scatter_planned(const void *plan, uint32_t M, float *G, nsig_stream_t stream);
+int hg_scatter_planned2(const void *plan_a, uint32_t M_a, const void *plan_b, uint32_t M_b, float *G, nsig_stream_t stream);
 
 int hg_fanout_grad(const float *G, float *const *grads_host, uint32_t D, int accumulate, nsig_stream_t stream);
 
@@ -186,6 +187,11 @@
 int field_bwd_planned(const float *xyzs, uint32_t M, float bound, const float *grad_sigmas, const float *grad_rgbs,
                       const float *sigmas, const float *rgbs, const uint32_t *masks, const void *packed, void *plan,
                       nsig_stream_t stream);
+int field_bwd_planned2(const float *xyzs_a, uint32_t M_a, const float *grad_sigmas_a, const float *grad_rgbs_a,
+                       const float *sigmas_a, const float *rgbs_a, const uint32_t *masks_a, void *plan_a,
+                       const float *xyzs_b, uint32_t M_b, const float *grad_sigmas_b, const float *grad_rgbs_b,
+                       const float *sigmas_b, const float *rgbs_b, const uint32_t *masks_b, void *plan_b,
+                       float bound, const void *packed, nsig_stream_t stream);
 
 int opt_adam_dense(uint32_t n, float *const *params_host, const float *const *grads_host, float *const *exp_avg_host,
                    float *const *exp_avg_sq_host, float *const *steps_host, const uint32_t *numel_host, const float *lr, float beta1,
diff --git a/nerf_signature_amd/_native.py b/nerf_signature_amd/_native.py
--- a/nerf_signature_amd/_native.py
+++ b/nerf_signature_amd/_native.py
@@ -104,6 +104,8 @@
     "hg_scatter_plan_bytes": [_u32],
     "hg_scatter_plan": [_vp, _u32, _fl, _vp, _vp],
     "hg_scatter_planned": [_vp, _u32, _vp, _vp],
+    "field_bwd_planned2": [_vp, _u32, _vp, _vp, _vp, _vp, _vp, _vp, _vp, _u32, _vp, _vp, _vp, _vp, _vp, _vp, _fl, _vp, _vp],
+    "hg_scatter_planned2": [_vp, _u32, _vp, _u32, _vp, _vp],
     "field_fwd_trace_rows": [_vp, _vp, _u32, _vp, _fl, _vp, _vp, _vp, _vp, _vp, _vp, _vp, _vp, _vp, _vp, _vp],
     "field_fwd_trace_f16": [_vp, _vp, _u32, _vp, _fl, _vp, _vp, _vp, _vp, _vp, _vp, _vp, _vp, _vp, _vp, _vp],
     "field_bwd_trace_rows": [_u32, _vp, _vp, _vp, _vp, _vp, _vp, _vp, _vp, _vp, _vp, _vp, _vp, _vp, _vp],
diff --git a/nerf_signature_amd/csrc/field.hip b/nerf_signature_amd/csrc/field.hip
--- a/nerf_signature_amd/csrc/field.hip
+++ b/nerf_signature_amd/csrc/field.hip
@@ -653,26 +653,41 @@
     }
 }
 
-template <typename P>
-__device__ inline void field_bwd_pipelined(const char *lds, int lane, const float *__restrict__ xyzs, uint32_t M, float bound,
-                                           const float *__restrict__ g_sigma, const float *__restrict__ g_rgb, const float *__restrict__ sigmas,
-                                           const float *__restrict__ rgbs, const uint32_t *__restrict__ masks, ScatterPlan plan) {
+struct BwdSegment {
+    const float *xyzs, *g_sigma, *g_rgb, *sigmas, *rgbs;
+    const uint32_t *masks;
+    ScatterPlan plan;
+    uint32_t M, first_tile;
+};
+template <int kSegs>
+struct BwdSegments {
+    BwdSegment s[kSegs];
+};
+
+template <typename P, int kSegs>
+__device__ inline void field_bwd_pipelined(const char *lds, int lane, const BwdSegments<kSegs> &sg, float bound) {
+    static_assert(kSegs == 1 || kSegs == 2, "one render, or the block and the content render of a step");
     constexpr size_t kHalf = kBwdBytes;
     constexpr bool kNormalise = P::kMfmaPerProduct == 1;
     const int p = lane & 31, h = lane >> 5;
     const uint32_t wid = (uint32_t)__builtin_amdgcn_readfirstlane((int)(threadIdx.x >> 6));
-    const uint32_t n_tiles = ceil_div(M, 32u);
     const float e_lo = expf(-15.0f), e_hi = expf(15.0f), two_b = 2.0f * bound;
     uint32_t gbits = 0;
-    const uint32_t xcd = blockIdx.x & 7u, per_xcd = gridDim.x >> 3, n_chunks = ceil_div(n_tiles, 32u);
+#define NSIG_SEG(i, field) (kSegs == 1 || (i) == 0u ? sg.s[0].field : sg.s[kSegs - 1].field)
+    const uint32_t last_tiles = ceil_div(sg.s[kSegs - 1].M, 32u), first_last = sg.s[kSegs - 1].first_tile;
+    const uint32_t xcd = blockIdx.x & 7u, per_xcd = gridDim.x >> 3, n_chunks = ceil_div(first_last + last_tiles, 32u);
     uint32_t lq = blockIdx.x >> 3;
+    uint32_t r_seg = 0;
     auto next_tile = [&]() -> uint32_t {
         for (;; lq += per_xcd) {
             const uint32_t chunk = (lq >> 3) * 8u + xcd;
             if (chunk >= n_chunks) return ~0u;
-            const uint32_t tile = (chunk * 8u + (lq & 7u)) * 4u + wid;
-            if (tile < n_tiles) {
+            uint32_t tile = (chunk * 8u + (lq & 7u)) * 4u + wid;
+            const uint32_t seg = kSegs > 1 && tile >= first_last ? 1u : 0u;
+            tile -= seg ? first_last : 0u;
+            if (tile < ceil_div(NSIG_SEG(seg, M), 32u)) {
                 lq += per_xcd;
+                r_seg = seg;
                 return tile;
             }
         }
@@ -684,20 +699,21 @@
     f32x3u n_rgb = {0.0f, 0.0f, 0.0f}, n_grgb = {0.0f, 0.0f, 0.0f}, n_xyz = {0.0f, 0.0f, 0.0f};
     float n_gs = 0.0f, n_sig = 0.0f;
     auto request = [&](uint32_t tile) {
-        const uint32_t s = tile * 32 + p, sl = min(s, M - 1);
-        const uint32_t *mrow = masks + (size_t)tile * 192 + lane;
+        const uint32_t s = tile * 32 + p, sl = min(s, NSIG_SEG(r_seg, M) - 1);
+        const uint32_t *mrow = NSIG_SEG(r_seg, masks) + (size_t)tile * 192 + lane;
         n_mask[0] = mrow[0]; n_mask[1] = mrow[64]; n_mask[2] = mrow[128];
-        n_dst = *reinterpret_cast<const u32x4 *>(plan.dest + sl);
-        n_rgb = *reinterpret_cast<const f32x3u *>(rgbs + 3 * (size_t)sl);
-        n_grgb = *reinterpret_cast<const f32x3u *>(g_rgb + 3 * (size_t)sl);
-        n_xyz = *reinterpret_cast<const f32x3u *>(xyzs + 3 * (size_t)sl);
-        n_gs = g_sigma[sl];
-        n_sig = sigmas[sl];
+        n_dst = *reinterpret_cast<const u32x4 *>(NSIG_SEG(r_seg, plan.dest) + sl);
+        n_rgb = *reinterpret_cast<const f32x3u *>(NSIG_SEG(r_seg, rgbs) + 3 * (size_t)sl);
+        n_grgb = *reinterpret_cast<const f32x3u *>(NSIG_SEG(r_seg, g_rgb) + 3 * (size_t)sl);
+        n_xyz = *reinterpret_cast<const f32x3u *>(NSIG_SEG(r_seg, xyzs) + 3 * (size_t)sl);
+        n_gs = NSIG_SEG(r_seg, g_sigma)[sl];
+        n_sig = NSIG_SEG(r_seg, sigmas)[sl];
     };
     bool have = false;
     float p_x = 0.0f, p_y = 0.0f, p_z = 0.0f, p_g0 = 0.0f, p_g1 = 0.0f;
     uint32_t p_d0 = 0u, p_d1 = 0u;
     bool p_live = false;
+    uint32_t c_seg = 0, p_seg = 0;
     auto store_prev = [&]() {
         if (!p_live) return;
         uint32_t ix, iy, iz;
@@ -706,15 +722,23 @@
         codebook_axis((p_y + bound) / two_b, iy, wy);
         codebook_axis((p_z + bound) / two_b, iz, wz);
         const uint32_t q0 = 2u * (uint32_t)h;
-        plan.queue[p_d0] = pair_entry(ix, pair_hash(iy, iz, q0), wx, wy, wz, p_g0, p_g1, q0);
-        plan.queue[p_d1] = pair_entry(ix, pair_hash(iy, iz, q0 + 1u), wx, wy, wz, p_g0, p_g1, q0 + 1u);
+        uint4 *queue = NSIG_SEG(p_seg, plan.queue);
+        queue[p_d0] = pair_entry(ix, pair_hash(iy, iz, q0), wx, wy, wz, p_g0, p_g1, q0);
+        queue[p_d1] = pair_entry(ix, pair_hash(iy, iz, q0 + 1u), wx, wy, wz, p_g0, p_g1, q0 + 1u);
         gbits = max(gbits, max(__float_as_uint(p_g0) & 0x7fffffffu, __float_as_uint(p_g1) & 0x7fffffffu));
+    };
+    auto raise_gmax = [&](uint32_t seg) {
+#pragma unroll
+        for (int d = 32; d >= 1; d >>= 1) gbits = max(gbits, (uint32_t)__shfl_xor((int)gbits, d, 64));
+        uint32_t *word = &NSIG_SEG(seg, plan.hd)->gmax_bits;
+        if (lane == 0 && gbits > __hip_atomic_load(word, __ATOMIC_RELAXED, __HIP_MEMORY_SCOPE_AGENT)) atomicMax(word, gbits);
     };
     uint32_t tile = next_tile();
     if (tile != ~0u) request(tile);
+    c_seg = r_seg;
     while (tile != ~0u) {
         const uint32_t s = tile * 32 + p;
-        const bool live = s < M;
+        const bool live = s < NSIG_SEG(c_seg, M);
         float dv[3] = {0.0f, 0.0f, 0.0f}, head0 = 0.0f;
         if (h == 0 && live) {
             dv[0] = n_grgb.x * (n_rgb.x * (1.0f - n_rgb.x));
@@ -727,7 +751,13 @@
         float cx = n_xyz.x, cy = n_xyz.y, cz = n_xyz.z;
         asm volatile("" : "+v"(dv[0]), "+v"(dv[1]), "+v"(dv[2]), "+v"(head0), "+v"(mask_s), "+v"(mask_c0), "+v"(mask_c1), "+v"(d0), "+v"(d1),
                      "+v"(cx), "+v"(cy), "+v"(cz) :: "memory");
-        if (have) store_prev();
+        if (have) {
+            store_prev();
+            if (kSegs > 1 && p_seg != c_seg) {
+                raise_gmax(p_seg);
+                gbits = 0;
+            }
+        }
         const uint32_t upcoming = next_tile();
         if (upcoming != ~0u) request(upcoming);
         asm volatile("" ::: "memory");
@@ -770,22 +800,28 @@
         p_g0 = __shfl(dfe[0][0], p, 64) * unscale;
         p_g1 = __shfl(dfe[0][1], p, 64) * unscale;
         p_x = cx; p_y = cy; p_z = cz; p_d0 = d0; p_d1 = d1; p_live = live;
+        p_seg = c_seg;
+        c_seg = r_seg;
         have = true;
         tile = upcoming;
     }
     if (have) store_prev();
-#pragma unroll
-    for (int d = 32; d >= 1; d >>= 1) gbits = max(gbits, (uint32_t)__shfl_xor((int)gbits, d, 64));
-    if (lane == 0 && gbits > __hip_atomic_load(&plan.hd->gmax_bits, __ATOMIC_RELAXED, __HIP_MEMORY_SCOPE_AGENT)) atomicMax(&plan.hd->gmax_bits, gbits);
+    if (kSegs == 1 || have) raise_gmax(p_seg);
+#undef NSIG_SEG
 }
 
 template <typename P>
-__global__ void __launch_bounds__(256) k_field_bwd_train(const float *__restrict__ xyzs, uint32_t M, float bound, const float *__restrict__ g_sigma,
-                                                         const float *__restrict__ g_rgb, const float *__restrict__ sigmas, const float *__restrict__ rgbs,
-                                                         const uint32_t *__restrict__ masks, const char *__restrict__ packed, ScatterPlan plan) {
+__global__ void __launch_bounds__(256) k_field_bwd_train(BwdSegments<1> sg, float bound, const char *__restrict__ packed) {
     extern __shared__ __attribute__((aligned(16))) char lds[];
     stage_weights(lds, packed + P::kBwdOffset, (int)P::kBwdLds);
-    field_bwd_pipelined<P>(lds, threadIdx.x & 63, xyzs, M, bound, g_sigma, g_rgb, sigmas, rgbs, masks, plan);
+    field_bwd_pipelined<P, 1>(lds, threadIdx.x & 63, sg, bound);
+}
+
+template <typename P>
+__global__ void __launch_bounds__(256) k_field_bwd_train2(BwdSegments<2> sg, float bound, const char *__restrict__ packed) {
+    extern __shared__ __attribute__((aligned(16))) char lds[];
+    stage_weights(lds, packed + P::kBwdOffset, (int)P::kBwdLds);
+    field_bwd_pipelined<P, 2>(lds, threadIdx.x & 63, sg, bound);
 }
 
 }
@@ -1002,10 +1038,11 @@
     if (M == 0) return NSIG_OK;
     NSIG_REQUIRE(xyzs && grad_sigmas && grad_rgbs && sigmas && rgbs && masks && packed && plan, "field_bwd_planned: null pointer");
     NSIG_REQUIRE(bound > 0.0f && (reinterpret_cast<uintptr_t>(plan) & 15) == 0 && M < (1u << 28), "field_bwd_planned: bound must be positive, plan 16-byte aligned, M < 2^28");
-    if (mlp_precision() == 1 && bwd_pipelined())
-        k_field_bwd_train<F16><<<field_grid(M), 256, F16::kBwdLds, as_stream(stream)>>>(xyzs, M, bound, grad_sigmas, grad_rgbs, sigmas, rgbs, masks,
-                                                                                reinterpret_cast<const char *>(packed), scatter_plan_view(plan, M));
-    else if (mlp_precision() == 1)
+    if (mlp_precision() == 1 && bwd_pipelined()) {
+        BwdSegments<1> sg;
+        sg.s[0] = BwdSegment{xyzs, grad_sigmas, grad_rgbs, sigmas, rgbs, masks, scatter_plan_view(plan, M), M, 0u};
+        k_field_bwd_train<F16><<<field_grid(M), 256, F16::kBwdLds, as_stream(stream)>>>(sg, bound, reinterpret_cast<const char *>(packed));
+    } else if (mlp_precision() == 1)
         k_field_bwd<F16, false><<<field_grid(M), 256, F16::kBwdLds, as_stream(stream)>>>(xyzs, M, bound, 1.0f / kCodebookResolution, grad_sigmas, grad_rgbs, sigmas, rgbs, masks,
                                                                                  reinterpret_cast<const char *>(packed), nullptr, nullptr, nullptr, GradTrace{}, 0,
                                                                                  scatter_plan_view(plan, M));
@@ -1014,6 +1051,25 @@
                                                                                        masks, reinterpret_cast<const char *>(packed), nullptr, nullptr, nullptr, GradTrace{}, 0,
                                                                                        scatter_plan_view(plan, M));
     return check_launch("field_bwd_planned");
+}
+
+NSIG_EXPORT int field_bwd_planned2(const float *xyzs_a, uint32_t M_a, const float *grad_sigmas_a, const float *grad_rgbs_a, const float *sigmas_a,
+                                   const float *rgbs_a, const uint32_t *masks_a, void *plan_a, const float *xyzs_b, uint32_t M_b,
+                                   const float *grad_sigmas_b, const float *grad_rgbs_b, const float *sigmas_b, const float *rgbs_b,
+                                   const uint32_t *masks_b, void *plan_b, float bound, const void *packed, nsig_stream_t stream) {
+    if (M_a == 0) return field_bwd_planned(xyzs_b, M_b, bound, grad_sigmas_b, grad_rgbs_b, sigmas_b, rgbs_b, masks_b, packed, plan_b, stream);
+    if (M_b == 0) return field_bwd_planned(xyzs_a, M_a, bound, grad_sigmas_a, grad_rgbs_a, sigmas_a, rgbs_a, masks_a, packed, plan_a, stream);
+    NSIG_REQUIRE(packed && plan_a && plan_b && xyzs_a && grad_sigmas_a && grad_rgbs_a && sigmas_a && rgbs_a && masks_a && xyzs_b && grad_sigmas_b && grad_rgbs_b &&
+                 sigmas_b && rgbs_b && masks_b, "field_bwd_planned2: null pointer");
+    NSIG_REQUIRE(bound > 0.0f && ((reinterpret_cast<uintptr_t>(plan_a) | reinterpret_cast<uintptr_t>(plan_b)) & 15) == 0 && M_a < (1u << 27) && M_b < (1u << 27),
+                 "field_bwd_planned2: bound must be positive, plans 16-byte aligned, M < 2^27");
+    NSIG_REQUIRE(mlp_precision() == 1 && bwd_pipelined(), "field_bwd_planned2: needs the fp16 MLP and the pipelined backward (mlp_set_precision(1), mlp_set_pipelined bit 1)");
+    BwdSegments<2> sg;
+    sg.s[0] = BwdSegment{xyzs_a, grad_sigmas_a, grad_rgbs_a, sigmas_a, rgbs_a, masks_a, scatter_plan_view(plan_a, M_a), M_a, 0u};
+    const uint32_t first_b = ceil_div(ceil_div(M_a, 32u), 32u) * 32u;
+    sg.s[1] = BwdSegment{xyzs_b, grad_sigmas_b, grad_rgbs_b, sigmas_b, rgbs_b, masks_b, scatter_plan_view(plan_b, M_b), M_b, first_b};
+    k_field_bwd_train2<F16><<<field_grid(first_b * 32u + M_b), 256, F16::kBwdLds, as_stream(stream)>>>(sg, bound, reinterpret_cast<const char *>(packed));
+    return check_launch("field_bwd_planned2");
 }
 
 
diff --git a/nerf_signature_amd/csrc/hashgrid.hip b/nerf_signature_amd/csrc/hashgrid.hip
--- a/nerf_signature_amd/csrc/hashgrid.hip
+++ b/nerf_signature_amd/csrc/hashgrid.hip
@@ -676,6 +676,8 @@
     return n > 2048u ? 62 - E - (32 - __builtin_clz(n)) : 51 - E;
 }
 
+__device__ inline uint32_t gmax_of_two(uint32_t gmax_bits_a, uint32_t gmax_bits_b) { return max(gmax_bits_a, gmax_bits_b); }
+
 __device__ inline void adam_update(float g, float &p, float &m, float &v, float beta1, float beta2, float eps, float step_size, float inv_bc2_sqrt) {
     m = m + (1.0f - beta1) * (g - m);
     v = v * beta2 + ((1.0f - beta2) * g) * g;
@@ -691,10 +693,12 @@
     uint32_t on;
 };
 
+template <bool kTwo>
 __global__ void __launch_bounds__(1024) k_scatter_binned(const BinHeader *__restrict__ hd_all, const uint4 *__restrict__ queue_all, uint32_t M,
                                                          ScatterTargets tg, uint32_t replicas,
                                                          const uint32_t *__restrict__ set_max = nullptr, uint32_t n_set_max = 0, OwnerAdam adam = OwnerAdam{},
-                                                         unsigned long long *__restrict__ slabs = nullptr) {
+                                                         unsigned long long *__restrict__ slabs = nullptr, const BinHeader *__restrict__ hd_b = nullptr,
+                                                         const uint4 *__restrict__ queue_b = nullptr) {
     extern __shared__ unsigned long long acc64[];
     const BinHeader *__restrict__ hd = hd_all + blockIdx.y;
     const uint4 *__restrict__ queue = queue_all + (size_t)blockIdx.y * 4 * M;
@@ -706,18 +710,34 @@
 #pragma unroll
     for (int d = 32; d >= 1; d >>= 1) before += (uint32_t)__shfl_xor((int)before, d, 64);
     const uint32_t start = (uint32_t)__builtin_amdgcn_readfirstlane((int)before);
-    const uint32_t n = (uint32_t)__builtin_amdgcn_readfirstlane(__shfl((int)cnt, (int)slice, 64)), chunk = ceil_div(n, replicas);
+    const uint32_t n_a = (uint32_t)__builtin_amdgcn_readfirstlane(__shfl((int)cnt, (int)slice, 64));
+    uint32_t n = n_a, start_b = 0;
+    if (kTwo) {
+        const uint32_t cnt_b = hd_b->counts[lane];
+        uint32_t before_b = lane < slice ? cnt_b : 0u;
+#pragma unroll
+        for (int d = 32; d >= 1; d >>= 1) before_b += (uint32_t)__shfl_xor((int)before_b, d, 64);
+        start_b = (uint32_t)__builtin_amdgcn_readfirstlane((int)before_b);
+        n += (uint32_t)__builtin_amdgcn_readfirstlane(__shfl((int)cnt_b, (int)slice, 64));
+    }
+    const uint32_t chunk = ceil_div(n, replicas);
     const uint32_t beg = min(n, replica * chunk), end = min(n, beg + chunk);
     constexpr int kAhead = 4;
     typedef uint32_t u32x4_t __attribute__((ext_vector_type(4)));
     const u32x4_t *__restrict__ q = reinterpret_cast<const u32x4_t *>(queue + start);
+    const u32x4_t *__restrict__ q_b = kTwo ? reinterpret_cast<const u32x4_t *>(queue_b + start_b) : nullptr;
+    auto entry_at = [&](uint32_t i) -> const u32x4_t * {
+        if (!kTwo) return q + i;
+        return i < n_a ? q + i : q_b + (i - n_a);
+    };
     const uint32_t round = blockDim.x * kAhead;
     u32x4_t cur[kAhead] = {}, nxt[kAhead];
     if (beg < end) {
 #pragma unroll
-        for (int u = 0; u < kAhead; ++u) cur[u] = __builtin_nontemporal_load(q + min(beg + u * blockDim.x + threadIdx.x, end - 1));
+        for (int u = 0; u < kAhead; ++u) cur[u] = __builtin_nontemporal_load(entry_at(min(beg + u * blockDim.x + threadIdx.x, end - 1)));
     }
     uint32_t gb = hd->gmax_bits, mx = 0;
+    if (kTwo) gb = gmax_of_two(gb, hd_b->gmax_bits);
     __shared__ uint32_t smax;
     if (set_max != nullptr) {
         for (uint32_t i = threadIdx.x; i < n_set_max; i += blockDim.x) mx = max(mx, set_max[(size_t)blockIdx.y * n_set_max + i]);
@@ -746,11 +766,12 @@
     if (beg < end) {
         for (uint32_t base = beg; base < end; base += round) {
 #pragma unroll
-            for (int u = 0; u < kAhead; ++u) nxt[u] = __builtin_nontemporal_load(q + min(base + round + u * blockDim.x + threadIdx.x, end - 1));
+            for (int u = 0; u < kAhead; ++u) nxt[u] = __builtin_nontemporal_load(entry_at(min(base + round + u * blockDim.x + threadIdx.x, end - 1)));
             __builtin_amdgcn_sched_barrier(0);
 #pragma unroll
             for (int u = 0; u < kAhead; ++u) {
-                if (base + u * blockDim.x + threadIdx.x < end) {
+                const bool adds = !kTwo || ((cur[u][2] | cur[u][3]) & 0x7fffffffu) != 0u;
+                if (base + u * blockDim.x + threadIdx.x < end && adds) {
                     const uint32_t ix = cur[u][0] & 0xffffu, hyz = cur[u][0] >> 16;
                     const float wx = __uint_as_float(cur[u][1]), a0 = __uint_as_float(cur[u][2]), a1 = __uint_as_float(cur[u][3]);
                     unsigned long long *d0 = acc64 + 2u * ((ix ^ hyz) & (kBinRows - 1)), *d1 = acc64 + 2u * (((ix + 1u) ^ hyz) & (kBinRows - 1));
@@ -821,12 +842,16 @@
 
 constexpr uint32_t kMergeParts = 4, kMergeThreads = 1024;
 __global__ void __launch_bounds__(kMergeThreads) k_scatter_merge(const BinHeader *__restrict__ hd_all, ScatterTargets tg, uint32_t replicas,
-                                                                 const unsigned long long *__restrict__ slabs) {
+                                                                 const unsigned long long *__restrict__ slabs, const BinHeader *__restrict__ hd_b = nullptr) {
     constexpr uint32_t kSlab = 2u * kBinRows, kPartWords = kSlab / kMergeParts, kTrips = kPartWords / kMergeThreads;
     static_assert(kPartWords % kMergeThreads == 0, "whole trips");
     const BinHeader *__restrict__ hd = hd_all + blockIdx.y;
     const uint32_t slice = blockIdx.x / kMergeParts, part = blockIdx.x - slice * kMergeParts;
-    const uint32_t n = hd->counts[slice], gb = hd->gmax_bits;
+    uint32_t n = hd->counts[slice], gb = hd->gmax_bits;
+    if (hd_b != nullptr) {
+        n += hd_b->counts[slice];
+        gb = gmax_of_two(gb, hd_b->gmax_bits);
+    }
     if (n == 0 || gb >= 0x7f800000u) return;
     const int k = fixed_scale(gb, n);
     const uint32_t chunk = ceil_div(n, replicas);
@@ -1383,7 +1408,8 @@
     static bool attr_set = false;
     const size_t lds = (size_t)kBinRows * 2 * sizeof(unsigned long long);
     if (!attr_set) {
-        if (hipFuncSetAttribute(reinterpret_cast<const void *>(k_scatter_binned), hipFuncAttributeMaxDynamicSharedMemorySize, (int)lds) != hipSuccess) {
+        if (hipFuncSetAttribute(reinterpret_cast<const void *>(k_scatter_binned<false>), hipFuncAttributeMaxDynamicSharedMemorySize, (int)lds) != hipSuccess ||
+            hipFuncSetAttribute(reinterpret_cast<const void *>(k_scatter_binned<true>), hipFuncAttributeMaxDynamicSharedMemorySize, (int)lds) != hipSuccess) {
             set_error("%s: cannot reserve %zu bytes of LDS", who, lds);
             return NSIG_ERR_LAUNCH;
         }
@@ -1415,7 +1441,7 @@
     k_bin_scan<<<sets, 1024, 0, st>>>(hd, blocks);
     k_bin_write<<<dim3(blocks, sets), kBinThreads, 0, st>>>(rec, M, hd, queue);
     unsigned long long *slabs = replicas > 1 ? reinterpret_cast<unsigned long long *>(queue + (size_t)sets * 4 * M) : nullptr;
-    k_scatter_binned<<<dim3(kBinSlices * replicas, sets), 1024, lds, st>>>(hd, queue, M, tg, replicas, nullptr, 0u, OwnerAdam{}, slabs);
+    k_scatter_binned<false><<<dim3(kBinSlices * replicas, sets), 1024, lds, st>>>(hd, queue, M, tg, replicas, nullptr, 0u, OwnerAdam{}, slabs);
     if (replicas > 1) k_scatter_merge<<<dim3(kBinSlices * kMergeParts, sets), kMergeThreads, 0, st>>>(hd, tg, replicas, slabs);
     return check_launch(who);
 }
@@ -1455,11 +1481,28 @@
     ScatterTargets tg{};
     tg.g[0] = G;
     if (int e = owner_targets_aligned(tg, 1, "hg_scatter_planned")) return e;
-    k_scatter_binned<<<dim3(kBinSlices * kBinReplicas, 1), 1024, (size_t)kBinRows * 2 * sizeof(unsigned long long), as_stream(stream)>>>(pl.hd, pl.queue, M, tg,
+    k_scatter_binned<false><<<dim3(kBinSlices * kBinReplicas, 1), 1024, (size_t)kBinRows * 2 * sizeof(unsigned long long), as_stream(stream)>>>(pl.hd, pl.queue, M, tg,
                                                                                                                                            kBinReplicas, nullptr, 0u,
                                                                                                                                            OwnerAdam{}, pl.slabs);
     k_scatter_merge<<<dim3(kBinSlices * kMergeParts, 1), kMergeThreads, 0, as_stream(stream)>>>(pl.hd, tg, kBinReplicas, pl.slabs);
     return check_launch("hg_scatter_planned");
+}
+
+NSIG_EXPORT int hg_scatter_planned2(const void *plan_a, uint32_t M_a, const void *plan_b, uint32_t M_b, float *G, nsig_stream_t stream) {
+    if (M_a == 0) return hg_scatter_planned(plan_b, M_b, G, stream);
+    if (M_b == 0) return hg_scatter_planned(plan_a, M_a, G, stream);
+    NSIG_REQUIRE(plan_a && plan_b && G, "hg_scatter_planned2: null pointer");
+    NSIG_REQUIRE(((reinterpret_cast<uintptr_t>(plan_a) | reinterpret_cast<uintptr_t>(plan_b)) & 15) == 0 && M_a < (1u << 27) && M_b < (1u << 27),
+                 "hg_scatter_planned2: plans must be 16-byte aligned and M < 2^27");
+    if (int e = reserve_owner_lds("hg_scatter_planned2")) return e;
+    const ScatterPlan a = scatter_plan_view(const_cast<void *>(plan_a), M_a), b = scatter_plan_view(const_cast<void *>(plan_b), M_b);
+    ScatterTargets tg{};
+    tg.g[0] = G;
+    if (int e = owner_targets_aligned(tg, 1, "hg_scatter_planned2")) return e;
+    k_scatter_binned<true><<<dim3(kBinSlices * kBinReplicas, 1), 1024, (size_t)kBinRows * 2 * sizeof(unsigned long long), as_stream(stream)>>>(
+        a.hd, a.queue, M_a, tg, kBinReplicas, nullptr, 0u, OwnerAdam{}, a.slabs, b.hd, b.queue);
+    k_scatter_merge<<<dim3(kBinSlices * kMergeParts, 1), kMergeThreads, 0, as_stream(stream)>>>(a.hd, tg, kBinReplicas, a.slabs, b.hd);
+    return check_launch("hg_scatter_planned2");
 }
 
 NSIG_EXPORT size_t hg_scatter_levels_scratch_bytes(uint32_t M) {
@@ -1534,11 +1577,11 @@
     for (int l = 0; l < NSIG_BASE_LEVELS; ++l) {
         ScatterTargets one{};
         one.g[0] = tg.g[l];
-        k_scatter_binned<<<dim3(kBinSlices, 1), 1024, (size_t)kBinRows * 2 * sizeof(unsigned long long), st>>>(pl.hd + l, pl.queue + (size_t)l * kLevelQueueStride * M,
+        k_scatter_binned<false><<<dim3(kBinSlices, 1), 1024, (size_t)kBinRows * 2 * sizeof(unsigned long long), st>>>(pl.hd + l, pl.queue + (size_t)l * kLevelQueueStride * M,
                                                                                                                M_stride, one, 1u, pl.chunk_max + (size_t)l * pl.n_chunks, pl.n_chunks);
     }
 #else
-    k_scatter_binned<<<dim3(kBinSlices, NSIG_BASE_LEVELS), 1024, (size_t)kBinRows * 2 * sizeof(unsigned long long), st>>>(pl.hd, pl.queue, M_stride, tg, 1u,
+    k_scatter_binned<false><<<dim3(kBinSlices, NSIG_BASE_LEVELS), 1024, (size_t)kBinRows * 2 * sizeof(unsigned long long), st>>>(pl.hd, pl.queue, M_stride, tg, 1u,
                                                                                                                           pl.chunk_max, pl.n_chunks, adam);
 #endif
     return check_launch(who);
diff --git a/nerf_signature_amd/fieldops.py b/nerf_signature_amd/fieldops.py
--- a/nerf_signature_amd/fieldops.py
+++ b/nerf_signature_amd/fieldops.py
@@ -305,6 +305,20 @@
     return G
 
 
+def merged_backward_available():
+    return nv.fn("mlp_get_precision")() == 1 and (nv.fn("mlp_get_pipelined")() & 2) != 0
+
+
+def field_backward_planned2(a, b, bound, packed, G):
+    segs = []
+    for xyzs, g_sigma, g_rgb, sigmas, rgbs, masks, plan in (a, b):
+        plan.join()
+        segs += [nv.ptr(xyzs), plan.M, nv.ptr(g_sigma), nv.ptr(g_rgb), nv.ptr(sigmas), nv.ptr(rgbs), nv.ptr(masks), nv.ptr(plan.buf)]
+    nv.call("field_bwd_planned2", *segs, float(bound), nv.ptr(packed), nv.stream())
+    nv.call("hg_scatter_planned2", nv.ptr(a[6].buf), a[6].M, nv.ptr(b[6].buf), b[6].M, nv.ptr(G), nv.stream())
+    return G
+
+
 def field_backward_into(xyzs, bound, g_sigma, g_rgb, sigmas, rgbs, masks, packed, G, plan=None):
     if plan is not None:
         return field_backward_planned(xyzs, bound, g_sigma, g_rgb, sigmas, rgbs, masks, packed, plan, G)
@@ -319,10 +333,39 @@
         self.G = self.arena[:T_ROWS * 2].view(T_ROWS, 2)
         self.tail = self.arena[T_ROWS * 2:]
         self.selected = None
+        self.pair = False
+        self._held = None
 
     def zero_(self):
         self.G.zero_()
         self.selected = None
+        self._held = None
+
+    def submit(self, seg, bound, packed):
+        cur = torch.cuda.current_stream()
+        if self._held is None:
+            done = torch.cuda.Event()
+            done.record(cur)
+            self._held = (seg, bound, packed, cur, done)
+            return
+        first, bound0, packed0, stream0, done0 = self._held
+        if bound0 != bound or packed0.data_ptr() != packed.data_ptr():
+            self.flush()
+            field_backward_into(seg[0], bound, *seg[1:6], packed, self.G, seg[6])
+            return
+        self._held = None
+        if stream0 != cur:
+            cur.wait_event(done0)
+            for t in first[:6] + (first[6].buf,):
+                t.record_stream(cur)
+        field_backward_planned2(first, seg, bound, packed, self.G)
+
+    def flush(self):
+        held, self._held = self._held, None
+        if held is not None:
+            seg, bound, packed, stream, _ = held
+            with torch.cuda.stream(stream):
+                field_backward_into(seg[0], bound, *seg[1:6], packed, self.G, seg[6])
 
     def fanout(self, accumulate=False):
         if self.selected is None:
@@ -419,7 +462,10 @@
         if ctx.sink is not None:
             if isinstance(ctx.sink, SharedGradient):
                 ctx.sink.begin_accumulation(ctx.sink_selected)
-            field_backward_into(xyzs, ctx.bound, g_sigma, g_rgb, sigmas, rgbs, masks, packed, ctx.sink.G, plan)
+            if ctx.sink.pair and plan is not None and merged_backward_available():
+                ctx.sink.submit((xyzs, g_sigma.contiguous().float(), g_rgb.contiguous().float(), sigmas, rgbs, masks, plan), ctx.bound, packed)
+            else:
+                field_backward_into(xyzs, ctx.bound, g_sigma, g_rgb, sigmas, rgbs, masks, packed, ctx.sink.G, plan)
             return head + (None,) * ctx.n_diff
         G = torch.zeros(T_ROWS, 2, dtype=torch.float32, device=xyzs.device)
         field_backward_into(xyzs, ctx.bound, g_sigma, g_rgb, sigmas, rgbs, masks, packed, G, plan)
diff --git a/nerf_signature_amd/trainer.py b/nerf_signature_amd/trainer.py
--- a/nerf_signature_amd/trainer.py
+++ b/nerf_signature_amd/trainer.py
@@ -373,6 +373,8 @@
 
 class GraphedWatermarkLoop:
 
+    merged_backward = True
+
     def __init__(self, model, optimizer, render_kwargs, data, lambda_w=1.0, lambda_i=1.0, lr_lambda=None, headroom=0.0, overlap_content=True,
                  content_headroom=None, content_sampler=None, fixed_blocks=False, distortion="none", distortion_seed=0):
         self.distortion = None if distortion in (None, "none") else (distortion if isinstance(distortion, DistortionLayer) else DistortionLayer(distortion, distortion_seed))
@@ -477,6 +479,7 @@
             self.model._graphed_loops.remove(self)
 
     def _forward_backward(self):
+        self.sink._held = None
         if self.stage_in_graph and torch.cuda.is_current_stream_capturing():
             nv.call("loop_step_begin", nv.ptr(self.sink.G), self.sink.G.numel(), ctypes.c_void_p(self.ring_dev), len(self.msg_ring),
                     self.stage_width, nv.ptr(self.stage_counter), nv.ptr(self.msg_all), nv.stream())
@@ -506,6 +509,7 @@
         finally:
             set_weights_stream(None)
             set_grad_arena(None)
+        self.sink.flush()
         join_stream(torch.cuda.current_stream(), self.side_stream)
         if self.weights_stream is not self.side_stream:
             join_stream(torch.cuda.current_stream(), self.weights_stream)
@@ -631,6 +635,7 @@
         self.exchange.shared_scale = 1.0 if self.sharded else None
         self.opt_shard = dp.optimizer_shard(model.message_dim) if self.sharded else None
         model.codebook_shard = self.opt_shard
+        self.sink.pair = self.merged_backward and not self.sharded
         if self.distortion is not None and self.distortion.name == "scaling":
             o = self.data["watermark"]["rays_o_block"]
             self.distortion._buffers(tuple(o.shape), o.device)
```

After: 4.468 million rays/s (median of 2 runs). Within noise of the previous version (-0.4%).
